# Lumina-Group/libzkp

Measured on NVIDIA B200. Metric: groth16_bn254_proofs_per_sec_batched, higher is better.
Workload: dtype u256 (8x32-bit Montgomery limbs, integer)

## Files before the change

### include/lzkp_b200.h

```cpp
#ifndef LZKP_B200_H
#define LZKP_B200_H
#include <stddef.h>
#include <stdint.h>

#ifdef __cplusplus
extern "C" {
#endif

#define LZKP_OK 0
#define LZKP_E_INVALID (-1)
#define LZKP_E_NO_DEVICE (-2)
#define LZKP_E_CUDA (-3)
#define LZKP_E_STATE (-4)
#define LZKP_E_NOMEM (-5)
#define LZKP_E_UNSUPPORTED (-6)

#define LZKP_CIRCUIT_EQUALITY 0
#define LZKP_CIRCUIT_MEMBERSHIP 1

typedef struct lzkp_pk lzkp_pk;

typedef struct lzkp_pk_options {
    int window_bits;
    uint64_t table_budget_bytes;
    uint32_t max_chunk;
    uint32_t shard_index, shard_count;
} lzkp_pk_options;
#define LZKP_PARTIAL_BYTES 768

int lzkp_init(const int *devices, int n_devices);
int lzkp_device_count(void);
int lzkp_shutdown(void);
const char *lzkp_last_error(void);
uint64_t lzkp_kernel_launches(void);

#define LZKP_REGION_WITGEN 0
#define LZKP_REGION_WITNESS_MAP 1
#define LZKP_REGION_DIGITS 2
#define LZKP_REGION_MSM_G1 3
#define LZKP_REGION_MSM_G2 4
#define LZKP_REGION_ASSEMBLE 5
#define LZKP_PROFILE_REGIONS 8
int lzkp_profile_enable(int on);
int lzkp_profile_read(lzkp_pk *pk, double ms[LZKP_PROFILE_REGIONS], uint64_t count[LZKP_PROFILE_REGIONS], int reset);

int lzkp_pk_load(const uint8_t *pk_bytes, size_t len, int validate, lzkp_pk **out);
int lzkp_pk_load_ex(const uint8_t *pk_bytes, size_t len, int validate, const lzkp_pk_options *opt, lzkp_pk **out);
void lzkp_pk_free(lzkp_pk *pk);
int lzkp_pk_info(const lzkp_pk *pk, uint64_t info[8]);
int lzkp_pk_work(const lzkp_pk *pk, uint64_t work[4]);

int lzkp_circuit_load(lzkp_pk *pk, uint32_t m, uint32_t n_inst, uint32_t n_wit,
                      const uint32_t *a_rowptr, const uint32_t *a_col, const uint8_t *a_val,
                      const uint32_t *b_rowptr, const uint32_t *b_col, const uint8_t *b_val,
                      const uint32_t *c_rowptr, const uint32_t *c_col, const uint8_t *c_val);
int lzkp_circuit_builtin(lzkp_pk *pk, int kind, uint32_t param);
int lzkp_builtin_circuit_csr(int kind, uint32_t param, uint64_t shape[6], uint32_t *rowptr[3], uint32_t *col[3],
                             uint8_t *val[3]);

int lzkp_key_sizes(uint32_t m, uint32_t n_inst, uint32_t n_wit, size_t *pk_len, size_t *vk_len);
int lzkp_setup(uint32_t m, uint32_t n_inst, uint32_t n_wit,
               const uint32_t *a_rowptr, const uint32_t *a_col, const uint8_t *a_val,
               const uint32_t *b_rowptr, const uint32_t *b_col, const uint8_t *b_val,
               const uint32_t *c_rowptr, const uint32_t *c_col, const uint8_t *c_val,
               const uint8_t toxic[160], uint8_t *pk_out, size_t pk_cap, uint8_t *vk_out, size_t vk_cap);
int lzkp_setup_builtin(int kind, uint32_t param, const uint8_t toxic[160], uint8_t *pk_out, size_t pk_cap,
                       uint8_t *vk_out, size_t vk_cap);

int lzkp_generator_mul(int group, const uint8_t *scalars, size_t n, uint8_t *out_affine);

int lzkp_builtin_witness(int kind, uint32_t param, uint64_t value, uint64_t other, const uint64_t *set,
                         uint32_t set_len, const uint8_t *commitment, uint8_t *z_out, size_t z_cap);

int lzkp_prove_batch(lzkp_pk *pk, size_t n_proofs, const uint8_t *z, const uint8_t *r, const uint8_t *s,
                     uint8_t *proofs_out, int32_t *status);
int lzkp_prove_batch_device(lzkp_pk *pk, size_t n_proofs, const void *d_z, const void *d_r, const void *d_s,
                            void *d_proofs, void *d_status, void *stream);
int lzkp_prove_equality_batch(lzkp_pk *pk, size_t n_proofs, const uint64_t *a, const uint64_t *b,
                              const uint8_t *commitments, const uint8_t *r, const uint8_t *s, uint8_t *proofs_out,
                              uint8_t *commitments_out, int32_t *status);
int lzkp_prove_membership_batch(lzkp_pk *pk, size_t n_proofs, const uint64_t *value, const uint64_t *sets,
                                const uint32_t *set_len, uint32_t set_stride, const uint8_t *commitments,
                                const uint8_t *r, const uint8_t *s, uint8_t *proofs_out, uint8_t *commitments_out,
                                int32_t *status);
int lzkp_prove_equality_enveloped(lzkp_pk *pk, size_t n_proofs, const uint64_t *a, const uint64_t *b, const uint8_t *r,
                                  const uint8_t *s, uint8_t *envelopes_out, uint32_t *envelope_len, int32_t *status);
int lzkp_prove_membership_enveloped(lzkp_pk *pk, size_t n_proofs, const uint64_t *value, const uint64_t *sets,
                                    const uint32_t *set_len, uint32_t set_stride, const uint8_t *r, const uint8_t *s,
                                    uint8_t *envelopes_out, uint32_t envelope_stride, uint32_t *envelope_len,
                                    int32_t *status);
int lzkp_prove_equality_batch_device(lzkp_pk *pk, size_t n_proofs, const void *d_a, const void *d_b, const void *d_r,
                                     const void *d_s, void *d_proofs, void *d_status, void *stream);

int lzkp_witness_map(lzkp_pk *pk, size_t n_proofs, const uint8_t *z, uint8_t *h_out);

int lzkp_witness_map_device(lzkp_pk *pk, const void *d_z, void *d_h, void *stream);
int lzkp_pk_shard_info(const lzkp_pk *pk, uint32_t first[5], uint32_t count[5], uint32_t *map_ranks);
int lzkp_prove_partial_device(lzkp_pk *pk, const void *d_z, const void *d_r, const void *d_s, const void *d_h,
                              void *d_partial, void *d_status, void *stream, int phase);
int lzkp_prove_combine_device(lzkp_pk *pk, const void *d_partials, int n_partials, const void *d_r, const void *d_s,
                              void *d_proof, void *stream);

int lzkp_msm_g1(const uint8_t *bases_affine, const uint8_t *scalars, size_t n, uint8_t *out_affine);
int lzkp_msm_g2(const uint8_t *bases_affine, const uint8_t *scalars, size_t n, uint8_t *out_affine);
typedef struct lzkp_bases lzkp_bases;
int lzkp_bases_load(int group, const uint8_t *bases_affine, size_t n, int window_bits, int resident_windows,
                    int validate, lzkp_bases **out);
void lzkp_bases_free(lzkp_bases *b);
int lzkp_msm(lzkp_bases *b, const uint8_t *scalars, size_t n, uint8_t *out_affine);
int lzkp_msm_device(lzkp_bases *b, const void *d_scalars, size_t n, void *d_out_affine, void *stream);

int lzkp_ntt(uint8_t *data, uint32_t log_n, int inverse, int coset);
int lzkp_ntt_device(void *d_in, void *d_out, uint32_t log_n, int inverse, int coset, void *stream);

typedef struct lzkp_vk lzkp_vk;
int lzkp_vk_load(const uint8_t *vk_bytes, size_t len, lzkp_vk **out);
void lzkp_vk_free(lzkp_vk *vk);
int lzkp_verify_batch(lzkp_vk *vk, size_t n, const uint8_t *proofs, const uint8_t *public_inputs, size_t n_pub,
                      uint8_t *ok_out);
int lzkp_vk_info(const lzkp_vk *vk, uint64_t info[4]);

int lzkp_commit_value_snark(uint64_t value, uint8_t out[32]);

#ifdef __cplusplus
}
#endif
#endif
```

### integration/rust/lzkp-sys/src/lib.rs

```rust
#![allow(non_camel_case_types)]
use std::ffi::CStr;
use std::os::raw::{c_char, c_int, c_void};

#[repr(C)]
pub struct lzkp_pk {
    _private: [u8; 0],
}
#[repr(C)]
pub struct lzkp_vk {
    _private: [u8; 0],
}
#[repr(C)]
#[derive(Default, Clone, Copy)]
pub struct lzkp_pk_options {
    pub window_bits: c_int,
    pub table_budget_bytes: u64,
    pub max_chunk: u32,
    pub shard_index: u32,
    pub shard_count: u32,
}
pub const LZKP_CIRCUIT_EQUALITY: c_int = 0;
pub const LZKP_CIRCUIT_MEMBERSHIP: c_int = 1;

extern "C" {
    pub fn lzkp_init(devices: *const c_int, n_devices: c_int) -> c_int;
    pub fn lzkp_device_count() -> c_int;
    pub fn lzkp_last_error() -> *const c_char;
    pub fn lzkp_pk_load_ex(pk: *const u8, len: usize, validate: c_int, opt: *const lzkp_pk_options,
                           out: *mut *mut lzkp_pk) -> c_int;
    pub fn lzkp_pk_free(pk: *mut lzkp_pk);
    pub fn lzkp_circuit_builtin(pk: *mut lzkp_pk, kind: c_int, param: u32) -> c_int;
    pub fn lzkp_key_sizes(m: u32, n_inst: u32, n_wit: u32, pk_len: *mut usize, vk_len: *mut usize) -> c_int;
    pub fn lzkp_setup_builtin(kind: c_int, param: u32, toxic: *const u8, pk_out: *mut u8, pk_cap: usize,
                              vk_out: *mut u8, vk_cap: usize) -> c_int;
    pub fn lzkp_prove_batch(pk: *mut lzkp_pk, n: usize, z: *const u8, r: *const u8, s: *const u8,
                            proofs_out: *mut u8, status: *mut i32) -> c_int;
    pub fn lzkp_prove_equality_batch(pk: *mut lzkp_pk, n: usize, a: *const u64, b: *const u64,
                                     commitments: *const u8, r: *const u8, s: *const u8, proofs_out: *mut u8,
                                     commitments_out: *mut u8, status: *mut i32) -> c_int;
    pub fn lzkp_prove_membership_batch(pk: *mut lzkp_pk, n: usize, value: *const u64, sets: *const u64,
                                       set_len: *const u32, set_stride: u32, commitments: *const u8,
                                       r: *const u8, s: *const u8, proofs_out: *mut u8,
                                       commitments_out: *mut u8, status: *mut i32) -> c_int;
    pub fn lzkp_prove_equality_enveloped(pk: *mut lzkp_pk, n: usize, a: *const u64, b: *const u64, r: *const u8,
                                         s: *const u8, envelopes_out: *mut u8, envelope_len: *mut u32,
                                         status: *mut i32) -> c_int;
    pub fn lzkp_prove_membership_enveloped(pk: *mut lzkp_pk, n: usize, value: *const u64, sets: *const u64,
                                           set_len: *const u32, set_stride: u32, r: *const u8, s: *const u8,
                                           envelopes_out: *mut u8, envelope_stride: u32, envelope_len: *mut u32,
                                           status: *mut i32) -> c_int;
    pub fn lzkp_vk_load(vk: *const u8, len: usize, out: *mut *mut lzkp_vk) -> c_int;
    pub fn lzkp_vk_free(vk: *mut lzkp_vk);
    pub fn lzkp_vk_info(vk: *const lzkp_vk, info: *mut u64) -> c_int;
    pub fn lzkp_verify_batch(vk: *mut lzkp_vk, n: usize, proofs: *const u8, public_inputs: *const u8, n_pub: usize,
                             ok_out: *mut u8) -> c_int;
    pub fn lzkp_commit_value_snark(value: u64, out: *mut u8) -> c_int;
    pub fn lzkp_msm_g1(bases: *const u8, scalars: *const u8, n: usize, out: *mut u8) -> c_int;
    pub fn lzkp_msm_g2(bases: *const u8, scalars: *const u8, n: usize, out: *mut u8) -> c_int;
    pub fn lzkp_ntt(data: *mut u8, log_n: u32, inverse: c_int, coset: c_int) -> c_int;
    pub fn lzkp_prove_batch_device(pk: *mut lzkp_pk, n: usize, d_z: *const c_void, d_r: *const c_void,
                                   d_s: *const c_void, d_proofs: *mut c_void, d_status: *mut c_void,
                                   stream: *mut c_void) -> c_int;
}

pub fn last_error() -> String {
    unsafe { CStr::from_ptr(lzkp_last_error()).to_string_lossy().into_owned() }
}

pub struct DevicePk(*mut lzkp_pk);
unsafe impl Send for DevicePk {}
unsafe impl Sync for DevicePk {}

impl DevicePk {
    pub fn load(pk_bytes: &[u8], kind: c_int, param: u32, validate: bool) -> Result<Self, String> {
        let mut h: *mut lzkp_pk = std::ptr::null_mut();
        let opt = lzkp_pk_options::default();
        let rc = unsafe { lzkp_pk_load_ex(pk_bytes.as_ptr(), pk_bytes.len(), validate as c_int, &opt, &mut h) };
        if rc != 0 {
            return Err(last_error());
        }
        let pk = DevicePk(h);
        if unsafe { lzkp_circuit_builtin(pk.0, kind, param) } != 0 {
            return Err(last_error());
        }
        Ok(pk)
    }

    pub fn prove_equality(&self, a: &[u64], b: &[u64], commitments: &[[u8; 32]], r: &[[u8; 32]],
                          s: &[[u8; 32]]) -> Result<Vec<Option<[u8; 256]>>, String> {
        let n = a.len();
        if b.len() != n || commitments.len() != n || r.len() != n || s.len() != n {
            return Err(format!("prove_equality: slice lengths differ (a {}, b {}, commitments {}, r {}, s {})",
                               n, b.len(), commitments.len(), r.len(), s.len()));
        }
        let mut proofs = vec![0u8; 256 * n];
        let mut status = vec![0i32; n];
        let rc = unsafe {
            lzkp_prove_equality_batch(self.0, n, a.as_ptr(), b.as_ptr(), commitments.as_ptr() as *const u8,
                                      r.as_ptr() as *const u8, s.as_ptr() as *const u8, proofs.as_mut_ptr(),
                                      std::ptr::null_mut(), status.as_mut_ptr())
        };
        if rc != 0 {
            return Err(last_error());
        }
        Ok((0..n).map(|i| if status[i] == 0 {
            let mut p = [0u8; 256];
            p.copy_from_slice(&proofs[256 * i..256 * (i + 1)]);
            Some(p)
        } else { None }).collect())
    }
}

impl Drop for DevicePk {
    fn drop(&mut self) {
        unsafe { lzkp_pk_free(self.0) }
    }
}
```

### libzkp_b200/_ffi.py

```python
from __future__ import annotations

import ctypes as C
import os

_HERE = os.path.dirname(os.path.abspath(__file__))
LIB_PATH = os.environ.get("LZKP_B200_LIB") or os.path.join(_HERE, "_lib", "liblzkp_b200.so")

LZKP_OK = 0
LZKP_E_INVALID = -1
LZKP_E_NO_DEVICE = -2
LZKP_E_CUDA = -3
LZKP_E_STATE = -4
LZKP_E_NOMEM = -5
LZKP_E_UNSUPPORTED = -6
LZKP_CIRCUIT_EQUALITY = 0
LZKP_CIRCUIT_MEMBERSHIP = 1
LZKP_PARTIAL_BYTES = 768


class PkOptions(C.Structure):
    _fields_ = [("window_bits", C.c_int), ("table_budget_bytes", C.c_uint64), ("max_chunk", C.c_uint32),
                ("shard_index", C.c_uint32), ("shard_count", C.c_uint32)]


_vp, _sz, _int = C.c_void_p, C.c_size_t, C.c_int
_u32, _u64 = C.c_uint32, C.c_uint64
SIGNATURES = {
    "lzkp_init": (_int, [_vp, _int]),
    "lzkp_device_count": (_int, []),
    "lzkp_shutdown": (_int, []),
    "lzkp_last_error": (C.c_char_p, []),
    "lzkp_kernel_launches": (_u64, []),
    "lzkp_profile_enable": (_int, [_int]),
    "lzkp_profile_read": (_int, [_vp, C.POINTER(C.c_double), C.POINTER(_u64), _int]),
    "lzkp_pk_load": (_int, [_vp, _sz, _int, C.POINTER(_vp)]),
    "lzkp_pk_load_ex": (_int, [_vp, _sz, _int, C.POINTER(PkOptions), C.POINTER(_vp)]),
    "lzkp_pk_free": (None, [_vp]),
    "lzkp_pk_info": (_int, [_vp, C.POINTER(_u64)]),
    "lzkp_pk_work": (_int, [_vp, C.POINTER(_u64)]),
    "lzkp_pk_shard_info": (_int, [_vp, C.POINTER(_u32), C.POINTER(_u32), C.POINTER(_u32)]),
    "lzkp_circuit_load": (_int, [_vp, _u32, _u32, _u32] + [_vp] * 9),
    "lzkp_circuit_builtin": (_int, [_vp, _int, _u32]),
    "lzkp_builtin_circuit_csr": (_int, [_int, _u32, C.POINTER(_u64), C.POINTER(_vp), C.POINTER(_vp), C.POINTER(_vp)]),
    "lzkp_key_sizes": (_int, [_u32, _u32, _u32, C.POINTER(_sz), C.POINTER(_sz)]),
    "lzkp_setup": (_int, [_u32, _u32, _u32] + [_vp] * 9 + [_vp, _vp, _sz, _vp, _sz]),
    "lzkp_setup_builtin": (_int, [_int, _u32, _vp, _vp, _sz, _vp, _sz]),
    "lzkp_generator_mul": (_int, [_int, _vp, _sz, _vp]),
    "lzkp_prove_batch": (_int, [_vp, _sz, _vp, _vp, _vp, _vp, _vp]),
    "lzkp_prove_batch_device": (_int, [_vp, _sz, _vp, _vp, _vp, _vp, _vp, _vp]),
    "lzkp_builtin_witness": (_int, [_int, _u32, _u64, _u64, _vp, _u32, _vp, _vp, _sz]),
    "lzkp_prove_equality_batch": (_int, [_vp, _sz, _vp, _vp, _vp, _vp, _vp, _vp, _vp, _vp]),
    "lzkp_prove_membership_batch": (_int, [_vp, _sz, _vp, _vp, _vp, _u32, _vp, _vp, _vp, _vp, _vp, _vp]),
    "lzkp_prove_equality_enveloped": (_int, [_vp, _sz, _vp, _vp, _vp, _vp, _vp, _vp, _vp]),
    "lzkp_prove_membership_enveloped": (_int, [_vp, _sz, _vp, _vp, _vp, _u32, _vp, _vp, _vp, _u32, _vp, _vp]),
    "lzkp_prove_equality_batch_device": (_int, [_vp, _sz, _vp, _vp, _vp, _vp, _vp, _vp, _vp]),
    "lzkp_witness_map": (_int, [_vp, _sz, _vp, _vp]),
    "lzkp_witness_map_device": (_int, [_vp, _vp, _vp, _vp]),
    "lzkp_prove_partial_device": (_int, [_vp, _vp, _vp, _vp, _vp, _vp, _vp, _vp, _int]),
    "lzkp_prove_combine_device": (_int, [_vp, _vp, _int, _vp, _vp, _vp, _vp]),
    "lzkp_msm_g1": (_int, [_vp, _vp, _sz, _vp]),
    "lzkp_msm_g2": (_int, [_vp, _vp, _sz, _vp]),
    "lzkp_bases_load": (_int, [_int, _vp, _sz, _int, _int, _int, C.POINTER(_vp)]),
    "lzkp_bases_free": (None, [_vp]),
    "lzkp_msm": (_int, [_vp, _vp, _sz, _vp]),
    "lzkp_msm_device": (_int, [_vp, _vp, _sz, _vp, _vp]),
    "lzkp_ntt": (_int, [_vp, _u32, _int, _int]),
    "lzkp_ntt_device": (_int, [_vp, _vp, _u32, _int, _int, _vp]),
    "lzkp_vk_load": (_int, [_vp, _sz, C.POINTER(_vp)]),
    "lzkp_vk_free": (None, [_vp]),
    "lzkp_vk_info": (_int, [_vp, C.POINTER(_u64)]),
    "lzkp_verify_batch": (_int, [_vp, _sz, _vp, _vp, _sz, _vp]),
    "lzkp_commit_value_snark": (_int, [_u64, _vp]),
}

_lib = None


def lib():
    global _lib
    if _lib is None:
        if not os.path.exists(LIB_PATH):
            raise ImportError(
                f"{LIB_PATH} is missing: build it with `python -c 'import __graft_entry__ as g; g.build()'` "
                "(the engine has no CPU fallback)")
        L = C.CDLL(LIB_PATH)
        for name, (res, args) in SIGNATURES.items():
            fn = getattr(L, name)
            fn.restype = res
            fn.argtypes = args
        _lib = L
    return _lib


def last_error() -> str:
    return (lib().lzkp_last_error() or b"").decode("utf-8", "replace")


def check(rc: int) -> None:
    if rc != LZKP_OK:
        from .errors import EngineError
        raise EngineError(rc, last_error())
```

### libzkp_b200/csrc/engine.cu

```cuda
#include <cuda_runtime.h>
#include <atomic>
#include <cmath>
#include <cstdio>
#include <cstdlib>
#include <mutex>
#include <string>
#include <thread>
#include <type_traits>
#include <vector>

#include "common.h"
#include "host_util.h"
#include "kernels_prove.cuh"
#include "tables.h"
#include "large.h"
#include "setup.h"
#include "verify.h"

using namespace lzkp;
using namespace lzkp::eng;

static thread_local std::string g_err;
static std::mutex g_mu;
static int g_device = -1;
static std::vector<int> g_devices;
static thread_local int t_device = -1;
static uint64_t g_mimc_uploaded = 0;
static std::atomic<int> g_profile{0};

namespace lzkp {
namespace eng {
std::atomic<uint64_t> g_launches{0};
int fail(int code, const std::string &msg) {
    g_err = msg;
    return code;
}
int DBuf::alloc(size_t n) {
    release();
    if (n == 0) n = 16;
    cudaError_t e = cudaMalloc(&p, n);
    if (e != cudaSuccess) {
        p = nullptr;
        cudaGetLastError();
        return fail(LZKP_E_NOMEM, "cudaMalloc(" + std::to_string(n) + "): " + cudaGetErrorString(e));
    }
    bytes = n;
    return LZKP_OK;
}
void DBuf::release() {
    if (p) cudaFree(p);
    p = nullptr;
    bytes = 0;
}
int ensure_device() {
    std::lock_guard<std::mutex> lk(g_mu);
    if (g_device < 0) {
        int n = 0;
        cudaError_t e = cudaGetDeviceCount(&n);
        if (e != cudaSuccess || n == 0) {
            cudaGetLastError();
            return fail(LZKP_E_NO_DEVICE, "no CUDA device: this engine has no CPU fallback");
        }
        int dev = 0;
        if (const char *lr = getenv("LOCAL_RANK")) dev = atoi(lr) % n;
        g_device = dev;
    }
    const int dev = t_device >= 0 ? t_device : g_device;
    CUDA_TRY(cudaSetDevice(dev));
    if (!(g_mimc_uploaded >> (dev & 63) & 1)) {
        std::vector<Fr> c(110);
        for (uint32_t i = 0; i < 110; i++) c[i] = host::mimc_constant(i);
        CUDA_TRY(cudaMemcpyToSymbol(c_mimc, c.data(), sizeof(Fr) * 110));
        g_mimc_uploaded |= 1ull << (dev & 63);
    }
    return LZKP_OK;
}
int current_device() { return t_device >= 0 ? t_device : g_device; }
DeviceScope::DeviceScope(int dev) : prev(t_device) {
    t_device = dev;
    cudaSetDevice(dev);
}
DeviceScope::~DeviceScope() {
    t_device = prev;
    const int back = prev >= 0 ? prev : g_device;
    if (back >= 0) cudaSetDevice(back);
}
}
}


struct MsmPlan {
    DBuf table;
    DBuf unit_dig, unit_tbl;
    DBuf items[4];
    DBuf msm_items[4];
    uint32_t n_items[4] = {0, 0, 0, 0};
    uint32_t item_len[4] = {8, 32, 128, 512};
    uint32_t n_units = 0, n_rows = 0, n_msm = 0;
    std::vector<uint32_t> msm_unit_begin;
    std::vector<uint2> msm_items_host[4];
};

struct HBuf {
    void *p = nullptr;
    size_t bytes = 0;
    int ensure(size_t n) {
        if (n <= bytes) return LZKP_OK;
        if (p) cudaFreeHost(p);
        p = nullptr;
        bytes = 0;
        cudaError_t err = cudaMallocHost(&p, n);
        if (err != cudaSuccess) { p = nullptr; cudaGetLastError(); return fail(LZKP_E_NOMEM, "cudaMallocHost failed"); }
        bytes = n;
        return LZKP_OK;
    }
    template <class T> T *as() const { return reinterpret_cast<T *>(p); }
    ~HBuf() { if (p) cudaFreeHost(p); }
};
struct Workspace {
    uint32_t chunk = 0;
    DBuf z, abc, tmp, h, dig, r, s, rs, part1, part2, res1, res2, proofs, status, a, b, commit, sets, setlen, env, envlen;
    HBuf h_proofs, h_status, h_commit, h_env, h_envlen;
    cudaEvent_t last_use = nullptr;
    ~Workspace() { if (last_use) cudaEventDestroy(last_use); }
};
static int ws_acquire(Workspace &ws, cudaStream_t st) {
    if (!ws.last_use) CUDA_TRY(cudaEventCreateWithFlags(&ws.last_use, cudaEventDisableTiming));
    else CUDA_TRY(cudaStreamWaitEvent(st, ws.last_use, 0));
    return LZKP_OK;
}
static int ws_release(Workspace &ws, cudaStream_t st) {
    CUDA_TRY(cudaEventRecord(ws.last_use, st));
    return LZKP_OK;
}

struct lzkp_pk {
    std::mutex mu;
    int device = 0;
    std::vector<lzkp_pk *> replicas;
    uint32_t n_vars = 0, n_inst = 0, n_wit = 0, n = 0, log_n = 0, m = 0;
    bool has_circuit = false;
    int kind = -1;
    uint32_t kind_param = 0;
    int c = 16;
    uint32_t W = 16, N = 32768;
    uint64_t table_bytes = 0;
    uint32_t max_chunk = 8192;
    uint32_t n_dig_rows = 0, nz = 0;
    MsmPlan g1, g2;
    MsmPlan g1_lat;
    uint32_t row_sz = 0, row_rz = 0;
    bool has_lat = false;
    ProofConsts consts;
    DBuf csr_rowptr[3], csr_col[3], csr_val[3];
    CsrDev csr[3];
    DBuf tw_fwd, tw_inv, coset_br, uncoset_br;
    NttTables ntt;
    Workspace ws[2];
    bool large = false;
    bool tiled_wm = false;
    MsmBases *L_a = nullptr, *L_b1 = nullptr, *L_b2 = nullptr, *L_l = nullptr, *L_h = nullptr;
    DBuf L_sa, L_sb, L_sl, L_sb1;
    cudaStream_t L_st[3] = {nullptr, nullptr, nullptr}, L_st_scale = nullptr;
    cudaEvent_t L_ev_in = nullptr, L_ev_done[3] = {nullptr, nullptr, nullptr}, L_ev_a = nullptr, L_ev_scale = nullptr;
    uint32_t shard_index = 0, shard_count = 1, map_ranks = 1;
    bool L_scaled = false;
    uint32_t L_lo[5] = {0, 0, 0, 0, 0}, L_cnt[5] = {0, 0, 0, 0, 0};
    cudaStream_t stream = nullptr, stream2 = nullptr;
    cudaEvent_t ev_fork = nullptr, ev_join[2] = {nullptr, nullptr};
    cudaStream_t chunk_stream(int i) const { return (i & 1) ? stream2 : stream; }
    struct Mark { int region; cudaEvent_t a, b; };
    std::vector<Mark> marks;
    double prof_ms[LZKP_PROFILE_REGIONS] = {0};
    uint64_t prof_count[LZKP_PROFILE_REGIONS] = {0};
    ~lzkp_pk() {
        for (lzkp_pk *r : replicas) { DeviceScope ds(r->device); delete r; }
        for (auto &m : marks) { cudaEventDestroy(m.a); cudaEventDestroy(m.b); }
        for (MsmBases *b : {L_a, L_b1, L_b2, L_l, L_h}) if (b) msm_bases_free(b);
        for (auto s_ : L_st) if (s_) cudaStreamDestroy(s_);
        if (L_ev_in) cudaEventDestroy(L_ev_in);
        if (L_ev_a) cudaEventDestroy(L_ev_a);
        if (L_ev_scale) cudaEventDestroy(L_ev_scale);
        if (L_st_scale) cudaStreamDestroy(L_st_scale);
        for (auto ev : L_ev_done) if (ev) cudaEventDestroy(ev);
        if (ev_fork) cudaEventDestroy(ev_fork);
        for (auto ev : ev_join) if (ev) cudaEventDestroy(ev);
        if (stream2) cudaStreamDestroy(stream2);
        if (stream) cudaStreamDestroy(stream);
    }
};

struct BaseRef { uint32_t dig_row, tbl_row; };
static int finish_plan(MsmPlan &pl, const std::vector<std::vector<BaseRef>> &msms, uint32_t W) {
    std::vector<uint32_t> ud, ut;
    pl.msm_unit_begin.clear();
    for (auto &ms : msms) {
        pl.msm_unit_begin.push_back((uint32_t)ud.size());
        for (auto &b : ms)
            for (uint32_t w = 0; w < W; w++) {
                ud.push_back(b.dig_row * W + w);
                ut.push_back(b.tbl_row * W + w);
            }
    }
    pl.msm_unit_begin.push_back((uint32_t)ud.size());
    pl.n_units = (uint32_t)ud.size();
    pl.n_msm = (uint32_t)msms.size();
    TRY(upload(pl.unit_dig, ud));
    TRY(upload(pl.unit_tbl, ut));
    for (int v = 0; v < 4; v++) {
        std::vector<uint2> items, mi;
        for (uint32_t q = 0; q < pl.n_msm; q++) {
            uint32_t first = (uint32_t)items.size();
            for (uint32_t u = pl.msm_unit_begin[q]; u < pl.msm_unit_begin[q + 1]; u += pl.item_len[v])
                items.push_back(make_uint2(u, std::min(u + pl.item_len[v], pl.msm_unit_begin[q + 1])));
            mi.push_back(make_uint2(first, (uint32_t)items.size()));
        }
        pl.n_items[v] = (uint32_t)items.size();
        pl.msm_items_host[v] = mi;
        TRY(upload(pl.items[v], items));
        TRY(upload(pl.msm_items[v], mi));
    }
    return LZKP_OK;
}

static uint32_t fit_item_len(const std::vector<std::vector<BaseRef>> &msms, uint32_t W, uint32_t resident) {
    uint32_t best = 128;
    uint64_t best_cost = UINT64_MAX;
    for (uint32_t len = 96; len <= 192; len++) {
        uint64_t items = 0, cost = 0;
        for (auto &ms : msms) items += ((uint64_t)ms.size() * W + len - 1) / len;
        for (uint64_t gx : {8u, 16u, 32u, 64u}) cost += (gx * items + resident - 1) / resident * len * (64 / gx);
        if (cost < best_cost) { best_cost = cost; best = len; }
    }
    return best;
}

static inline uint32_t window_count(int c) { return (uint32_t)((255 + c - 1) / c); }

namespace {
struct Reader {
    const uint8_t *p, *end;
    bool take(size_t n, const uint8_t **out) {
        if ((size_t)(end - p) < n) return false;
        *out = p;
        p += n;
        return true;
    }
    bool g1(host::G1Canon &o) { const uint8_t *b; return take(64, &b) && host::read_g1(b, o); }
    bool g2(host::G2Canon &o) { const uint8_t *b; return take(128, &b) && host::read_g2(b, o); }
    bool vec_g1(std::vector<host::G1Canon> &v) {
        const uint8_t *b;
        if (!take(8, &b)) return false;
        uint64_t len;
        memcpy(&len, b, 8);
        if (len > (uint64_t)(end - p) / 64) return false;
        v.resize(len);
        for (auto &x : v) if (!g1(x)) return false;
        return true;
    }
    bool vec_g2(std::vector<host::G2Canon> &v) {
        const uint8_t *b;
        if (!take(8, &b)) return false;
        uint64_t len;
        memcpy(&len, b, 8);
        if (len > (uint64_t)(end - p) / 128) return false;
        v.resize(len);
        for (auto &x : v) if (!g2(x)) return false;
        return true;
    }
};
host::G1Canon neg_canon(const host::G1Canon &p) {
    host::G1Canon r = p;
    if (!host::is_inf(p)) {
        Fq m = Fq::modulus();
        sub8(r.y.l, m.l, p.y.l);
    }
    return r;
}
}

static int pk_load_impl(const uint8_t *bytes, size_t len, int validate, const lzkp_pk_options *opt, lzkp_pk *pk) {
    static_assert(sizeof(host::G1Canon) == sizeof(G1Affine) && sizeof(host::G2Canon) == sizeof(G2Affine), "layout");
    Reader rd{bytes, bytes + len};
    host::G1Canon alpha_g1, beta_g1, delta_g1;
    host::G2Canon beta_g2, gamma_g2, delta_g2;
    std::vector<host::G1Canon> gamma_abc, a_q, b1_q, h_q, l_q;
    std::vector<host::G2Canon> b2_q;
    bool ok = rd.g1(alpha_g1) && rd.g2(beta_g2) && rd.g2(gamma_g2) && rd.g2(delta_g2) && rd.vec_g1(gamma_abc) &&
              rd.g1(beta_g1) && rd.g1(delta_g1) && rd.vec_g1(a_q) && rd.vec_g1(b1_q) && rd.vec_g2(b2_q) &&
              rd.vec_g1(h_q) && rd.vec_g1(l_q);
    if (!ok || rd.p != rd.end) return fail(LZKP_E_INVALID, "proving key: malformed ark-serialize bytes");
    const uint32_t nv = (uint32_t)a_q.size();
    if (nv < 2 || b1_q.size() != nv || b2_q.size() != nv || l_q.size() >= nv || gamma_abc.size() + l_q.size() != nv)
        return fail(LZKP_E_INVALID, "proving key: inconsistent query lengths");
    const uint32_t n = (uint32_t)h_q.size() + 1;
    if (n < 2 || (n & (n - 1))) return fail(LZKP_E_INVALID, "proving key: h_query length + 1 is not a power of two");
    pk->n_vars = nv;
    pk->n_wit = (uint32_t)l_q.size();
    pk->n_inst = nv - pk->n_wit;
    pk->n = n;
    pk->log_n = 0;
    while ((1u << pk->log_n) < n) pk->log_n++;
    pk->nz = nv - 1;
    pk->n_dig_rows = pk->nz + 3 + (n - 1);
    const uint32_t ROW_R = pk->nz, ROW_S = pk->nz + 1, ROW_RS = pk->nz + 2, ROW_H = pk->nz + 3;

    {
        size_t free_b0 = 0, total_b0 = 0;
        CUDA_TRY(cudaMemGetInfo(&free_b0, &total_b0));
        const uint64_t budget0 = opt && opt->table_budget_bytes ? opt->table_budget_bytes : (uint64_t)(free_b0 * 0.6);
        const uint64_t rows1_max = 2ull * nv + pk->n_wit + n + 2, rows2_max = (uint64_t)nv + 1;
        const uint64_t min_table = (rows1_max * 64 + rows2_max * 128) * 32 * 128;
        pk->large = pk->log_n > 16 || min_table > budget0 || getenv("LZKP_FORCE_LARGE") != nullptr;
    }
    if (pk->large) {
        CUDA_TRY(cudaStreamCreate(&pk->stream));
    CUDA_TRY(cudaStreamCreate(&pk->stream2));
    CUDA_TRY(cudaEventCreateWithFlags(&pk->ev_fork, cudaEventDisableTiming));
    for (auto &ev : pk->ev_join) CUDA_TRY(cudaEventCreateWithFlags(&ev, cudaEventDisableTiming));
        const int wb = opt && opt->window_bits ? opt->window_bits : 0;
        pk->shard_count = opt && opt->shard_count > 1 ? opt->shard_count : 1;
        pk->shard_index = pk->shard_count > 1 ? opt->shard_index : 0;
        if (pk->shard_index >= pk->shard_count) return fail(LZKP_E_INVALID, "shard_index >= shard_count");
        const uint32_t G_ = pk->shard_count;
        const uint64_t w_g2 = getenv("LZKP_SHARD_G2_WEIGHT") ? (uint64_t)atoi(getenv("LZKP_SHARD_G2_WEIGHT")) : (G_ > 2 ? 32 : 28);
        const uint64_t sizes[5] = {nv, nv, (uint64_t)pk->n_wit + 1, (uint64_t)n - 1, nv}, wts[5] = {10, 10, 10, 10, w_g2};
        const double Wh = (double)sizes[3] * wts[3];
        double Wz = 0;
        for (int q : {0, 1, 2, 4}) Wz += (double)sizes[q] * wts[q];
        const double map_frac = getenv("LZKP_SHARD_MAP_COST") ? atof(getenv("LZKP_SHARD_MAP_COST")) : (G_ > 4 ? 0.085 : 0.11);
        const double M = G_ > 1 ? map_frac * (Wz + Wh) : 0.0;
        uint32_t k = 1;
        while (k < G_ && k * ((Wz + Wh + k * M) / G_ - M) < Wh) k++;
        const double T = (Wz + Wh + k * M) / G_;
        std::vector<double> cutz(G_ + 1, 0.0), share(G_, 0.0);
        for (uint32_t i = 0; i < G_; i++) share[i] = i < k ? std::max(0.0, T - M - Wh / k) : T;
        const double piece_cost = G_ > 2 ? (getenv("LZKP_SHARD_PIECE_COST") ? atof(getenv("LZKP_SHARD_PIECE_COST")) : (G_ > 4 ? 0.25 : 0.45)) * 2.76e6 : 0.0;
        std::vector<double> adj(share);
        for (int round = 0; round < 4; round++) {
            double tot = 0;
            for (uint32_t i = 0; i < G_; i++) tot += adj[i];
            for (uint32_t i = 0; i < G_; i++) cutz[i + 1] = cutz[i] + adj[i] * Wz / tot;
            double bounds[5] = {0, 0, 0, 0, 0};
            { int j = 0; for (int q : {0, 1, 2, 4}) { bounds[j + 1] = bounds[j] + (double)sizes[q] * wts[q]; j++; } }
            if (piece_cost != 0.0)
                for (uint32_t i = 1; i < G_; i++)
                    for (int j = 1; j < 4; j++)
                        if (std::fabs(cutz[i] - bounds[j]) < 1.0e5) cutz[i] = bounds[j];
            if (round == 3 || piece_cost == 0.0) break;
            double extra_total = 0;
            std::vector<double> extra(G_, 0.0);
            for (uint32_t i = 0; i < G_; i++) {
                int pieces = 0;
                for (int j = 0; j < 4; j++)
                    if (std::min(cutz[i + 1], bounds[j + 1]) - std::max(cutz[i], bounds[j]) > 1e-6 * Wz) pieces++;
                extra[i] = piece_cost * std::max(0, pieces - 1);
                extra_total += extra[i];
            }
            for (uint32_t i = 0; i < G_; i++) adj[i] = std::max(0.0, share[i] - extra[i] + extra_total / G_);
        }
        pk->map_ranks = k;
        const uint32_t me = pk->shard_index;
        if (me < k) {
            pk->L_lo[3] = (uint32_t)(sizes[3] * me / k);
            pk->L_cnt[3] = (uint32_t)(sizes[3] * (me + 1) / k) - pk->L_lo[3];
        } else {
            pk->L_lo[3] = 0;
            pk->L_cnt[3] = 0;
        }
        double acc_w = 0;
        for (int q : {0, 1, 2, 4}) {
            auto first_at = [&](double w) -> uint64_t {
                if (w <= acc_w) return 0;
                return std::min<uint64_t>((uint64_t)std::ceil((w - acc_w) / wts[q]), sizes[q]);
            };
            uint64_t lo = first_at(cutz[me]), hi = me + 1 == G_ ? sizes[q] : first_at(cutz[me + 1]);
            pk->L_lo[q] = (uint32_t)lo;
            pk->L_cnt[q] = (uint32_t)(hi - lo);
            acc_w += (double)sizes[q] * wts[q];
        }
        auto load1 = [&](std::vector<host::G1Canon> v, size_t skip, const host::G1Canon *extra, int q, MsmBases **out) {
            v.erase(v.begin(), v.begin() + skip);
            if (extra) v.push_back(*extra);
            return msm_bases_load(1, reinterpret_cast<const uint8_t *>(v.data() + pk->L_lo[q]), pk->L_cnt[q], wb, 1, validate, out, 1);
        };
        host::G1Canon nd1 = neg_canon(delta_g1);
        TRY(load1(a_q, 1, &delta_g1, 0, &pk->L_a));
        TRY(load1(b1_q, 1, &delta_g1, 1, &pk->L_b1));
        TRY(load1(l_q, 0, &nd1, 2, &pk->L_l));
        TRY(load1(h_q, 0, nullptr, 3, &pk->L_h));
        {
            std::vector<host::G2Canon> v(b2_q.begin() + 1, b2_q.end());
            v.push_back(delta_g2);
            TRY(msm_bases_load(2, reinterpret_cast<const uint8_t *>(v.data() + pk->L_lo[4]), pk->L_cnt[4], wb, 1, validate, &pk->L_b2, 1));
        }
        {
            int prio_lo = 0, prio_hi = 0;
            CUDA_TRY(cudaDeviceGetStreamPriorityRange(&prio_lo, &prio_hi));
            const bool prio = !(getenv("LZKP_NO_STREAM_PRIORITY") && atoi(getenv("LZKP_NO_STREAM_PRIORITY")));
            for (int i = 0; i < 3; i++)
                CUDA_TRY(cudaStreamCreateWithPriority(&pk->L_st[i], cudaStreamNonBlocking, prio_lo));
            CUDA_TRY(cudaStreamCreateWithPriority(&pk->L_st_scale, cudaStreamNonBlocking, prio ? prio_hi : prio_lo));
        }
        CUDA_TRY(cudaEventCreateWithFlags(&pk->L_ev_in, cudaEventDisableTiming));
        CUDA_TRY(cudaEventCreateWithFlags(&pk->L_ev_a, cudaEventDisableTiming));
        CUDA_TRY(cudaEventCreateWithFlags(&pk->L_ev_scale, cudaEventDisableTiming));
        for (auto &ev : pk->L_ev_done) CUDA_TRY(cudaEventCreateWithFlags(&ev, cudaEventDisableTiming));
        pk->c = wb ? wb : 16;
        pk->W = (255 + pk->c - 1) / pk->c;
        pk->max_chunk = 1;
        pk->table_bytes = ((uint64_t)(a_q.size() + b1_q.size() + l_q.size() + 1 + h_q.size()) * 64 + (uint64_t)b2_q.size() * 128) * pk->W;
        std::vector<host::G1Canon> misc1 = {alpha_g1, beta_g1, a_q[0], b1_q[0]};
        std::vector<host::G2Canon> misc2 = {beta_g2, b2_q[0]};
        DBuf d_misc1, d_misc2, d_out1, d_out2;
        cudaStream_t st = pk->stream;
        TRY(upload(d_misc1, misc1)); TRY(upload(d_misc2, misc2));
        LAUNCH(k_fq_to_mont, 1, 128, 0, st, d_misc1.as<Fq>(), misc1.size() * 2);
        LAUNCH(k_fq_to_mont, 1, 128, 0, st, d_misc2.as<Fq>(), misc2.size() * 4);
        if (validate) {
            std::vector<host::G1Canon> v1 = gamma_abc;
            v1.push_back(alpha_g1); v1.push_back(beta_g1); v1.push_back(delta_g1); v1.push_back(a_q[0]); v1.push_back(b1_q[0]);
            std::vector<host::G2Canon> v2 = {beta_g2, gamma_g2, delta_g2, b2_q[0]};
            DBuf d_v1, d_v2, d_bad;
            TRY(upload(d_v1, v1)); TRY(upload(d_v2, v2)); TRY(d_bad.alloc(sizeof(int)));
            CUDA_TRY(cudaMemsetAsync(d_bad.p, 0, sizeof(int), st));
            LAUNCH(k_fq_to_mont, (unsigned)((v1.size() * 2 + 127) / 128), 128, 0, st, d_v1.as<Fq>(), v1.size() * 2);
            LAUNCH(k_fq_to_mont, 1, 128, 0, st, d_v2.as<Fq>(), v2.size() * 4);
            LAUNCH(k_check_g1, (unsigned)((v1.size() + 63) / 64), 64, 0, st, d_v1.as<G1Affine>(), (uint32_t)v1.size(), d_bad.as<int>());
            LAUNCH(k_check_g2, 1, 64, 0, st, d_v2.as<G2Affine>(), (uint32_t)v2.size(), d_bad.as<int>());
            int bad = 0;
            CUDA_TRY(cudaMemcpyAsync(&bad, d_bad.p, sizeof(int), cudaMemcpyDeviceToHost, st));
            CUDA_TRY(cudaStreamSynchronize(st));
            if (bad) return fail(LZKP_E_INVALID, "proving key: " + std::to_string(bad) + " point(s) off-curve or outside the subgroup");
        }
        TRY(d_out1.alloc(2 * sizeof(G1Affine))); TRY(d_out2.alloc(sizeof(G2Affine)));
        LAUNCH((k_affine_add<Fq>), 1, 1, 0, st, d_misc1.as<G1Affine>() + 0, d_misc1.as<G1Affine>() + 2, d_out1.as<G1Affine>() + 0, 0);
        LAUNCH((k_affine_add<Fq>), 1, 1, 0, st, d_misc1.as<G1Affine>() + 1, d_misc1.as<G1Affine>() + 3, d_out1.as<G1Affine>() + 1, 0);
        LAUNCH((k_affine_add<Fq2>), 1, 1, 0, st, d_misc2.as<G2Affine>() + 0, d_misc2.as<G2Affine>() + 1, d_out2.as<G2Affine>(), 0);
        G1Affine c1[2];
        G2Affine c2;
        CUDA_TRY(cudaMemcpyAsync(c1, d_out1.p, sizeof(c1), cudaMemcpyDeviceToHost, st));
        CUDA_TRY(cudaMemcpyAsync(&c2, d_out2.p, sizeof(c2), cudaMemcpyDeviceToHost, st));
        CUDA_TRY(cudaStreamSynchronize(st));
        pk->consts.a0 = c1[0]; pk->consts.b0 = c1[1]; pk->consts.b2 = c2;
        CUDA_TRY(cudaGetLastError());
        return LZKP_OK;
    }

    std::vector<host::G1Canon> rows1;
    std::vector<host::G2Canon> rows2;
    std::vector<std::vector<BaseRef>> msm1(5), msm2(1);
    std::vector<BaseRef> a_all, b1_all;
    auto add1 = [&](const host::G1Canon &p) { rows1.push_back(p); return (uint32_t)rows1.size() - 1; };
    auto same_point = [](const host::G1Canon &u, const host::G1Canon &v) {
        return memcmp(&u.x, &v.x, sizeof(Fq)) == 0 && memcmp(&u.y, &v.y, sizeof(Fq)) == 0;
    };
    for (uint32_t j = 1; j < nv; j++) {
        const bool has_a = !host::is_inf(a_q[j]), has_b = !host::is_inf(b1_q[j]);
        if (has_a && has_b && same_point(a_q[j], b1_q[j])) {
            const BaseRef ref{j - 1, add1(a_q[j])};
            msm1[4].push_back(ref); a_all.push_back(ref); b1_all.push_back(ref);
            continue;
        }
        if (has_a) { msm1[0].push_back({j - 1, add1(a_q[j])}); a_all.push_back(msm1[0].back()); }
        if (has_b) { msm1[1].push_back({j - 1, add1(b1_q[j])}); b1_all.push_back(msm1[1].back()); }
    }
    for (uint32_t j = 0; j < pk->n_wit; j++) if (!host::is_inf(l_q[j])) msm1[2].push_back({pk->n_inst + j - 1, add1(l_q[j])});
    for (uint32_t i = 0; i + 1 < n; i++) if (!host::is_inf(h_q[i])) msm1[3].push_back({ROW_H + i, add1(h_q[i])});
    if (!host::is_inf(delta_g1)) {
        uint32_t rd1 = add1(delta_g1), rnd1 = add1(neg_canon(delta_g1));
        msm1[0].push_back({ROW_R, rd1});
        msm1[1].push_back({ROW_S, rd1});
        msm1[2].push_back({ROW_RS, rnd1});
        a_all.push_back({ROW_R, rd1});
    }
    std::vector<std::vector<BaseRef>> msm1_lat(6);
    {
        pk->row_sz = pk->n_dig_rows;
        pk->row_rz = pk->n_dig_rows + pk->nz;
        msm1_lat[0] = a_all;
        msm1_lat[2] = msm1[2];
        msm1_lat[3] = msm1[3];
        for (auto &b : a_all) if (b.dig_row < pk->nz) msm1_lat[4].push_back({pk->row_sz + b.dig_row, b.tbl_row});
        for (auto &b : b1_all) msm1_lat[5].push_back({pk->row_rz + b.dig_row, b.tbl_row});
        auto mont = [](const host::G1Canon &c) { return G1Affine{Fq::from_canonical(c.x), Fq::from_canonical(c.y)}; };
        auto canon = [](const G1Affine &m) { host::G1Canon c; c.x = m.x.to_canonical(); c.y = m.y.to_canonical(); return c; };
        auto sum2 = [&](const host::G1Canon &u, const host::G1Canon &v) {
            G1XYZZ t = host::is_inf(u) ? G1XYZZ::inf() : G1XYZZ::from_affine(mont(u));
            if (!host::is_inf(v)) t.madd(mont(v));
            return t.is_inf() ? host::G1Canon{Fq::zero(), Fq::zero()} : canon(t.to_affine());
        };
        const host::G1Canon a0c = sum2(alpha_g1, a_q[0]), b0c = sum2(beta_g1, b1_q[0]), d2c = sum2(delta_g1, delta_g1);
        if (!host::is_inf(a0c)) msm1_lat[4].push_back({ROW_S, add1(a0c)});
        if (!host::is_inf(b0c)) msm1_lat[5].push_back({ROW_R, add1(b0c)});
        if (!host::is_inf(d2c)) msm1_lat[5].push_back({ROW_RS, add1(d2c)});
        pk->n_dig_rows += 2 * pk->nz;
        pk->has_lat = true;
    }
    for (uint32_t j = 1; j < nv; j++)
        if (!host::is_inf(b2_q[j])) { rows2.push_back(b2_q[j]); msm2[0].push_back({j - 1, (uint32_t)rows2.size() - 1}); }
    if (!host::is_inf(delta_g2)) { rows2.push_back(delta_g2); msm2[0].push_back({ROW_S, (uint32_t)rows2.size() - 1}); }
    pk->g1.n_rows = (uint32_t)rows1.size();
    pk->g2.n_rows = (uint32_t)rows2.size();

    size_t free_b = 0, total_b = 0;
    CUDA_TRY(cudaMemGetInfo(&free_b, &total_b));
    uint64_t budget = opt && opt->table_budget_bytes ? opt->table_budget_bytes : (uint64_t)(free_b * 0.6);
    int c = opt && opt->window_bits ? opt->window_bits : 0;
    if (const char *e = getenv("LZKP_WINDOW_BITS")) if (!c) c = atoi(e);
    auto bytes_for = [&](int cc) {
        uint64_t W = window_count(cc), N = 1ull << (cc - 1);
        return (rows1.size() * 64ull + rows2.size() * 128ull) * W * N;
    };
    if (c == 0) {
        c = 16;
        while (c > 8 && bytes_for(c) > budget) c--;
    }
    if (c < 8 || c > 17) return fail(LZKP_E_INVALID, "window_bits must be in [8,17]");
    if (bytes_for(c) > free_b) return fail(LZKP_E_NOMEM, "window tables do not fit in device memory");
    pk->c = c;
    pk->W = window_count(c);
    pk->N = 1u << (c - 1);
    pk->table_bytes = bytes_for(c);
    pk->max_chunk = opt && opt->max_chunk ? opt->max_chunk : 8192;
    if (pk->max_chunk > 32768) pk->max_chunk = 32768;

    CUDA_TRY(cudaStreamCreate(&pk->stream));
    CUDA_TRY(cudaStreamCreate(&pk->stream2));
    CUDA_TRY(cudaEventCreateWithFlags(&pk->ev_fork, cudaEventDisableTiming));
    for (auto &ev : pk->ev_join) CUDA_TRY(cudaEventCreateWithFlags(&ev, cudaEventDisableTiming));
    CUDA_TRY(cudaStreamCreateWithFlags(&pk->L_st[0], cudaStreamNonBlocking));
    CUDA_TRY(cudaEventCreateWithFlags(&pk->L_ev_in, cudaEventDisableTiming));
    CUDA_TRY(cudaEventCreateWithFlags(&pk->L_ev_done[0], cudaEventDisableTiming));
    cudaStream_t st = pk->stream;

    std::vector<host::G1Canon> misc1 = {alpha_g1, beta_g1, delta_g1, a_q[0], b1_q[0]};
    std::vector<host::G2Canon> misc2 = {beta_g2, gamma_g2, delta_g2, b2_q[0]};
    DBuf d_rows1, d_rows2, d_misc1, d_misc2, d_out1, d_out2;
    TRY(upload(d_rows1, rows1)); TRY(upload(d_rows2, rows2)); TRY(upload(d_misc1, misc1)); TRY(upload(d_misc2, misc2));
    auto to_mont = [&](DBuf &b, size_t n_fq) {
        if (n_fq) LAUNCH(k_fq_to_mont, (unsigned)((n_fq + 127) / 128), 128, 0, st, b.as<Fq>(), n_fq);
    };
    to_mont(d_rows1, rows1.size() * 2); to_mont(d_rows2, rows2.size() * 4);
    to_mont(d_misc1, misc1.size() * 2); to_mont(d_misc2, misc2.size() * 4);
    if (validate) {
        std::vector<host::G1Canon> all1 = gamma_abc;
        std::vector<host::G2Canon> all2;
        DBuf d_all1, d_bad;
        TRY(upload(d_all1, all1));
        to_mont(d_all1, all1.size() * 2);
        TRY(d_bad.alloc(sizeof(int)));
        CUDA_TRY(cudaMemsetAsync(d_bad.p, 0, sizeof(int), st));
        auto chk1 = [&](DBuf &b, size_t cnt) {
            if (cnt) LAUNCH(k_check_g1, (unsigned)((cnt + 63) / 64), 64, 0, st, b.as<G1Affine>(), (uint32_t)cnt, d_bad.as<int>());
        };
        auto chk2 = [&](DBuf &b, size_t cnt) {
            if (cnt) LAUNCH(k_check_g2, (unsigned)((cnt + 63) / 64), 64, 0, st, b.as<G2Affine>(), (uint32_t)cnt, d_bad.as<int>());
        };
        chk1(d_rows1, rows1.size()); chk1(d_misc1, misc1.size()); chk1(d_all1, all1.size());
        chk2(d_rows2, rows2.size()); chk2(d_misc2, misc2.size());
        int bad = 0;
        CUDA_TRY(cudaMemcpyAsync(&bad, d_bad.p, sizeof(int), cudaMemcpyDeviceToHost, st));
        CUDA_TRY(cudaStreamSynchronize(st));
        if (bad) return fail(LZKP_E_INVALID, "proving key: " + std::to_string(bad) + " point(s) off-curve or outside the subgroup");
    }
    TRY(d_out1.alloc(2 * sizeof(G1Affine))); TRY(d_out2.alloc(sizeof(G2Affine)));
    LAUNCH((k_affine_add<Fq>), 1, 1, 0, st, d_misc1.as<G1Affine>() + 0, d_misc1.as<G1Affine>() + 3, d_out1.as<G1Affine>() + 0, 0);
    LAUNCH((k_affine_add<Fq>), 1, 1, 0, st, d_misc1.as<G1Affine>() + 1, d_misc1.as<G1Affine>() + 4, d_out1.as<G1Affine>() + 1, 0);
    LAUNCH((k_affine_add<Fq2>), 1, 1, 0, st, d_misc2.as<G2Affine>() + 0, d_misc2.as<G2Affine>() + 3, d_out2.as<G2Affine>(), 0);
    G1Affine c1[2];
    G2Affine c2;
    CUDA_TRY(cudaMemcpyAsync(c1, d_out1.p, sizeof(c1), cudaMemcpyDeviceToHost, st));
    CUDA_TRY(cudaMemcpyAsync(&c2, d_out2.p, sizeof(c2), cudaMemcpyDeviceToHost, st));
    CUDA_TRY(cudaStreamSynchronize(st));
    pk->consts.a0 = c1[0]; pk->consts.b0 = c1[1]; pk->consts.b2 = c2;

    TRY(pk->g1.table.alloc((size_t)rows1.size() * pk->W * pk->N * sizeof(G1Affine)));
    TRY(pk->g2.table.alloc((size_t)rows2.size() * pk->W * pk->N * sizeof(G2Affine)));
    if (!rows1.empty())
        TRY(build_table_g1(d_rows1.p, (uint32_t)rows1.size(), c, pk->W, pk->N, pk->g1.table.p, st));
    if (!rows2.empty())
        TRY(build_table_g2(d_rows2.p, (uint32_t)rows2.size(), c, pk->W, pk->N, pk->g2.table.p, st));
    {
        uint32_t resident = 0;
        TRY(batch_msm_g1_resident(c > 16 ? 4 : 2, &resident));
        pk->g1.item_len[2] = fit_item_len(msm1, pk->W, resident);
    }
    TRY(finish_plan(pk->g1, msm1, pk->W));
    TRY(finish_plan(pk->g1_lat, msm1_lat, pk->W));
    TRY(finish_plan(pk->g2, msm2, pk->W));
    {
        const uint64_t per_proof = (uint64_t)nv * 32 + 7ull * n * 32 + (uint64_t)pk->n_dig_rows * pk->W * (c > 16 ? 4 : 2) +
                                   (uint64_t)pk->g1.n_items[2] * sizeof(G1XYZZ) + (uint64_t)pk->g2.n_items[1] * sizeof(G2XYZZ) +
                                   4 * sizeof(G1XYZZ) + sizeof(G2XYZZ) + 1024;
        size_t free_now = 0, total_now = 0;
        CUDA_TRY(cudaMemGetInfo(&free_now, &total_now));
        uint64_t fit = (uint64_t)(free_now * 0.4) / (2 * per_proof);
        fit = std::max<uint64_t>(32, fit / 32 * 32);
        if (pk->max_chunk > fit) pk->max_chunk = (uint32_t)fit;
    }
    CUDA_TRY(cudaGetLastError());
    return LZKP_OK;
}

static int circuit_install(lzkp_pk *pk, uint32_t m, uint32_t n_inst, uint32_t n_wit, const uint32_t *const rowptr[3],
                           const uint32_t *const col[3], const uint8_t *const val[3]) {
    if (n_inst != pk->n_inst || n_wit != pk->n_wit) return fail(LZKP_E_INVALID, "circuit shape does not match the proving key");
    uint64_t need = (uint64_t)m + n_inst;
    uint32_t n = 1;
    while (n < need) n <<= 1;
    if (n != pk->n) return fail(LZKP_E_INVALID, "circuit domain size does not match the proving key's h_query");
    pk->tiled_wm = pk->large || pk->log_n > 12;
    cudaStream_t st = pk->stream;
    for (int k = 0; k < 3; k++) {
        uint32_t nnz = rowptr[k][m];
        for (uint32_t i = 0; i < nnz; i++) if (col[k][i] >= pk->n_vars) return fail(LZKP_E_INVALID, "matrix column out of range");
        TRY(pk->csr_rowptr[k].alloc(sizeof(uint32_t) * (m + 1)));
        TRY(pk->csr_col[k].alloc(sizeof(uint32_t) * nnz));
        TRY(pk->csr_val[k].alloc(sizeof(Fr) * (size_t)nnz));
        CUDA_TRY(cudaMemcpy(pk->csr_rowptr[k].p, rowptr[k], sizeof(uint32_t) * (m + 1), cudaMemcpyHostToDevice));
        if (nnz) {
            CUDA_TRY(cudaMemcpy(pk->csr_col[k].p, col[k], sizeof(uint32_t) * nnz, cudaMemcpyHostToDevice));
            CUDA_TRY(cudaMemcpy(pk->csr_val[k].p, val[k], 32 * (size_t)nnz, cudaMemcpyHostToDevice));
            LAUNCH(k_to_r2_form, (nnz + 127) / 128, 128, 0, st, pk->csr_val[k].as<Fr>(), nnz);
        }
        pk->csr[k] = CsrDev{pk->csr_rowptr[k].as<uint32_t>(), pk->csr_col[k].as<uint32_t>(), pk->csr_val[k].as<Fr>()};
    }
    pk->m = m;
    Fr w, wi, g, gi;
    for (int i = 0; i < 8; i++) { w.l[i] = FrParams::ROOT28(i); wi.l[i] = FrParams::ROOT28_INV(i); g.l[i] = FrParams::GEN(i); gi.l[i] = FrParams::GEN_INV(i); }
    for (uint32_t i = pk->log_n; i < 28; i++) { w = w.sqr(); wi = wi.sqr(); }
    Fr ninv = host::fr_from_u64(n).inverse();
    Fr gn = g;
    for (uint32_t i = 0; i < pk->log_n; i++) gn = gn.sqr();
    Fr zinv = (gn - Fr::one()).inverse();
    if (pk->tiled_wm) {
        pk->ntt = NttTables{nullptr, nullptr, nullptr, nullptr, nullptr, ninv, zinv};
        CUDA_TRY(cudaStreamSynchronize(st));
        CUDA_TRY(cudaGetLastError());
        pk->has_circuit = true;
        return LZKP_OK;
    }
    TRY(pk->tw_fwd.alloc(sizeof(Fr) * (n / 2))); TRY(pk->tw_inv.alloc(sizeof(Fr) * (n / 2)));
    TRY(pk->coset_br.alloc(sizeof(Fr) * n)); TRY(pk->uncoset_br.alloc(sizeof(Fr) * n));
    LAUNCH(k_pow_table, (n / 2 + 127) / 128, 128, 0, st, pk->tw_fwd.as<Fr>(), w, Fr::one(), n / 2, 0u);
    LAUNCH(k_pow_table, (n / 2 + 127) / 128, 128, 0, st, pk->tw_inv.as<Fr>(), wi, Fr::one(), n / 2, 0u);
    LAUNCH(k_pow_table, (n + 127) / 128, 128, 0, st, pk->coset_br.as<Fr>(), g, ninv, n, pk->log_n);
    LAUNCH(k_pow_table, (n + 127) / 128, 128, 0, st, pk->uncoset_br.as<Fr>(), gi, ninv.to_canonical(), n, pk->log_n);
    pk->ntt = NttTables{pk->tw_fwd.as<Fr>(), pk->tw_inv.as<Fr>(), pk->coset_br.as<Fr>(), pk->uncoset_br.as<Fr>(), nullptr, ninv, zinv};
    size_t smem = (size_t)32 * n;
    if (smem > 48 * 1024) {
        CUDA_TRY(cudaFuncSetAttribute(k_ntt_icoset, cudaFuncAttributeMaxDynamicSharedMemorySize, (int)smem));
        CUDA_TRY(cudaFuncSetAttribute(k_ntt_final, cudaFuncAttributeMaxDynamicSharedMemorySize, (int)smem));
    }
    CUDA_TRY(cudaStreamSynchronize(st));
    CUDA_TRY(cudaGetLastError());
    pk->has_circuit = true;
    return LZKP_OK;
}

static inline int item_variant(uint32_t P) {
    return P > small_batch_limit() ? (P >= 256 ? 2 : 1) : 0;
}
static inline int fit_variant(const MsmPlan &pl, int v) {
    while (v < 3 && pl.n_items[v] > 65535u) v++;
    return v;
}
static inline uint32_t latency_limit() {
    static const uint32_t v = getenv("LZKP_LATENCY_BATCH") ? (uint32_t)atoi(getenv("LZKP_LATENCY_BATCH")) : 384u;
    return v;
}
static inline bool use_lat(const lzkp_pk *pk, uint32_t P) { return pk->has_lat && P <= latency_limit() && P <= small_batch_limit(); }
static inline int item_variant_g2(uint32_t P) {
    return P > small_batch_limit() ? 1 : 0;
}
static int ensure_workspace(lzkp_pk *pk, Workspace &ws, uint32_t P) {
    if (P <= ws.chunk) return LZKP_OK;
    size_t part1 = 0, part2 = 0;
    for (uint32_t pp : {std::min(P, small_batch_limit()), std::min(P, std::max(latency_limit(), 1u)), std::min(P, 255u), std::min(P, 2047u), P}) {
        part1 = std::max(part1, (size_t)pk->g1.n_items[fit_variant(pk->g1, item_variant(pp))] * pp);
        if (use_lat(pk, pp)) part1 = std::max(part1, (size_t)pk->g1_lat.n_items[fit_variant(pk->g1_lat, item_variant(pp))] * pp);
        part2 = std::max(part2, (size_t)pk->g2.n_items[fit_variant(pk->g2, item_variant_g2(pp))] * pp);
    }
    const size_t nv = pk->n_vars, n = pk->n;
    TRY(ws.z.ensure(P * nv * 32));
    TRY(ws.abc.ensure(3 * P * n * 32));
    TRY(ws.h.ensure(P * n * 32));
    if (pk->tiled_wm) TRY(ws.tmp.ensure(3 * P * n * 32));
    if (pk->large) {
        TRY(pk->L_sa.ensure(nv * 32)); TRY(pk->L_sb.ensure(nv * 32)); TRY(pk->L_sb1.ensure(nv * 32)); TRY(pk->L_sl.ensure(((size_t)pk->n_wit + 1) * 32));
    } else {
        TRY(ws.dig.ensure((size_t)pk->n_dig_rows * pk->W * P * (pk->c > 16 ? 4 : 2)));
    }
    TRY(ws.r.ensure(P * 32)); TRY(ws.s.ensure(P * 32)); TRY(ws.rs.ensure(P * 32));
    TRY(ws.part1.ensure(part1 * sizeof(G1XYZZ)));
    TRY(ws.part2.ensure(part2 * sizeof(G2XYZZ)));
    TRY(ws.res1.ensure((size_t)6 * P * sizeof(G1XYZZ)));
    TRY(ws.res2.ensure((size_t)P * sizeof(G2XYZZ)));
    TRY(ws.proofs.ensure((size_t)P * 256));
    TRY(ws.status.ensure((size_t)P * sizeof(int32_t)));
    TRY(ws.a.ensure(P * 8)); TRY(ws.b.ensure(P * 8)); TRY(ws.commit.ensure(P * 32));
    ws.chunk = P;
    return LZKP_OK;
}

static inline void wires_to_canonical(Fr *z, uint32_t P, uint32_t nv, uint32_t first, uint32_t count, cudaStream_t st) {
    const size_t total = (size_t)P * count;
    LAUNCH(k_wires_to_canonical, (unsigned)((total + 127) / 128), 128, 0, st, z, P, nv, first, count);
}

struct Region {
    lzkp_pk *pk;
    cudaStream_t st;
    cudaEvent_t b = nullptr;
    Region(lzkp_pk *pk_, int region, cudaStream_t st_) : pk(pk_), st(st_) {
        if (!g_profile.load(std::memory_order_relaxed) || pk->marks.size() > 65536) return;
        cudaEvent_t a;
        if (cudaEventCreate(&a) != cudaSuccess || cudaEventCreate(&b) != cudaSuccess) { b = nullptr; return; }
        cudaEventRecord(a, st);
        pk->marks.push_back({region, a, b});
    }
    ~Region() { if (b) cudaEventRecord(b, st); }
};

static int run_witness_map(lzkp_pk *pk, Workspace &ws, uint32_t P, cudaStream_t st) {
    const uint32_t n = pk->n, threads = std::max(32u, std::min(n / 2, 512u));
    const size_t smem = (size_t)32 * n;
    Region reg(pk, LZKP_REGION_WITNESS_MAP, st);
    if (pk->tiled_wm) {
        Fr *abc = ws.abc.as<Fr>(), *tmp = ws.tmp.as<Fr>(), *h = ws.h.as<Fr>();
        const size_t plane = (size_t)P * n;
        LAUNCH(k_spmv_abc, dim3((n + 127) / 128, P), 128, 0, st, pk->csr[0], pk->csr[1], pk->csr[2], ws.z.as<Fr>(), abc, P,
               pk->n_vars, pk->m, pk->n_inst, n);
        TRY(large_ntt_device(abc, tmp, pk->log_n, 1, 0, st, 3 * P, n));
        TRY(large_ntt_device(tmp, abc, pk->log_n, 0, 1, st, 3 * P, n));
        LAUNCH(k_pointwise_h, (unsigned)((plane + 127) / 128), 128, 0, st, abc, abc + plane, abc + 2 * plane, tmp, pk->ntt.zinv,
               plane);
        TRY(large_ntt_device(tmp, h, pk->log_n, 1, 1, st, P, n));
        LAUNCH(k_fr_to_canonical, (unsigned)((plane + 127) / 128), 128, 0, st, h, plane);
        return LZKP_OK;
    }
    LAUNCH(k_spmv_abc, dim3((n + 127) / 128, P), 128, 0, st, pk->csr[0], pk->csr[1], pk->csr[2], ws.z.as<Fr>(),
           ws.abc.as<Fr>(), P, pk->n_vars, pk->m, pk->n_inst, n);
    LAUNCH(k_ntt_icoset, dim3(P, 3), threads, smem, st, ws.abc.as<Fr>(), pk->ntt, P, pk->log_n);
    LAUNCH(k_ntt_final, P, threads, smem, st, ws.abc.as<Fr>(), ws.h.as<Fr>(), pk->ntt, P, pk->log_n);
    return LZKP_OK;
}

static int run_prove(lzkp_pk *pk, Workspace &ws, uint32_t P, const Fr *d_r, const Fr *d_s, uint8_t *d_proofs,
                     int32_t *d_status, cudaStream_t st, bool have_h = false, int phase = 3) {
    if (pk->large) {
        if (P != 1) return fail(LZKP_E_STATE, "large-domain proving runs one proof per pass");
        const uint32_t nv = pk->n_vars, ni = pk->n_inst, nw = pk->n_wit;
        const uint8_t *z = ws.z.as<uint8_t>();
        uint8_t *sa = pk->L_sa.as<uint8_t>(), *sb = pk->L_sb.as<uint8_t>(), *sl = pk->L_sl.as<uint8_t>();
        G1XYZZ *res1 = ws.res1.as<G1XYZZ>();
        const uint32_t *lo = pk->L_lo, *cnt = pk->L_cnt;
        if (phase & 1) {
        LAUNCH(k_fr_mul_canonical, 1, 128, 0, st, d_r, d_s, ws.rs.as<Fr>(), 1u);
        LAUNCH(k_check_canonical, (nv + 127) / 128, 128, 0, st, ws.z.as<Fr>(), nv, d_status);
        LAUNCH(k_check_canonical, 1, 32, 0, st, d_r, 1u, d_status);
        LAUNCH(k_check_canonical, 1, 32, 0, st, d_s, 1u, d_status);
        const cudaMemcpyKind dd = cudaMemcpyDeviceToDevice;
        CUDA_TRY(cudaMemcpyAsync(sa, z + 32, (size_t)(nv - 1) * 32, dd, st));
        CUDA_TRY(cudaMemcpyAsync(sa + (size_t)(nv - 1) * 32, d_r, 32, dd, st));
        CUDA_TRY(cudaMemcpyAsync(sb, z + 32, (size_t)(nv - 1) * 32, dd, st));
        CUDA_TRY(cudaMemcpyAsync(sb + (size_t)(nv - 1) * 32, d_s, 32, dd, st));
        CUDA_TRY(cudaMemcpyAsync(sl, z + (size_t)ni * 32, (size_t)nw * 32, dd, st));
        CUDA_TRY(cudaMemcpyAsync(sl + (size_t)nw * 32, ws.rs.p, 32, dd, st));
        CUDA_TRY(cudaEventRecord(pk->L_ev_in, st));
        for (auto s_ : pk->L_st) CUDA_TRY(cudaStreamWaitEvent(s_, pk->L_ev_in, 0));
        CUDA_TRY(cudaStreamWaitEvent(pk->L_st_scale, pk->L_ev_in, 0));
        TRY(msm_device_raw(pk->L_a, sa + (size_t)lo[0] * 32, cnt[0], res1 + 0, pk->L_st_scale));
        pk->L_scaled = cnt[0] || pk->shard_index == 0;
        if (pk->L_scaled) LAUNCH(k_scale_a, 1, 128, 0, pk->L_st_scale, res1, pk->consts, d_r, d_s, pk->shard_index == 0 ? 1 : 0);
        CUDA_TRY(cudaEventRecord(pk->L_ev_scale, pk->L_st_scale));
        {
            Region reg(pk, LZKP_REGION_MSM_G1, pk->L_st[0]);
            TRY(msm_device_raw(pk->L_l, sl + (size_t)lo[2] * 32, cnt[2], res1 + 2, pk->L_st[0]));
        }
        if (cnt[1]) {
            uint8_t *sb1 = pk->L_sb1.as<uint8_t>();
            const uint32_t last = nv - 1, hi = lo[1] + cnt[1], zc = std::min(hi, last) - lo[1];
            if (zc) LAUNCH(k_scalars_times, (zc + 127) / 128, 128, 0, pk->L_st[1], (const Fr *)(sb + (size_t)lo[1] * 32), d_r,
                           (Fr *)(sb1 + (size_t)lo[1] * 32), zc);
            if (hi > last) CUDA_TRY(cudaMemcpyAsync(sb1 + (size_t)last * 32, ws.rs.p, 32, dd, pk->L_st[1]));
            TRY(msm_device_raw(pk->L_b1, sb1 + (size_t)lo[1] * 32, cnt[1], res1 + 1, pk->L_st[1]));
        } else {
            TRY(msm_device_raw(pk->L_b1, sb, 0, res1 + 1, pk->L_st[1]));
        }
        {
            Region reg(pk, LZKP_REGION_MSM_G2, pk->L_st[2]);
            TRY(msm_device_raw(pk->L_b2, sb + (size_t)lo[4] * 32, cnt[4], ws.res2.p, pk->L_st[2]));
        }
        }
        if (!(phase & 2)) return LZKP_OK;
        if (!have_h && cnt[3]) TRY(run_witness_map(pk, ws, P, st));
        TRY(msm_device_raw(pk->L_h, ws.h.as<uint8_t>() + (size_t)lo[3] * 32, cnt[3], res1 + 3, st));
        for (int i = 0; i < 3; i++) {
            CUDA_TRY(cudaEventRecord(pk->L_ev_done[i], pk->L_st[i]));
            CUDA_TRY(cudaStreamWaitEvent(st, pk->L_ev_done[i], 0));
        }
        CUDA_TRY(cudaStreamWaitEvent(st, pk->L_ev_scale, 0));
        if (pk->L_scaled) LAUNCH(k_add_slot, 1, 1, 0, st, res1, 1, 4);
        if (!d_proofs) return LZKP_OK;
        Region reg(pk, LZKP_REGION_ASSEMBLE, st);
        LAUNCH(k_assemble_sums, 1, 96, 0, st, res1, ws.res2.as<G2XYZZ>(), pk->consts, 1u, d_proofs, 1, -1);
        return LZKP_OK;
    }
    const uint32_t c = pk->c, W = pk->W, gx = (P + 127) / 128;
    void *dig = ws.dig.p;
    const uint32_t dig_bytes = pk->c > 16 ? 4u : 2u;
    const bool lat = use_lat(pk, P);
    const uint32_t ymax = 32768u;
    auto digits_z = [&](auto *dg) -> int {
        using DigT = std::remove_pointer_t<decltype(dg)>;
        LAUNCH(k_digits<DigT>, dim3(gx, std::min(pk->nz, ymax)), 128, 0, st, ws.z.as<Fr>(), pk->n_vars, 1u, dg, 0u, P, c, W, d_status, pk->nz);
        LAUNCH(k_digits<DigT>, dim3(gx, 1), 128, 0, st, d_r, 1u, 0u, dg, pk->nz, P, c, W, d_status, 1u);
        LAUNCH(k_digits<DigT>, dim3(gx, 1), 128, 0, st, d_s, 1u, 0u, dg, pk->nz + 1, P, c, W, d_status, 1u);
        LAUNCH(k_digits<DigT>, dim3(gx, 1), 128, 0, st, ws.rs.as<Fr>(), 1u, 0u, dg, pk->nz + 2, P, c, W, d_status, 1u);
        if (lat) {
            LAUNCH(k_digits_scaled<DigT>, dim3(gx, std::min(pk->nz, ymax)), 128, 0, st, ws.z.as<Fr>(), pk->n_vars, 1u, d_s, dg, pk->row_sz, P, c, W, pk->nz);
            LAUNCH(k_digits_scaled<DigT>, dim3(gx, std::min(pk->nz, ymax)), 128, 0, st, ws.z.as<Fr>(), pk->n_vars, 1u, d_r, dg, pk->row_rz, P, c, W, pk->nz);
        }
        return LZKP_OK;
    };
    auto digits_h = [&](auto *dg) -> int {
        using DigT = std::remove_pointer_t<decltype(dg)>;
        LAUNCH(k_digits<DigT>, dim3(gx, std::min(pk->n - 1, ymax)), 128, 0, st, ws.h.as<Fr>(), pk->n, 0u, dg, pk->nz + 3, P, c, W, d_status,
               pk->n - 1);
        return LZKP_OK;
    };
    auto args = [&](MsmPlan &pl, int iv, void *partial, void *out) {
        return BatchMsmArgs{pl.table.p, pk->N, pl.unit_dig.as<uint32_t>(), pl.unit_tbl.as<uint32_t>(), pl.items[iv].p,
                            pl.n_items[iv], pl.msm_items[iv].p, pl.n_msm, dig, dig_bytes, P, partial, out};
    };
    cudaStream_t st_g2 = st;
    if (lat) {
        {
            Region reg(pk, LZKP_REGION_DIGITS, st);
            LAUNCH(k_fr_mul_canonical, gx, 128, 0, st, d_r, d_s, ws.rs.as<Fr>(), P);
            if (dig_bytes == 2) TRY(digits_z((int16_t *)dig)); else TRY(digits_z((int32_t *)dig));
        }
        st_g2 = pk->L_st[0];
        CUDA_TRY(cudaEventRecord(pk->L_ev_in, st));
        CUDA_TRY(cudaStreamWaitEvent(st_g2, pk->L_ev_in, 0));
        { Region reg(pk, LZKP_REGION_MSM_G2, st_g2); batch_msm_g2(args(pk->g2, fit_variant(pk->g2, item_variant_g2(P)), ws.part2.p, ws.res2.p), st_g2); }
        CUDA_TRY(cudaEventRecord(pk->L_ev_done[0], st_g2));
        if (!have_h) TRY(run_witness_map(pk, ws, P, st));
        { Region reg(pk, LZKP_REGION_DIGITS, st); if (dig_bytes == 2) TRY(digits_h((int16_t *)dig)); else TRY(digits_h((int32_t *)dig)); }
    } else {
        if (!have_h) TRY(run_witness_map(pk, ws, P, st));
        Region reg(pk, LZKP_REGION_DIGITS, st);
        LAUNCH(k_fr_mul_canonical, gx, 128, 0, st, d_r, d_s, ws.rs.as<Fr>(), P);
        if (dig_bytes == 2) { TRY(digits_z((int16_t *)dig)); TRY(digits_h((int16_t *)dig)); }
        else { TRY(digits_z((int32_t *)dig)); TRY(digits_h((int32_t *)dig)); }
    }
    MsmPlan &pl1 = lat ? pk->g1_lat : pk->g1;
    static const bool g2_conc = getenv("LZKP_G2_CONCURRENT") && atoi(getenv("LZKP_G2_CONCURRENT")) != 0;
    if (!lat && g2_conc) {
        CUDA_TRY(cudaEventRecord(pk->L_ev_in, st));
        CUDA_TRY(cudaStreamWaitEvent(pk->L_st[0], pk->L_ev_in, 0));
        { Region reg(pk, LZKP_REGION_MSM_G2, pk->L_st[0]); batch_msm_g2(args(pk->g2, fit_variant(pk->g2, item_variant_g2(P)), ws.part2.p, ws.res2.p), pk->L_st[0]); }
        CUDA_TRY(cudaEventRecord(pk->L_ev_done[0], pk->L_st[0]));
    }
    {
        Region reg(pk, LZKP_REGION_MSM_G1, st);
        BatchMsmArgs a1 = args(pl1, fit_variant(pl1, item_variant(P)), ws.part1.p, ws.res1.p);
        a1.table = pk->g1.table.p;
        batch_msm_g1(a1, st);
    }
    if (lat || g2_conc) CUDA_TRY(cudaStreamWaitEvent(st, pk->L_ev_done[0], 0));
    else { Region reg(pk, LZKP_REGION_MSM_G2, st); batch_msm_g2(args(pk->g2, fit_variant(pk->g2, item_variant_g2(P)), ws.part2.p, ws.res2.p), st); }
    Region reg(pk, LZKP_REGION_ASSEMBLE, st);
    if (lat) {
        LAUNCH(k_assemble_sums, (P + 31) / 32, 96, 0, st, ws.res1.as<G1XYZZ>(), ws.res2.as<G2XYZZ>(), pk->consts, P, d_proofs, 4, 5);
        return LZKP_OK;
    }
    LAUNCH(k_assemble, (P + 31) / 32, 128, 0, st, ws.res1.as<G1XYZZ>(), ws.res2.as<G2XYZZ>(), pk->consts, d_r, d_s, P, d_proofs);
    return LZKP_OK;
}

static void blank_failed(size_t n, const int32_t *status, uint8_t *proofs) {
    for (size_t i = 0; i < n; i++)
        if (status[i]) memset(proofs + 256 * i, 0, 256);
}

static int small_ntt_host(uint8_t *data, uint32_t log_n, int inverse, int coset) {
    const uint32_t n = 1u << log_n;
    DBuf d, tw_f, tw_i, cbr, ubr;
    TRY(d.alloc((size_t)n * 32));
    TRY(tw_f.alloc(sizeof(Fr) * std::max(1u, n / 2))); TRY(tw_i.alloc(sizeof(Fr) * std::max(1u, n / 2)));
    TRY(cbr.alloc(sizeof(Fr) * n)); TRY(ubr.alloc(sizeof(Fr) * n));
    Fr w, wi, g, gi;
    for (int i = 0; i < 8; i++) { w.l[i] = FrParams::ROOT28(i); wi.l[i] = FrParams::ROOT28_INV(i); g.l[i] = FrParams::GEN(i); gi.l[i] = FrParams::GEN_INV(i); }
    for (uint32_t i = log_n; i < 28; i++) { w = w.sqr(); wi = wi.sqr(); }
    Fr ninv = host::fr_from_u64(n).inverse();
    cudaStream_t st = nullptr;
    if (n >= 2) {
        LAUNCH(k_pow_table, (n / 2 + 127) / 128, 128, 0, st, tw_f.as<Fr>(), w, Fr::one(), n / 2, 0u);
        LAUNCH(k_pow_table, (n / 2 + 127) / 128, 128, 0, st, tw_i.as<Fr>(), wi, Fr::one(), n / 2, 0u);
    }
    LAUNCH(k_pow_table, (n + 127) / 128, 128, 0, st, cbr.as<Fr>(), g, ninv, n, log_n);
    LAUNCH(k_pow_table, (n + 127) / 128, 128, 0, st, ubr.as<Fr>(), gi, ninv.to_canonical(), n, log_n);
    NttTables T{tw_f.as<Fr>(), tw_i.as<Fr>(), cbr.as<Fr>(), ubr.as<Fr>(), nullptr, ninv, Fr::zero()};
    CUDA_TRY(cudaMemcpy(d.p, data, (size_t)n * 32, cudaMemcpyHostToDevice));
    size_t smem = (size_t)32 * n;
    if (smem > 48 * 1024) CUDA_TRY(cudaFuncSetAttribute(k_ntt_small, cudaFuncAttributeMaxDynamicSharedMemorySize, (int)smem));
    LAUNCH(k_ntt_small, 1, std::max(32u, std::min(n / 2, 512u)), smem, st, d.as<Fr>(), T, log_n, inverse, coset);
    CUDA_TRY(cudaMemcpy(data, d.p, (size_t)n * 32, cudaMemcpyDeviceToHost));
    CUDA_TRY(cudaGetLastError());
    return LZKP_OK;
}

static uint32_t chunk_size(const lzkp_pk *pk, size_t n) {
    if (pk->large) return 1;
    uint32_t c = pk->max_chunk;
    static const int split = getenv("LZKP_BATCH_SPLIT") ? atoi(getenv("LZKP_BATCH_SPLIT")) : 1;
    if (split > 1 && n >= 1024) {
        uint32_t q = (uint32_t)((n + split - 1) / split);
        q = (q + 127) / 128 * 128;
        c = std::min(c, std::max(256u, q));
    }
    return c;
}
struct HostOut {
    uint8_t *proofs; int32_t *status; uint8_t *commit;
    uint8_t *env = nullptr; uint32_t *env_len = nullptr; uint32_t env_stride = 0, scheme = 0; bool with_sets = false;
    uint32_t set_stride = 0;
};
template <class Prep>
static int run_batch_host(lzkp_pk *pk, size_t n, const uint8_t *r, const uint8_t *s, HostOut out, Prep prep) {
    const uint32_t C = chunk_size(pk, n);
    struct Pending { size_t off; uint32_t P; int w; };
    std::vector<Pending> pend;
    auto drain = [&](int w) -> int {
        CUDA_TRY(cudaStreamSynchronize(pk->chunk_stream(w)));
        for (auto it = pend.begin(); it != pend.end();) {
            if (it->w != w) { ++it; continue; }
            Workspace &ws = pk->ws[w];
            if (out.proofs) memcpy(out.proofs + it->off * 256, ws.h_proofs.p, (size_t)it->P * 256);
            if (out.env) {
                memcpy(out.env + it->off * out.env_stride, ws.h_env.p, (size_t)it->P * out.env_stride);
                memcpy(out.env_len + it->off, ws.h_envlen.p, (size_t)it->P * 4);
            }
            memcpy(out.status + it->off, ws.h_status.p, (size_t)it->P * 4);
            if (out.commit) memcpy(out.commit + it->off * 32, ws.h_commit.p, (size_t)it->P * 32);
            it = pend.erase(it);
        }
        return LZKP_OK;
    };
    int i = 0;
    for (size_t off = 0; off < n; off += C, i++) {
        const int w = pk->large ? 0 : (i & 1);
        const uint32_t P = (uint32_t)std::min<size_t>(C, n - off);
        Workspace &ws = pk->ws[w];
        cudaStream_t st = pk->chunk_stream(w);
        TRY(drain(w));
        TRY(ws_acquire(ws, st));
        TRY(ensure_workspace(pk, ws, P));
        TRY(ws.h_proofs.ensure((size_t)ws.chunk * 256)); TRY(ws.h_status.ensure((size_t)ws.chunk * 4));
        TRY(ws.h_commit.ensure((size_t)ws.chunk * 32));
        CUDA_TRY(cudaMemcpyAsync(ws.r.p, r + off * 32, (size_t)P * 32, cudaMemcpyHostToDevice, st));
        CUDA_TRY(cudaMemcpyAsync(ws.s.p, s + off * 32, (size_t)P * 32, cudaMemcpyHostToDevice, st));
        CUDA_TRY(cudaMemsetAsync(ws.status.p, 0, (size_t)P * 4, st));
        TRY(prep(ws, off, P, st));
        TRY(run_prove(pk, ws, P, ws.r.as<Fr>(), ws.s.as<Fr>(), ws.proofs.as<uint8_t>(), ws.status.as<int32_t>(), st));
        if (out.proofs) CUDA_TRY(cudaMemcpyAsync(ws.h_proofs.p, ws.proofs.p, (size_t)P * 256, cudaMemcpyDeviceToHost, st));
        if (out.env) {
            TRY(ws.env.ensure((size_t)ws.chunk * out.env_stride)); TRY(ws.envlen.ensure((size_t)ws.chunk * 4));
            TRY(ws.h_env.ensure((size_t)ws.chunk * out.env_stride)); TRY(ws.h_envlen.ensure((size_t)ws.chunk * 4));
            LAUNCH(k_envelope, (P * 32 + 127) / 128, 128, 0, st, ws.proofs.as<uint8_t>(), ws.commit.as<uint8_t>(),
                   ws.status.as<int32_t>(), out.with_sets ? ws.sets.as<uint64_t>() : nullptr, ws.setlen.as<uint32_t>(),
                   out.set_stride, out.scheme, P, ws.env.as<uint8_t>(), out.env_stride, ws.envlen.as<uint32_t>());
            CUDA_TRY(cudaMemcpyAsync(ws.h_env.p, ws.env.p, (size_t)P * out.env_stride, cudaMemcpyDeviceToHost, st));
            CUDA_TRY(cudaMemcpyAsync(ws.h_envlen.p, ws.envlen.p, (size_t)P * 4, cudaMemcpyDeviceToHost, st));
        }
        CUDA_TRY(cudaMemcpyAsync(ws.h_status.p, ws.status.p, (size_t)P * 4, cudaMemcpyDeviceToHost, st));
        if (out.commit) CUDA_TRY(cudaMemcpyAsync(ws.h_commit.p, ws.commit.p, (size_t)P * 32, cudaMemcpyDeviceToHost, st));
        TRY(ws_release(ws, st));
        pend.push_back({off, P, w});
    }
    TRY(drain(0));
    TRY(drain(1));
    CUDA_TRY(cudaGetLastError());
    if (out.proofs) blank_failed(n, out.status, out.proofs);
    return LZKP_OK;
}
template <class Prep>
static int run_batch_device(lzkp_pk *pk, size_t n, const void *d_r, const void *d_s, void *d_proofs, void *d_status,
                            cudaStream_t caller, Prep prep) {
    const uint32_t C = chunk_size(pk, n);
    const bool fork = !pk->large && n > C;
    if (fork) {
        CUDA_TRY(cudaEventRecord(pk->ev_fork, caller));
        CUDA_TRY(cudaStreamWaitEvent(pk->stream, pk->ev_fork, 0));
        CUDA_TRY(cudaStreamWaitEvent(pk->stream2, pk->ev_fork, 0));
    }
    int i = 0;
    for (size_t off = 0; off < n; off += C, i++) {
        const int w = fork ? (i & 1) : 0;
        const uint32_t P = (uint32_t)std::min<size_t>(C, n - off);
        Workspace &ws = pk->ws[w];
        cudaStream_t st = fork ? pk->chunk_stream(w) : caller;
        TRY(ws_acquire(ws, st));
        TRY(ensure_workspace(pk, ws, P));
        int32_t *stat = (int32_t *)d_status + off;
        CUDA_TRY(cudaMemsetAsync(stat, 0, (size_t)P * 4, st));
        TRY(prep(ws, off, P, stat, st));
        TRY(run_prove(pk, ws, P, (const Fr *)d_r + off, (const Fr *)d_s + off, (uint8_t *)d_proofs + off * 256, stat, st));
        TRY(ws_release(ws, st));
    }
    if (fork) {
        for (int w = 0; w < 2; w++) {
            CUDA_TRY(cudaEventRecord(pk->ev_join[w], pk->chunk_stream(w)));
            CUDA_TRY(cudaStreamWaitEvent(caller, pk->ev_join[w], 0));
        }
    }
    CUDA_TRY(cudaGetLastError());
    return LZKP_OK;
}

static constexpr size_t kFanMinBlock = 256;
static thread_local bool t_in_fan = false;
static inline bool should_fan(const lzkp_pk *pk, size_t n) {
    return !t_in_fan && !pk->replicas.empty() && n >= 2 * kFanMinBlock;
}
static HostOut slice(HostOut o, size_t off) {
    if (o.proofs) o.proofs += off * 256;
    o.status += off;
    if (o.commit) o.commit += off * 32;
    if (o.env) { o.env += off * o.env_stride; o.env_len += off; }
    return o;
}
template <class Fn>
static int fan_out(lzkp_pk *pk, size_t n, Fn fn) {
    const size_t G = std::min<size_t>(1 + pk->replicas.size(), std::max<size_t>(1, n / kFanMinBlock));
    const size_t base = n / G, rem = n % G;
    auto begin = [&](size_t g) { return g * base + std::min(g, rem); };
    std::vector<int> rcs(G, LZKP_OK);
    std::vector<std::string> errs(G);
    std::vector<std::thread> th;
    for (size_t g = 1; g < G; g++)
        th.emplace_back([&, g] {
            lzkp_pk *q = pk->replicas[g - 1];
            DeviceScope ds(q->device);
            t_in_fan = true;
            rcs[g] = fn(q, begin(g), begin(g + 1) - begin(g));
            if (rcs[g] != LZKP_OK) errs[g] = g_err;
        });
    t_in_fan = true;
    rcs[0] = fn(pk, 0, begin(1));
    t_in_fan = false;
    if (rcs[0] != LZKP_OK) errs[0] = g_err;
    for (auto &t : th) t.join();
    for (size_t g = 0; g < G; g++)
        if (rcs[g] != LZKP_OK) return fail(rcs[g], errs[g]);
    return LZKP_OK;
}

#pragma GCC visibility push(default)
extern "C" {

int lzkp_init(const int *devices, int n_devices) {
    if (devices && n_devices > 0) {
        int visible = 0;
        if (cudaGetDeviceCount(&visible) != cudaSuccess || visible == 0) {
            cudaGetLastError();
            return fail(LZKP_E_NO_DEVICE, "no CUDA device: this engine has no CPU fallback");
        }
        if (n_devices > 64) return fail(LZKP_E_INVALID, "at most 64 devices");
        for (int i = 0; i < n_devices; i++) {
            if (devices[i] < 0 || devices[i] >= visible) return fail(LZKP_E_INVALID, "device index out of range");
            for (int j = 0; j < i; j++) if (devices[j] == devices[i]) return fail(LZKP_E_INVALID, "device listed twice");
        }
        std::lock_guard<std::mutex> lk(g_mu);
        if (g_device >= 0 && g_device != devices[0]) return fail(LZKP_E_STATE, "device already selected");
        g_device = devices[0];
        if ((size_t)n_devices > g_devices.size()) g_devices.assign(devices, devices + n_devices);
    }
    TRY(ensure_device());
    std::vector<int> devs;
    { std::lock_guard<std::mutex> lk(g_mu); devs = g_devices; }
    for (size_t i = 1; i < devs.size(); i++) {
        DeviceScope ds(devs[i]);
        TRY(ensure_device());
    }
    return LZKP_OK;
}
int lzkp_device_count(void) {
    std::lock_guard<std::mutex> lk(g_mu);
    return g_devices.empty() ? (g_device >= 0 ? 1 : 0) : (int)g_devices.size();
}
int lzkp_shutdown(void) {
    if (g_device >= 0) cudaSetDevice(g_device);
    ntt_plans_free();
    generator_tables_free();
    return LZKP_OK;
}
const char *lzkp_last_error(void) { return g_err.c_str(); }
uint64_t lzkp_kernel_launches(void) { return g_launches.load(); }

int lzkp_profile_enable(int on) {
    g_profile.store(on ? 1 : 0);
    return LZKP_OK;
}
int lzkp_profile_read(lzkp_pk *pk, double ms[LZKP_PROFILE_REGIONS], uint64_t count[LZKP_PROFILE_REGIONS], int reset) {
    if (!pk || !ms || !count) return fail(LZKP_E_INVALID, "null argument");
    TRY(ensure_device());
    std::lock_guard<std::mutex> lk(pk->mu);
    for (auto &m : pk->marks) {
        float t = 0;
        CUDA_TRY(cudaEventSynchronize(m.b));
        CUDA_TRY(cudaEventElapsedTime(&t, m.a, m.b));
        pk->prof_ms[m.region] += t;
        pk->prof_count[m.region]++;
        cudaEventDestroy(m.a);
        cudaEventDestroy(m.b);
    }
    pk->marks.clear();
    for (int i = 0; i < LZKP_PROFILE_REGIONS; i++) {
        ms[i] = pk->prof_ms[i];
        count[i] = pk->prof_count[i];
        if (reset) { pk->prof_ms[i] = 0; pk->prof_count[i] = 0; }
    }
    return LZKP_OK;
}

int lzkp_pk_load_ex(const uint8_t *pk_bytes, size_t len, int validate, const lzkp_pk_options *opt, lzkp_pk **out) {
    if (!pk_bytes || !out) return fail(LZKP_E_INVALID, "null argument");
    *out = nullptr;
    TRY(ensure_device());
    lzkp_pk *pk = new (std::nothrow) lzkp_pk();
    if (!pk) return fail(LZKP_E_NOMEM, "host allocation failed");
    pk->device = current_device();
    int rc = pk_load_impl(pk_bytes, len, validate, opt, pk);
    if (rc != LZKP_OK) {
        delete pk;
        return rc;
    }
    std::vector<int> devs;
    { std::lock_guard<std::mutex> lk(g_mu); devs = g_devices; }
    const bool sharded = opt && opt->shard_count > 1;
    if (devs.size() > 1 && !sharded && !pk->large && pk->device == devs[0]) {
        lzkp_pk_options ro{};
        if (opt) ro = *opt;
        ro.window_bits = pk->c;
        ro.max_chunk = pk->max_chunk;
        const size_t R = devs.size() - 1;
        std::vector<lzkp_pk *> reps(R, nullptr);
        std::vector<int> rcs(R, LZKP_OK);
        std::vector<std::string> errs(R);
        std::vector<std::thread> th;
        for (size_t i = 0; i < R; i++)
            th.emplace_back([&, i] {
                DeviceScope ds(devs[i + 1]);
                int rc_ = ensure_device();
                lzkp_pk *r = rc_ == LZKP_OK ? new (std::nothrow) lzkp_pk() : nullptr;
                if (rc_ == LZKP_OK && !r) rc_ = fail(LZKP_E_NOMEM, "host allocation failed");
                if (rc_ == LZKP_OK) {
                    r->device = devs[i + 1];
                    rc_ = pk_load_impl(pk_bytes, len, 0 , &ro, r);
                }
                if (rc_ != LZKP_OK) { errs[i] = g_err; delete r; r = nullptr; }
                reps[i] = r;
                rcs[i] = rc_;
            });
        for (auto &t : th) t.join();
        for (size_t i = 0; i < R; i++)
            if (rcs[i] != LZKP_OK) {
                for (lzkp_pk *r : reps) if (r) { DeviceScope ds(r->device); delete r; }
                delete pk;
                return fail(rcs[i], "replica on device " + std::to_string(devs[i + 1]) + ": " + errs[i]);
            }
        pk->replicas = reps;
    }
    *out = pk;
    return LZKP_OK;
}
int lzkp_pk_load(const uint8_t *pk_bytes, size_t len, int validate, lzkp_pk **out) {
    return lzkp_pk_load_ex(pk_bytes, len, validate, nullptr, out);
}
void lzkp_pk_free(lzkp_pk *pk) {
    if (!pk) return;
    DeviceScope ds(pk->device);
    delete pk;
}
int lzkp_pk_info(const lzkp_pk *pk, uint64_t info[8]) {
    if (!pk || !info) return fail(LZKP_E_INVALID, "null argument");
    info[0] = pk->n_vars; info[1] = pk->n_inst; info[2] = pk->n_wit; info[3] = pk->n;
    info[4] = (uint64_t)pk->c; info[5] = pk->W; info[6] = pk->table_bytes; info[7] = pk->max_chunk;
    if (pk->large) info[7] = 1;
    return LZKP_OK;
}

int lzkp_pk_shard_info(const lzkp_pk *pk, uint32_t first[5], uint32_t count[5], uint32_t *map_ranks) {
    if (!pk || !first || !count) return fail(LZKP_E_INVALID, "null argument");
    if (!pk->large) return fail(LZKP_E_STATE, "not a large-domain proving key");
    for (int q = 0; q < 5; q++) { first[q] = pk->L_lo[q]; count[q] = pk->L_cnt[q]; }
    if (map_ranks) *map_ranks = pk->map_ranks;
    return LZKP_OK;
}

int lzkp_pk_work(const lzkp_pk *pk, uint64_t work[4]) {
    if (!pk || !work) return fail(LZKP_E_INVALID, "null argument");
    work[0] = pk->g1.n_units; work[1] = pk->g2.n_units; work[2] = pk->g1.n_rows; work[3] = pk->g2.n_rows;
    return LZKP_OK;
}

int lzkp_circuit_load(lzkp_pk *pk, uint32_t m, uint32_t n_inst, uint32_t n_wit, const uint32_t *a_rowptr,
                      const uint32_t *a_col, const uint8_t *a_val, const uint32_t *b_rowptr, const uint32_t *b_col,
                      const uint8_t *b_val, const uint32_t *c_rowptr, const uint32_t *c_col, const uint8_t *c_val) {
    if (!pk || !a_rowptr || !b_rowptr || !c_rowptr) return fail(LZKP_E_INVALID, "null argument");
    TRY(ensure_device());
    std::lock_guard<std::mutex> lk(pk->mu);
    const uint32_t *rp[3] = {a_rowptr, b_rowptr, c_rowptr}, *cl[3] = {a_col, b_col, c_col};
    const uint8_t *vl[3] = {a_val, b_val, c_val};
    pk->kind = -1;
    TRY(circuit_install(pk, m, n_inst, n_wit, rp, cl, vl));
    for (lzkp_pk *q : pk->replicas) {
        DeviceScope ds(q->device);
        TRY(ensure_device());
        std::lock_guard<std::mutex> lq(q->mu);
        q->kind = -1;
        TRY(circuit_install(q, m, n_inst, n_wit, rp, cl, vl));
    }
    return LZKP_OK;
}
static host::R1cs synth(int kind, uint32_t param) {
    return kind == LZKP_CIRCUIT_EQUALITY ? host::synth_equality(param) : host::synth_membership(param);
}
int lzkp_circuit_builtin(lzkp_pk *pk, int kind, uint32_t param) {
    if (!pk || (kind != LZKP_CIRCUIT_EQUALITY && kind != LZKP_CIRCUIT_MEMBERSHIP) || param == 0)
        return fail(LZKP_E_INVALID, "bad circuit kind / parameter");
    TRY(ensure_device());
    std::lock_guard<std::mutex> lk(pk->mu);
    host::R1cs cs = synth(kind, param);
    const host::Csr *M[3] = {&cs.A, &cs.B, &cs.C};
    const uint32_t *rp[3], *cl[3];
    const uint8_t *vl[3];
    for (int k = 0; k < 3; k++) {
        rp[k] = M[k]->rowptr.data(); cl[k] = M[k]->col.data();
        vl[k] = reinterpret_cast<const uint8_t *>(M[k]->val.data());
    }
    TRY(circuit_install(pk, cs.m, cs.n_inst, cs.n_wit, rp, cl, vl));
    pk->kind = kind;
    pk->kind_param = param;
    for (lzkp_pk *q : pk->replicas) {
        DeviceScope ds(q->device);
        TRY(ensure_device());
        std::lock_guard<std::mutex> lq(q->mu);
        TRY(circuit_install(q, cs.m, cs.n_inst, cs.n_wit, rp, cl, vl));
        q->kind = kind;
        q->kind_param = param;
    }
    return LZKP_OK;
}
int lzkp_builtin_circuit_csr(int kind, uint32_t param, uint64_t shape[6], uint32_t *rowptr[3], uint32_t *col[3],
                             uint8_t *val[3]) {
    if ((kind != LZKP_CIRCUIT_EQUALITY && kind != LZKP_CIRCUIT_MEMBERSHIP) || param == 0 || !shape)
        return fail(LZKP_E_INVALID, "bad circuit kind / parameter");
    host::R1cs cs = synth(kind, param);
    const host::Csr *M[3] = {&cs.A, &cs.B, &cs.C};
    shape[0] = cs.m; shape[1] = cs.n_inst; shape[2] = cs.n_wit;
    for (int k = 0; k < 3; k++) shape[3 + k] = M[k]->col.size();
    if (rowptr && col && val)
        for (int k = 0; k < 3; k++) {
            memcpy(rowptr[k], M[k]->rowptr.data(), sizeof(uint32_t) * (cs.m + 1));
            memcpy(col[k], M[k]->col.data(), sizeof(uint32_t) * M[k]->col.size());
            memcpy(val[k], M[k]->val.data(), 32 * M[k]->col.size());
        }
    return LZKP_OK;
}

int lzkp_key_sizes(uint32_t m, uint32_t n_inst, uint32_t n_wit, size_t *pk_len, size_t *vk_len) {
    if (!pk_len || !vk_len || n_inst < 1) return fail(LZKP_E_INVALID, "bad argument");
    uint64_t need = (uint64_t)m + n_inst, n = 2;
    while (n < need) n <<= 1;
    const size_t nv = (size_t)n_inst + n_wit;
    *vk_len = 64 + 3 * 128 + 8 + 64 * (size_t)n_inst;
    *pk_len = *vk_len + 128 + 5 * 8 + 64 * (2 * nv + (n - 1) + n_wit) + 128 * nv;
    return LZKP_OK;
}
static int setup_common(uint32_t m, uint32_t n_inst, uint32_t n_wit, const uint32_t *const rp[3],
                        const uint32_t *const cl[3], const uint8_t *const vl[3], const uint8_t *toxic, uint8_t *pk_out,
                        size_t pk_cap, uint8_t *vk_out, size_t vk_cap) {
    if (!toxic || !pk_out || !vk_out) return fail(LZKP_E_INVALID, "null argument");
    size_t pl, vl_;
    TRY(lzkp_key_sizes(m, n_inst, n_wit, &pl, &vl_));
    if (pk_cap < pl || vk_cap < vl_) return fail(LZKP_E_INVALID, "setup: output buffer too small (see lzkp_key_sizes)");
    TRY(ensure_device());
    std::vector<uint8_t> pk, vk;
    TRY(setup_run(m, n_inst, n_wit, rp, cl, vl, toxic, pk, vk));
    if (pk.size() != pl || vk.size() != vl_) return fail(LZKP_E_STATE, "setup: size mismatch");
    memcpy(pk_out, pk.data(), pl);
    memcpy(vk_out, vk.data(), vl_);
    return LZKP_OK;
}
int lzkp_setup(uint32_t m, uint32_t n_inst, uint32_t n_wit, const uint32_t *a_rowptr, const uint32_t *a_col,
               const uint8_t *a_val, const uint32_t *b_rowptr, const uint32_t *b_col, const uint8_t *b_val,
               const uint32_t *c_rowptr, const uint32_t *c_col, const uint8_t *c_val, const uint8_t toxic[160],
               uint8_t *pk_out, size_t pk_cap, uint8_t *vk_out, size_t vk_cap) {
    if (!a_rowptr || !b_rowptr || !c_rowptr) return fail(LZKP_E_INVALID, "null argument");
    const uint32_t *rp[3] = {a_rowptr, b_rowptr, c_rowptr}, *cl[3] = {a_col, b_col, c_col};
    const uint8_t *vl[3] = {a_val, b_val, c_val};
    return setup_common(m, n_inst, n_wit, rp, cl, vl, toxic, pk_out, pk_cap, vk_out, vk_cap);
}
int lzkp_setup_builtin(int kind, uint32_t param, const uint8_t toxic[160], uint8_t *pk_out, size_t pk_cap,
                       uint8_t *vk_out, size_t vk_cap) {
    if ((kind != LZKP_CIRCUIT_EQUALITY && kind != LZKP_CIRCUIT_MEMBERSHIP) || param == 0)
        return fail(LZKP_E_INVALID, "bad circuit kind / parameter");
    host::R1cs cs = synth(kind, param);
    const host::Csr *M[3] = {&cs.A, &cs.B, &cs.C};
    const uint32_t *rp[3], *cl[3];
    const uint8_t *vl[3];
    for (int k = 0; k < 3; k++) {
        rp[k] = M[k]->rowptr.data(); cl[k] = M[k]->col.data();
        vl[k] = reinterpret_cast<const uint8_t *>(M[k]->val.data());
    }
    return setup_common(cs.m, cs.n_inst, cs.n_wit, rp, cl, vl, toxic, pk_out, pk_cap, vk_out, vk_cap);
}

int lzkp_generator_mul(int group, const uint8_t *scalars, size_t n, uint8_t *out_affine) {
    if ((group != 1 && group != 2) || (n && (!scalars || !out_affine))) return fail(LZKP_E_INVALID, "bad argument");
    return generator_mul(group, scalars, n, out_affine);
}

int lzkp_prove_batch(lzkp_pk *pk, size_t n_proofs, const uint8_t *z, const uint8_t *r, const uint8_t *s,
                     uint8_t *proofs_out, int32_t *status) {
    if (!pk || (n_proofs && (!z || !r || !s || !proofs_out || !status))) return fail(LZKP_E_INVALID, "null argument");
    if (should_fan(pk, n_proofs)) {
        const size_t zrow = (size_t)pk->n_vars * 32;
        return fan_out(pk, n_proofs, [&](lzkp_pk *q, size_t off, size_t cnt) {
            return lzkp_prove_batch(q, cnt, z + off * zrow, r + off * 32, s + off * 32, proofs_out + off * 256, status + off);
        });
    }
    TRY(ensure_device());
    std::lock_guard<std::mutex> lk(pk->mu);
    if (!pk->has_circuit) return fail(LZKP_E_STATE, "lzkp_circuit_load has not been called");
    const size_t nv = pk->n_vars;
    return run_batch_host(pk, n_proofs, r, s, HostOut{proofs_out, status, nullptr},
                          [&](Workspace &ws, size_t off, uint32_t P, cudaStream_t st) -> int {
        CUDA_TRY(cudaMemcpyAsync(ws.z.p, z + off * nv * 32, (size_t)P * nv * 32, cudaMemcpyHostToDevice, st));
        return LZKP_OK;
    });
}

int lzkp_prove_batch_device(lzkp_pk *pk, size_t n_proofs, const void *d_z, const void *d_r, const void *d_s,
                            void *d_proofs, void *d_status, void *stream) {
    if (!pk || (n_proofs && (!d_z || !d_r || !d_s || !d_proofs || !d_status))) return fail(LZKP_E_INVALID, "null argument");
    TRY(ensure_device());
    std::lock_guard<std::mutex> lk(pk->mu);
    if (!pk->has_circuit) return fail(LZKP_E_STATE, "lzkp_circuit_load has not been called");
    const size_t nv = pk->n_vars;
    return run_batch_device(pk, n_proofs, d_r, d_s, d_proofs, d_status, (cudaStream_t)stream,
                            [&](Workspace &ws, size_t off, uint32_t P, int32_t *, cudaStream_t st) -> int {
        CUDA_TRY(cudaMemcpyAsync(ws.z.p, (const uint8_t *)d_z + off * nv * 32, (size_t)P * nv * 32, cudaMemcpyDeviceToDevice, st));
        return LZKP_OK;
    });
}

int lzkp_builtin_witness(int kind, uint32_t param, uint64_t value, uint64_t other, const uint64_t *set,
                         uint32_t set_len, const uint8_t *commitment, uint8_t *z_out, size_t z_cap) {
    if (!z_out || param == 0) return fail(LZKP_E_INVALID, "bad argument");
    std::vector<Fr> z;
    if (kind == LZKP_CIRCUIT_EQUALITY) z = host::assign_equality(param, value, other, commitment);
    else if (kind == LZKP_CIRCUIT_MEMBERSHIP) {
        if (!set) return fail(LZKP_E_INVALID, "null set");
        z = host::assign_membership(param, value, set, set_len, commitment);
        if (z.empty()) return fail(LZKP_E_INVALID, "membership inputs rejected (empty / oversized set or value not in set)");
    } else return fail(LZKP_E_INVALID, "bad circuit kind");
    if (z_cap < z.size() * 32) return fail(LZKP_E_INVALID, "z_out too small");
    memcpy(z_out, z.data(), z.size() * 32);
    return LZKP_OK;
}

static int equality_batch_impl(lzkp_pk *pk, size_t n_proofs, const uint64_t *a, const uint64_t *b,
                               const uint8_t *commitments, const uint8_t *r, const uint8_t *s, HostOut out) {
    if (!pk || (n_proofs && (!a || !b || !r || !s || !out.status || (!out.proofs && !out.env)))) return fail(LZKP_E_INVALID, "null argument");
    if (should_fan(pk, n_proofs))
        return fan_out(pk, n_proofs, [&](lzkp_pk *q, size_t off, size_t cnt) {
            return equality_batch_impl(q, cnt, a + off, b + off, commitments ? commitments + off * 32 : nullptr, r + off * 32,
                                       s + off * 32, slice(out, off));
        });
    TRY(ensure_device());
    std::lock_guard<std::mutex> lk(pk->mu);
    if (!pk->has_circuit || pk->kind != LZKP_CIRCUIT_EQUALITY) return fail(LZKP_E_STATE, "pk is not bound to the builtin equality circuit");
    return run_batch_host(pk, n_proofs, r, s, out,
                          [&](Workspace &ws, size_t off, uint32_t P, cudaStream_t st) -> int {
        CUDA_TRY(cudaMemcpyAsync(ws.a.p, a + off, (size_t)P * 8, cudaMemcpyHostToDevice, st));
        CUDA_TRY(cudaMemcpyAsync(ws.b.p, b + off, (size_t)P * 8, cudaMemcpyHostToDevice, st));
        if (commitments) CUDA_TRY(cudaMemcpyAsync(ws.commit.p, commitments + off * 32, (size_t)P * 32, cudaMemcpyHostToDevice, st));
        Region reg(pk, LZKP_REGION_WITGEN, st);
        LAUNCH(k_witgen_equality, (P + 127) / 128, 128, 0, st, ws.a.as<uint64_t>(), ws.b.as<uint64_t>(),
               commitments ? ws.commit.as<Fr>() : nullptr, ws.z.as<Fr>(), ws.commit.as<Fr>(), ws.status.as<int32_t>(), P,
               pk->kind_param, pk->n_vars);
        wires_to_canonical(ws.z.as<Fr>(), P, pk->n_vars, 4u, 3u * pk->kind_param, st);
        return LZKP_OK;
    });
}

int lzkp_prove_equality_batch(lzkp_pk *pk, size_t n_proofs, const uint64_t *a, const uint64_t *b,
                              const uint8_t *commitments, const uint8_t *r, const uint8_t *s, uint8_t *proofs_out,
                              uint8_t *commitments_out, int32_t *status) {
    if (n_proofs && !proofs_out) return fail(LZKP_E_INVALID, "null argument");
    HostOut out{proofs_out, status, commitments_out};
    return equality_batch_impl(pk, n_proofs, a, b, commitments, r, s, out);
}
int lzkp_prove_equality_enveloped(lzkp_pk *pk, size_t n_proofs, const uint64_t *a, const uint64_t *b, const uint8_t *r,
                                  const uint8_t *s, uint8_t *envelopes_out, uint32_t *envelope_len, int32_t *status) {
    if (n_proofs && (!envelopes_out || !envelope_len)) return fail(LZKP_E_INVALID, "null argument");
    HostOut out{nullptr, status, nullptr};
    out.env = envelopes_out; out.env_len = envelope_len; out.env_stride = 298; out.scheme = 2;
    return equality_batch_impl(pk, n_proofs, a, b, nullptr, r, s, out);
}

static int membership_batch_impl(lzkp_pk *pk, size_t n_proofs, const uint64_t *value, const uint64_t *sets,
                                 const uint32_t *set_len, uint32_t set_stride, const uint8_t *commitments,
                                 const uint8_t *r, const uint8_t *s, HostOut out) {
    if (!pk || (n_proofs && (!value || !sets || !set_len || !r || !s || !out.status || (!out.proofs && !out.env))))
        return fail(LZKP_E_INVALID, "null argument");
    if (n_proofs && set_stride == 0) return fail(LZKP_E_INVALID, "set_stride must be at least 1");
    if (should_fan(pk, n_proofs))
        return fan_out(pk, n_proofs, [&](lzkp_pk *q, size_t off, size_t cnt) {
            return membership_batch_impl(q, cnt, value + off, sets + off * set_stride, set_len + off, set_stride,
                                         commitments ? commitments + off * 32 : nullptr, r + off * 32, s + off * 32, slice(out, off));
        });
    TRY(ensure_device());
    std::lock_guard<std::mutex> lk(pk->mu);
    if (!pk->has_circuit || pk->kind != LZKP_CIRCUIT_MEMBERSHIP) return fail(LZKP_E_STATE, "pk is not bound to the builtin membership circuit");
    return run_batch_host(pk, n_proofs, r, s, out,
                          [&](Workspace &ws, size_t off, uint32_t P, cudaStream_t st) -> int {
        TRY(ws.sets.ensure((size_t)ws.chunk * set_stride * 8));
        TRY(ws.setlen.ensure((size_t)ws.chunk * 4));
        CUDA_TRY(cudaMemcpyAsync(ws.a.p, value + off, (size_t)P * 8, cudaMemcpyHostToDevice, st));
        CUDA_TRY(cudaMemcpyAsync(ws.sets.p, sets + off * set_stride, (size_t)P * set_stride * 8, cudaMemcpyHostToDevice, st));
        CUDA_TRY(cudaMemcpyAsync(ws.setlen.p, set_len + off, (size_t)P * 4, cudaMemcpyHostToDevice, st));
        if (commitments) CUDA_TRY(cudaMemcpyAsync(ws.commit.p, commitments + off * 32, (size_t)P * 32, cudaMemcpyHostToDevice, st));
        Region reg(pk, LZKP_REGION_WITGEN, st);
        LAUNCH(k_witgen_membership, (P + 127) / 128, 128, 0, st, ws.a.as<uint64_t>(), ws.sets.as<uint64_t>(),
               ws.setlen.as<uint32_t>(), set_stride, commitments ? ws.commit.as<Fr>() : nullptr, ws.z.as<Fr>(),
               ws.commit.as<Fr>(), ws.status.as<int32_t>(), P, pk->kind_param, pk->n_vars);
        wires_to_canonical(ws.z.as<Fr>(), P, pk->n_vars, 2u + 2u * pk->kind_param + 1u, 330u, st);
        return LZKP_OK;
    });
}

int lzkp_prove_membership_batch(lzkp_pk *pk, size_t n_proofs, const uint64_t *value, const uint64_t *sets,
                                const uint32_t *set_len, uint32_t set_stride, const uint8_t *commitments,
                                const uint8_t *r, const uint8_t *s, uint8_t *proofs_out, uint8_t *commitments_out,
                                int32_t *status) {
    if (n_proofs && !proofs_out) return fail(LZKP_E_INVALID, "null argument");
    HostOut out{proofs_out, status, commitments_out};
    return membership_batch_impl(pk, n_proofs, value, sets, set_len, set_stride, commitments, r, s, out);
}
int lzkp_prove_membership_enveloped(lzkp_pk *pk, size_t n_proofs, const uint64_t *value, const uint64_t *sets,
                                    const uint32_t *set_len, uint32_t set_stride, const uint8_t *r, const uint8_t *s,
                                    uint8_t *envelopes_out, uint32_t envelope_stride, uint32_t *envelope_len,
                                    int32_t *status) {
    if (n_proofs && (!envelopes_out || !envelope_len)) return fail(LZKP_E_INVALID, "null argument");
    if (!pk) return fail(LZKP_E_INVALID, "null argument");
    if (pk->kind != LZKP_CIRCUIT_MEMBERSHIP) return fail(LZKP_E_STATE, "pk is not bound to the builtin membership circuit");
    if (envelope_stride < 10 + 4 + 8 * std::max(pk->kind_param, set_stride) + 256 + 32)
        return fail(LZKP_E_INVALID, "envelope_stride below 302 + 8 * set slots");
    HostOut out{nullptr, status, nullptr};
    out.env = envelopes_out; out.env_len = envelope_len; out.env_stride = envelope_stride; out.scheme = 4;
    out.with_sets = true; out.set_stride = set_stride;
    return membership_batch_impl(pk, n_proofs, value, sets, set_len, set_stride, nullptr, r, s, out);
}

int lzkp_prove_equality_batch_device(lzkp_pk *pk, size_t n_proofs, const void *d_a, const void *d_b, const void *d_r,
                                     const void *d_s, void *d_proofs, void *d_status, void *stream) {
    if (!pk || !d_a || !d_b || !d_r || !d_s || !d_proofs || !d_status) return fail(LZKP_E_INVALID, "null argument");
    TRY(ensure_device());
    std::lock_guard<std::mutex> lk(pk->mu);
    if (!pk->has_circuit || pk->kind != LZKP_CIRCUIT_EQUALITY) return fail(LZKP_E_STATE, "pk is not bound to the builtin equality circuit");
    return run_batch_device(pk, n_proofs, d_r, d_s, d_proofs, d_status, (cudaStream_t)stream,
                            [&](Workspace &ws, size_t off, uint32_t P, int32_t *stat, cudaStream_t st) -> int {
        Region reg(pk, LZKP_REGION_WITGEN, st);
        LAUNCH(k_witgen_equality, (P + 127) / 128, 128, 0, st, (const uint64_t *)d_a + off, (const uint64_t *)d_b + off,
               (const Fr *)nullptr, ws.z.as<Fr>(), ws.commit.as<Fr>(), stat, P, pk->kind_param, pk->n_vars);
        wires_to_canonical(ws.z.as<Fr>(), P, pk->n_vars, 4u, 3u * pk->kind_param, st);
        return LZKP_OK;
    });
}

int lzkp_witness_map(lzkp_pk *pk, size_t n_proofs, const uint8_t *z, uint8_t *h_out) {
    if (!pk || (n_proofs && (!z || !h_out))) return fail(LZKP_E_INVALID, "null argument");
    TRY(ensure_device());
    std::lock_guard<std::mutex> lk(pk->mu);
    if (!pk->has_circuit) return fail(LZKP_E_STATE, "lzkp_circuit_load has not been called");
    cudaStream_t st = pk->stream;
    Workspace &ws = pk->ws[0];
    const size_t nv = pk->n_vars, n = pk->n;
    for (size_t off = 0; off < n_proofs; off += pk->max_chunk) {
        uint32_t P = (uint32_t)std::min<size_t>(pk->max_chunk, n_proofs - off);
        TRY(ws_acquire(ws, st));
        TRY(ensure_workspace(pk, ws, P));
        CUDA_TRY(cudaMemcpyAsync(ws.z.p, z + off * nv * 32, (size_t)P * nv * 32, cudaMemcpyHostToDevice, st));
        TRY(run_witness_map(pk, ws, P, st));
        CUDA_TRY(cudaMemcpyAsync(h_out + off * n * 32, ws.h.p, (size_t)P * n * 32, cudaMemcpyDeviceToHost, st));
        TRY(ws_release(ws, st));
        CUDA_TRY(cudaStreamSynchronize(st));
        CUDA_TRY(cudaGetLastError());
    }
    return LZKP_OK;
}

int lzkp_witness_map_device(lzkp_pk *pk, const void *d_z, void *d_h, void *stream) {
    if (!pk || !d_z || !d_h) return fail(LZKP_E_INVALID, "null argument");
    TRY(ensure_device());
    std::lock_guard<std::mutex> lk(pk->mu);
    if (!pk->has_circuit) return fail(LZKP_E_STATE, "lzkp_circuit_load has not been called");
    cudaStream_t st = (cudaStream_t)stream;
    Workspace &ws = pk->ws[0];
    TRY(ws_acquire(ws, st));
    TRY(ensure_workspace(pk, ws, 1));
    CUDA_TRY(cudaMemcpyAsync(ws.z.p, d_z, (size_t)pk->n_vars * 32, cudaMemcpyDeviceToDevice, st));
    TRY(run_witness_map(pk, ws, 1, st));
    CUDA_TRY(cudaMemcpyAsync(d_h, ws.h.p, (size_t)pk->n * 32, cudaMemcpyDeviceToDevice, st));
    TRY(ws_release(ws, st));
    return LZKP_OK;
}

int lzkp_prove_partial_device(lzkp_pk *pk, const void *d_z, const void *d_r, const void *d_s, const void *d_h,
                              void *d_partial, void *d_status, void *stream, int phase) {
    if (phase == 0) phase = 3;
    if (!pk || !d_r || !d_s || !d_status || ((phase & 1) && !d_z) || ((phase & 2) && !d_partial))
        return fail(LZKP_E_INVALID, "null argument");
    TRY(ensure_device());
    std::lock_guard<std::mutex> lk(pk->mu);
    if (!pk->large) return fail(LZKP_E_STATE, "sharded proving needs a large-domain proving key");
    if ((phase & 2) && !d_h && pk->L_cnt[3] && !pk->has_circuit)
        return fail(LZKP_E_STATE, "this shard holds h_query points: pass h, or bind the circuit so that it runs the witness map itself");
    cudaStream_t st = (cudaStream_t)stream;
    Workspace &ws = pk->ws[0];
    TRY(ws_acquire(ws, st));
    TRY(ensure_workspace(pk, ws, 1));
    if (phase & 1) {
        for (auto ev : pk->L_ev_done) CUDA_TRY(cudaStreamWaitEvent(st, ev, 0));
        if (pk->L_ev_scale) CUDA_TRY(cudaStreamWaitEvent(st, pk->L_ev_scale, 0));
        CUDA_TRY(cudaMemsetAsync(d_status, 0, 4, st));
        CUDA_TRY(cudaMemcpyAsync(ws.z.p, d_z, (size_t)pk->n_vars * 32, cudaMemcpyDeviceToDevice, st));
    }
    if ((phase & 2) && d_h) CUDA_TRY(cudaMemcpyAsync(ws.h.p, d_h, (size_t)pk->n * 32, cudaMemcpyDeviceToDevice, st));
    TRY(run_prove(pk, ws, 1, (const Fr *)d_r, (const Fr *)d_s, nullptr, (int32_t *)d_status, st, d_h != nullptr, phase));
    if (!(phase & 2)) { TRY(ws_release(ws, st)); return LZKP_OK; }
    uint8_t *out = (uint8_t *)d_partial;
    CUDA_TRY(cudaMemcpyAsync(out, ws.res1.p, 4 * sizeof(G1XYZZ), cudaMemcpyDeviceToDevice, st));
    CUDA_TRY(cudaMemcpyAsync(out + 4 * sizeof(G1XYZZ), ws.res2.p, sizeof(G2XYZZ), cudaMemcpyDeviceToDevice, st));
    TRY(ws_release(ws, st));
    return LZKP_OK;
}

int lzkp_prove_combine_device(lzkp_pk *pk, const void *d_partials, int n_partials, const void *d_r, const void *d_s,
                              void *d_proof, void *stream) {
    if (!pk || !d_partials || n_partials < 1 || !d_r || !d_s || !d_proof) return fail(LZKP_E_INVALID, "bad argument");
    TRY(ensure_device());
    std::lock_guard<std::mutex> lk(pk->mu);
    if (!pk->large) return fail(LZKP_E_STATE, "sharded proving needs a large-domain proving key");
    cudaStream_t st = (cudaStream_t)stream;
    Workspace &ws = pk->ws[0];
    TRY(ws_acquire(ws, st));
    TRY(ensure_workspace(pk, ws, 1));
    LAUNCH(k_sum_partials, 1, 160, 0, st, (const uint8_t *)d_partials, (uint32_t)n_partials, ws.res1.as<G1XYZZ>(),
           ws.res2.as<G2XYZZ>());
    LAUNCH(k_assemble_sums, 1, 96, 0, st, ws.res1.as<G1XYZZ>(), ws.res2.as<G2XYZZ>(), pk->consts, 1u, (uint8_t *)d_proof, 1, -1);
    TRY(ws_release(ws, st));
    CUDA_TRY(cudaGetLastError());
    return LZKP_OK;
}

int lzkp_msm_g1(const uint8_t *bases_affine, const uint8_t *scalars, size_t n, uint8_t *out_affine) {
    if (!out_affine || (n && (!bases_affine || !scalars))) return fail(LZKP_E_INVALID, "null argument");
    TRY(ensure_device());
    return large_msm_g1_host(bases_affine, scalars, n, out_affine);
}
int lzkp_msm_g2(const uint8_t *bases_affine, const uint8_t *scalars, size_t n, uint8_t *out_affine) {
    if (!out_affine || (n && (!bases_affine || !scalars))) return fail(LZKP_E_INVALID, "null argument");
    TRY(ensure_device());
    return large_msm_g2_host(bases_affine, scalars, n, out_affine);
}
struct lzkp_bases { MsmBases *b; };
int lzkp_bases_load(int group, const uint8_t *bases_affine, size_t n, int window_bits, int resident_windows,
                    int validate, lzkp_bases **out) {
    if (!out || (group != 1 && group != 2) || (n && !bases_affine)) return fail(LZKP_E_INVALID, "bad argument");
    *out = nullptr;
    TRY(ensure_device());
    MsmBases *b = nullptr;
    TRY(msm_bases_load(group, bases_affine, n, window_bits, resident_windows, validate, &b));
    *out = new lzkp_bases{b};
    return LZKP_OK;
}
void lzkp_bases_free(lzkp_bases *b) {
    if (!b) return;
    if (g_device >= 0) cudaSetDevice(g_device);
    msm_bases_free(b->b);
    delete b;
}
int lzkp_msm(lzkp_bases *b, const uint8_t *scalars, size_t n, uint8_t *out_affine) {
    if (!b || !out_affine || (n && !scalars)) return fail(LZKP_E_INVALID, "null argument");
    TRY(ensure_device());
    return msm_host(b->b, scalars, n, out_affine);
}
int lzkp_msm_device(lzkp_bases *b, const void *d_scalars, size_t n, void *d_out_affine, void *stream) {
    if (!b || !d_out_affine || (n && !d_scalars)) return fail(LZKP_E_INVALID, "null argument");
    TRY(ensure_device());
    return msm_device(b->b, d_scalars, n, d_out_affine, (cudaStream_t)stream);
}

int lzkp_ntt(uint8_t *data, uint32_t log_n, int inverse, int coset) {
    if (!data || log_n > 28) return fail(LZKP_E_INVALID, "bad argument");
    TRY(ensure_device());
    if (log_n <= 12 && !getenv("LZKP_NTT_FORCE_TILED")) return small_ntt_host(data, log_n, inverse, coset);
    return large_ntt_host(data, log_n, inverse, coset);
}

int lzkp_ntt_device(void *d_in, void *d_out, uint32_t log_n, int inverse, int coset, void *stream) {
    if (!d_in || !d_out || log_n > 28) return fail(LZKP_E_INVALID, "bad argument");
    if (log_n > 11 && d_in == d_out) return fail(LZKP_E_INVALID, "lzkp_ntt_device: d_out must differ from d_in above 2^11");
    TRY(ensure_device());
    return large_ntt_device(d_in, d_out, log_n, inverse, coset, (cudaStream_t)stream);
}

struct lzkp_vk { VerifyingKeyDev *v; };
int lzkp_vk_load(const uint8_t *vk_bytes, size_t len, lzkp_vk **out) {
    if (!vk_bytes || !out) return fail(LZKP_E_INVALID, "null argument");
    *out = nullptr;
    TRY(ensure_device());
    VerifyingKeyDev *v = nullptr;
    TRY(vk_load(vk_bytes, len, &v));
    *out = new lzkp_vk{v};
    return LZKP_OK;
}
int lzkp_vk_info(const lzkp_vk *vk, uint64_t info[4]) {
    if (!vk || !info) return fail(LZKP_E_INVALID, "null argument");
    vk_info(vk->v, info);
    return LZKP_OK;
}
void lzkp_vk_free(lzkp_vk *vk) {
    if (!vk) return;
    if (g_device >= 0) cudaSetDevice(g_device);
    vk_free(vk->v);
    delete vk;
}
int lzkp_verify_batch(lzkp_vk *vk, size_t n, const uint8_t *proofs, const uint8_t *public_inputs, size_t n_pub,
                      uint8_t *ok_out) {
    if (!vk || (n && (!proofs || !ok_out || (n_pub && !public_inputs)))) return fail(LZKP_E_INVALID, "null argument");
    TRY(ensure_device());
    return verify_batch(vk->v, n, proofs, public_inputs, n_pub, ok_out);
}

int lzkp_commit_value_snark(uint64_t value, uint8_t out[32]) {
    if (!out) return fail(LZKP_E_INVALID, "null argument");
    static std::mutex mu;
    std::lock_guard<std::mutex> lk(mu);
    host::commit_value_snark(value, out);
    return LZKP_OK;
}

}
#pragma GCC visibility pop
```

### libzkp_b200/csrc/kernels_prove.cuh

```cuda
#pragma once
#include "dev_util.cuh"

namespace lzkp {

__global__ void k_pow_table(Fr *out, Fr base, Fr scale, uint32_t count, uint32_t log_rev) {
    uint32_t k = blockIdx.x * blockDim.x + threadIdx.x;
    if (k >= count) return;
    uint32_t e = log_rev ? bitrev(k, log_rev) : k;
    Fr acc = Fr::one(), b = base;
    while (e) {
        if (e & 1u) acc = acc * b;
        b = b.sqr();
        e >>= 1;
    }
    st_vec(out + k, acc * scale);
}
__global__ void k_to_r2_form(Fr *v, uint32_t count) {
    uint32_t k = blockIdx.x * blockDim.x + threadIdx.x;
    if (k >= count) return;
    Fr r3;
#pragma unroll
    for (int i = 0; i < 8; i++) r3.l[i] = FrParams::R3(i);
    st_vec(v + k, ld_vec(v + k) * r3);
}
__global__ void k_fq_to_mont(Fq *v, size_t count) {
    size_t k = (size_t)blockIdx.x * blockDim.x + threadIdx.x;
    if (k >= count) return;
    st_vec(v + k, Fq::from_canonical(ld_vec(v + k)));
}

__constant__ Fr c_mimc[110];

__global__ void k_witgen_equality(const uint64_t *a, const uint64_t *b, const Fr *commit_in, Fr *z, Fr *commit_out,
                                  int32_t *status, uint32_t P, uint32_t rounds, uint32_t nv) {
    uint32_t p = blockIdx.x * blockDim.x + threadIdx.x;
    if (p >= P) return;
    if (a[p] != b[p]) status[p] = 1;
    Fr *zp = z + (size_t)p * nv;
    Fr one = Fr::zero();
    one.l[0] = 1;
    st_vec(zp + 0, one);
    st_vec(zp + 2, fr_from_u64(a[p]));
    st_vec(zp + 3, fr_from_u64(b[p]));
    Fr x = Fr::from_canonical(fr_from_u64(a[p]));
    for (uint32_t i = 0; i < rounds; i++) {
        Fr t = x + c_mimc[i % 110];
        Fr t2 = t.sqr(), t4 = t2.sqr();
        x = t4 * t;
        st_vec(zp + 4 + 3 * i, t2);
        st_vec(zp + 5 + 3 * i, t4);
        st_vec(zp + 6 + 3 * i, x);
    }
    Fr cm = commit_in ? ld_vec(commit_in + p) : x.to_canonical();
    st_vec(zp + 1, cm);
    if (commit_out) st_vec(commit_out + p, cm);
}

__global__ void __launch_bounds__(128) k_wires_to_canonical(Fr *z, uint32_t P, uint32_t nv, uint32_t first, uint32_t count) {
    const size_t i = (size_t)blockIdx.x * blockDim.x + threadIdx.x;
    if (i >= (size_t)P * count) return;
    Fr *e = z + (i / count) * nv + first + (uint32_t)(i % count);
    st_vec(e, ld_vec(e).to_canonical());
}

__global__ void k_witgen_membership(const uint64_t *value, const uint64_t *sets, const uint32_t *set_len,
                                    uint32_t set_stride, const Fr *commit_in, Fr *z, Fr *commit_out, int32_t *status,
                                    uint32_t P, uint32_t S, uint32_t nv) {
    uint32_t p = blockIdx.x * blockDim.x + threadIdx.x;
    if (p >= P) return;
    Fr *zp = z + (size_t)p * nv;
    const uint64_t *set = sets + (size_t)p * set_stride;
    uint32_t len = set_len[p];
    uint64_t v = value[p];
    uint32_t pos = 0xffffffffu;
    if (len >= 1 && len <= S && len <= set_stride)
        for (uint32_t i = 0; i < len; i++)
            if (set[i] == v) { pos = i; break; }
    if (pos == 0xffffffffu) { status[p] = 2; len = 0; }
    Fr one = Fr::zero(), zero = Fr::zero();
    one.l[0] = 1;
    st_vec(zp + 0, one);
    for (uint32_t i = 0; i < S; i++) {
        st_vec(zp + 2 + i, i < len ? fr_from_u64(set[i]) : zero);
        st_vec(zp + 2 + S + i, i < len ? one : zero);
    }
    const uint32_t w0 = 2 + 2 * S;
    st_vec(zp + w0, fr_from_u64(v));
    Fr x = Fr::from_canonical(fr_from_u64(v));
    for (uint32_t i = 0; i < 110; i++) {
        Fr t = x + c_mimc[i];
        Fr t2 = t.sqr(), t4 = t2.sqr();
        x = t4 * t;
        st_vec(zp + w0 + 1 + 3 * i, t2);
        st_vec(zp + w0 + 2 + 3 * i, t4);
        st_vec(zp + w0 + 3 + 3 * i, x);
    }
    Fr cm = commit_in ? ld_vec(commit_in + p) : x.to_canonical();
    st_vec(zp + 1, cm);
    if (commit_out) st_vec(commit_out + p, cm);
    const uint32_t s0 = w0 + 331;
    Fr r = Fr::modulus();
    for (uint32_t i = 0; i < S; i++) {
        bool sel = (i == pos);
        st_vec(zp + s0 + i, sel ? one : zero);
        st_vec(zp + s0 + S + i, zero);
        Fr d = zero;
        if (sel) {
            Fr sv = fr_from_u64(i < len ? set[i] : 0), vv = fr_from_u64(v), t;
            uint32_t bw = sub8(t.l, vv.l, sv.l);
            if (bw) add8(d.l, t.l, r.l); else d = t;
        }
        st_vec(zp + s0 + 2 * S + i, d);
    }
}

struct CsrDev {
    const uint32_t *rowptr;
    const uint32_t *col;
    const Fr *val;
};

__device__ __forceinline__ Fr spmv_row(const CsrDev &M, uint32_t row, const Fr *z) {
    Fr acc = Fr::zero();
    uint32_t lo = __ldg(M.rowptr + row), hi = __ldg(M.rowptr + row + 1);
    for (uint32_t t = lo; t < hi; t++) acc = acc + ldg_vec(M.val + t) * ld_vec(z + __ldg(M.col + t));
    return acc;
}
__global__ void __launch_bounds__(128) k_spmv_abc(CsrDev A, CsrDev B, CsrDev C, const Fr *z, Fr *abc, uint32_t P,
                                                  uint32_t nv, uint32_t m, uint32_t n_inst, uint32_t n) {
    uint32_t i = blockIdx.x * blockDim.x + threadIdx.x, p = blockIdx.y;
    if (i >= n) return;
    const Fr *zp = z + (size_t)p * nv;
    Fr a = Fr::zero(), b = Fr::zero(), c = Fr::zero();
    if (i < m) {
        a = spmv_row(A, i, zp);
        b = spmv_row(B, i, zp);
        c = spmv_row(C, i, zp);
    } else if (i < m + n_inst) {
        a = Fr::from_canonical(ld_vec(zp + (i - m)));
    }
    size_t plane = (size_t)P * n, off = (size_t)p * n + i;
    st_vec(abc + off, a);
    st_vec(abc + plane + off, b);
    st_vec(abc + 2 * plane + off, c);
}

struct SmemPoly {
    uint4 *lo, *hi;
    __device__ __forceinline__ Fr get(uint32_t i) const {
        Fr r;
        uint4 a = lo[i], b = hi[i];
        r.l[0] = a.x; r.l[1] = a.y; r.l[2] = a.z; r.l[3] = a.w;
        r.l[4] = b.x; r.l[5] = b.y; r.l[6] = b.z; r.l[7] = b.w;
        return r;
    }
    __device__ __forceinline__ void put(uint32_t i, const Fr &v) const {
        lo[i] = make_uint4(v.l[0], v.l[1], v.l[2], v.l[3]);
        hi[i] = make_uint4(v.l[4], v.l[5], v.l[6], v.l[7]);
    }
};
__device__ __forceinline__ void ntt_dif(const SmemPoly &s, uint32_t log_n, const Fr *tw) {
    const uint32_t n = 1u << log_n;
    for (uint32_t lh = log_n; lh-- > 0;) {
        const uint32_t h = 1u << lh;
        for (uint32_t bf = threadIdx.x; bf < n / 2; bf += blockDim.x) {
            uint32_t k = bf & (h - 1), i = ((bf >> lh) << (lh + 1)) | k;
            Fr x = s.get(i), y = s.get(i + h);
            s.put(i, x + y);
            Fr d = x - y;
            s.put(i + h, lh == 0 ? d : d * ldg_vec(tw + (k << (log_n - 1 - lh))));
        }
        __syncthreads();
    }
}
__device__ __forceinline__ void ntt_dit(const SmemPoly &s, uint32_t log_n, const Fr *tw) {
    const uint32_t n = 1u << log_n;
    for (uint32_t lh = 0; lh < log_n; lh++) {
        const uint32_t h = 1u << lh;
        for (uint32_t bf = threadIdx.x; bf < n / 2; bf += blockDim.x) {
            uint32_t k = bf & (h - 1), i = ((bf >> lh) << (lh + 1)) | k;
            Fr x = s.get(i), y = s.get(i + h);
            if (lh != 0) y = y * ldg_vec(tw + (k << (log_n - 1 - lh)));
            s.put(i, x + y);
            s.put(i + h, x - y);
        }
        __syncthreads();
    }
}
struct NttTables {
    const Fr *tw_fwd;
    const Fr *tw_inv;
    const Fr *coset_br;
    const Fr *uncoset_br;
    const Fr *ninv_br;
    Fr ninv;
    Fr zinv;
};
__global__ void k_ntt_icoset(Fr *abc, NttTables T, uint32_t P, uint32_t log_n) {
    extern __shared__ uint4 smem[];
    const uint32_t n = 1u << log_n;
    SmemPoly s{smem, smem + n};
    Fr *poly = abc + ((size_t)blockIdx.y * P + blockIdx.x) * n;
    for (uint32_t i = threadIdx.x; i < n; i += blockDim.x) s.put(i, ld_vec(poly + i));
    __syncthreads();
    ntt_dif(s, log_n, T.tw_inv);
    for (uint32_t i = threadIdx.x; i < n; i += blockDim.x) s.put(i, s.get(i) * ldg_vec(T.coset_br + i));
    __syncthreads();
    ntt_dit(s, log_n, T.tw_fwd);
    for (uint32_t i = threadIdx.x; i < n; i += blockDim.x) st_vec(poly + i, s.get(i));
}
__global__ void k_ntt_final(const Fr *abc, Fr *h, NttTables T, uint32_t P, uint32_t log_n) {
    extern __shared__ uint4 smem[];
    const uint32_t n = 1u << log_n;
    SmemPoly s{smem, smem + n};
    const size_t plane = (size_t)P * n, off = (size_t)blockIdx.x * n;
    for (uint32_t i = threadIdx.x; i < n; i += blockDim.x) {
        Fr a = ld_vec(abc + off + i), b = ld_vec(abc + plane + off + i), c = ld_vec(abc + 2 * plane + off + i);
        s.put(i, (a * b - c) * T.zinv);
    }
    __syncthreads();
    ntt_dif(s, log_n, T.tw_inv);
    for (uint32_t i = threadIdx.x; i < n; i += blockDim.x)
        st_vec(h + off + bitrev(i, log_n), s.get(i) * ldg_vec(T.uncoset_br + i));
}
__global__ void k_ntt_small(Fr *data, NttTables T, uint32_t log_n, int inverse, int coset) {
    extern __shared__ uint4 smem[];
    const uint32_t n = 1u << log_n;
    SmemPoly s{smem, smem + n};
    Fr *poly = data + (size_t)blockIdx.x * n;
    Fr one_c = Fr::zero();
    one_c.l[0] = 1;
    if (!inverse) {
        Fr nn = T.ninv.inverse();
        for (uint32_t i = threadIdx.x; i < n; i += blockDim.x) {
            Fr v = Fr::from_canonical(ld_vec(poly + i));
            if (coset) v = v * ldg_vec(T.coset_br + bitrev(i, log_n)) * nn;
            s.put(i, v);
        }
        __syncthreads();
        ntt_dif(s, log_n, T.tw_fwd);
        for (uint32_t i = threadIdx.x; i < n; i += blockDim.x) st_vec(poly + bitrev(i, log_n), s.get(i).to_canonical());
    } else {
        for (uint32_t i = threadIdx.x; i < n; i += blockDim.x) s.put(i, Fr::from_canonical(ld_vec(poly + i)));
        __syncthreads();
        ntt_dif(s, log_n, T.tw_inv);
        for (uint32_t i = threadIdx.x; i < n; i += blockDim.x) {
            Fr v = s.get(i);
            v = coset ? v * ldg_vec(T.uncoset_br + i) : (v * T.ninv).to_canonical();
            st_vec(poly + bitrev(i, log_n), v);
        }
    }
}

__global__ void k_pointwise_h(const Fr *a, const Fr *b, const Fr *c, Fr *hq, Fr zinv, size_t n) {
    size_t i = (size_t)blockIdx.x * blockDim.x + threadIdx.x;
    if (i >= n) return;
    st_vec(hq + i, (ld_vec(a + i) * ld_vec(b + i) - ld_vec(c + i)) * zinv);
}
__global__ void k_fr_to_canonical(Fr *v, size_t n) {
    size_t i = (size_t)blockIdx.x * blockDim.x + threadIdx.x;
    if (i >= n) return;
    st_vec(v + i, ld_vec(v + i).to_canonical());
}
__global__ void k_check_canonical(const Fr *v, uint32_t count, int32_t *status) {
    uint32_t i = blockIdx.x * blockDim.x + threadIdx.x;
    if (i >= count) return;
    if (!fr_is_canonical(ld_vec(v + i))) status[0] = 1;
}

template <class DigT>
__global__ void __launch_bounds__(128) k_digits(const Fr *scalars, uint32_t stride, uint32_t first, DigT *dig,
                                                uint32_t row0, uint32_t P, uint32_t c, uint32_t W, int32_t *status,
                                                uint32_t count) {
    uint32_t p = blockIdx.x * blockDim.x + threadIdx.x;
    if (p >= P) return;
    for (uint32_t j = blockIdx.y; j < count; j += gridDim.y) {
        Fr s = ld_vec(scalars + (size_t)p * stride + first + j);
        if (!fr_is_canonical(s)) {
            status[p] = 1;
            s = Fr::zero();
        }
        uint32_t v[10];
        recode_offset(s, c, W, v);
        const size_t base = ((size_t)(row0 + j) * W) * P + p;
        for (uint32_t w = 0; w < W; w++) dig[base + (size_t)w * P] = (DigT)recoded_digit(v, c, w);
    }
}
template <class DigT>
__global__ void __launch_bounds__(128) k_digits_scaled(const Fr *scalars, uint32_t stride, uint32_t first, const Fr *mult,
                                                       DigT *dig, uint32_t row0, uint32_t P, uint32_t c, uint32_t W,
                                                       uint32_t count) {
    uint32_t p = blockIdx.x * blockDim.x + threadIdx.x;
    if (p >= P) return;
    Fr m = ld_vec(mult + p);
    if (!fr_is_canonical(m)) m = Fr::zero();
    const Fr mr2 = m * Fr::r2();
    for (uint32_t j = blockIdx.y; j < count; j += gridDim.y) {
        Fr z = ld_vec(scalars + (size_t)p * stride + first + j);
        if (!fr_is_canonical(z)) z = Fr::zero();
        const Fr s = z * mr2;
        uint32_t v[10];
        recode_offset(s, c, W, v);
        const size_t base = ((size_t)(row0 + j) * W) * P + p;
        for (uint32_t w = 0; w < W; w++) dig[base + (size_t)w * P] = (DigT)recoded_digit(v, c, w);
    }
}
__global__ void k_fr_mul_canonical(const Fr *r, const Fr *s, Fr *rs, uint32_t P) {
    uint32_t p = blockIdx.x * blockDim.x + threadIdx.x;
    if (p >= P) return;
    st_vec(rs + p, (ld_vec(r + p) * ld_vec(s + p)) * Fr::r2());
}

struct ProofConsts {
    G1Affine a0;
    G1Affine b0;
    G2Affine b2;
};
__device__ __forceinline__ G1XYZZ glv_half(const G1XYZZ &P, const Fr &k, int half) {
    GlvSplit sp = glv_split(k);
    if (!sp.ok) return half == 0 ? scalar_mul(P, k) : G1XYZZ::inf();
    G1XYZZ Q = P;
    if (half == 1) {
        Fq beta;
#pragma unroll
        for (int i = 0; i < 8; i++) beta.l[i] = FqParams::BETA(i);
        Q.x = Q.x * beta;
    }
    if (half == 0 ? sp.neg1 : sp.neg2) Q.y = Q.y.neg();
    return half == 0 ? scalar_mul_u128(Q, sp.k1) : scalar_mul_u128(Q, sp.k2);
}
__global__ void __launch_bounds__(128) k_assemble(const G1XYZZ *g1, const G2XYZZ *g2, ProofConsts K, const Fr *r,
                                                  const Fr *s, uint32_t P, uint8_t *proofs) {
    __shared__ uint4 sm_raw[3 * 32 * sizeof(G1XYZZ) / 16];
    G1XYZZ *sm = reinterpret_cast<G1XYZZ *>(sm_raw);
    const uint32_t role = threadIdx.x >> 5, lane = threadIdx.x & 31, p = blockIdx.x * 32 + lane;
    const bool live = p < P;
    uint8_t *out = proofs + (size_t)p * 256;
    G1XYZZ acc = G1XYZZ::inf(), A = G1XYZZ::inf();
    if (live) {
        if (role <= 1) {
            A = ld_vec(g1 + p);
            A.add_cold(ld_vec(g1 + 4 * (size_t)P + p));
            A.madd_cold(K.a0);
            if (role == 0) acc = glv_half(A, ld_vec(s + p), 0);
            else st_vec(sm + lane, glv_half(A, ld_vec(s + p), 1));
        } else {
            G1XYZZ B1 = ld_vec(g1 + (size_t)P + p);
            B1.add_cold(ld_vec(g1 + 4 * (size_t)P + p));
            B1.madd_cold(K.b0);
            st_vec(sm + (role - 1) * 32 + lane, glv_half(B1, ld_vec(r + p), role - 2));
        }
    }
    __syncthreads();
    if (!live) return;
    if (role == 0) {
        acc.add_cold(ld_vec(sm + lane));
        acc.add_cold(ld_vec(sm + 32 + lane));
        acc.add_cold(ld_vec(sm + 64 + lane));
        acc.add_cold(ld_vec(g1 + 2 * (size_t)P + p));
        acc.add_cold(ld_vec(g1 + 3 * (size_t)P + p));
        write_g1(out + 192, acc.to_affine());
    } else if (role == 1) {
        write_g1(out, A.to_affine());
    } else if (role == 2) {
        G2XYZZ B2 = ld_vec(g2 + p);
        B2.madd_cold(K.b2);
        write_g2(out + 64, B2.to_affine());
    }
}

__global__ void __launch_bounds__(128) k_scale_a(G1XYZZ *g1, ProofConsts K, const Fr *r, const Fr *s, int with_consts) {
    __shared__ uint4 sm_raw[3 * sizeof(G1XYZZ) / 16];
    G1XYZZ *sm = reinterpret_cast<G1XYZZ *>(sm_raw);
    const uint32_t role = threadIdx.x >> 5, lane = threadIdx.x & 31;
    G1XYZZ acc = G1XYZZ::inf();
    if (lane == 0 && (role <= 1 || with_consts)) {
        G1XYZZ X = role <= 1 ? ld_vec(g1) : G1XYZZ::from_affine(K.b0);
        if (role <= 1 && with_consts) X.madd_cold(K.a0);
        acc = glv_half(X, ld_vec(role <= 1 ? s : r), role & 1);
    }
    if (lane == 0 && role) st_vec(sm + (role - 1), acc);
    __syncthreads();
    if (threadIdx.x == 0) {
        acc.add_cold(ld_vec(sm));
        acc.add_cold(ld_vec(sm + 1));
        acc.add_cold(ld_vec(sm + 2));
        st_vec(g1 + 4, acc);
    }
}
__global__ void k_scalars_times(const Fr *z, const Fr *k, Fr *out, uint32_t count) {
    const uint32_t i = blockIdx.x * blockDim.x + threadIdx.x;
    if (i >= count) return;
    st_vec(out + i, (ld_vec(z + i) * ld_vec(k)) * Fr::r2());
}
__global__ void k_add_slot(G1XYZZ *g1, int dst, int src) {
    G1XYZZ a = ld_vec(g1 + dst);
    a.add_cold(ld_vec(g1 + src));
    st_vec(g1 + dst, a);
}

__global__ void __launch_bounds__(96) k_assemble_sums(const G1XYZZ *g1, const G2XYZZ *g2, ProofConsts K, uint32_t P,
                                                      uint8_t *proofs, int q0, int q1) {
    const uint32_t role = threadIdx.x >> 5, lane = threadIdx.x & 31, p = blockIdx.x * 32 + lane;
    if (p >= P) return;
    uint8_t *out = proofs + (size_t)p * 256;
    if (role == 0) {
        G1XYZZ acc = ld_vec(g1 + (size_t)q0 * P + p);
        if (q1 >= 0) acc.add_cold(ld_vec(g1 + (size_t)q1 * P + p));
        acc.add_cold(ld_vec(g1 + 2 * (size_t)P + p));
        acc.add_cold(ld_vec(g1 + 3 * (size_t)P + p));
        write_g1(out + 192, acc.to_affine());
    } else if (role == 1) {
        G1XYZZ A = ld_vec(g1 + p);
        A.madd_cold(K.a0);
        write_g1(out, A.to_affine());
    } else {
        G2XYZZ B2 = ld_vec(g2 + p);
        B2.madd_cold(K.b2);
        write_g2(out + 64, B2.to_affine());
    }
}

__global__ void __launch_bounds__(128) k_envelope(const uint8_t *proofs, const uint8_t *commit, const int32_t *status,
                                                  const uint64_t *sets, const uint32_t *set_len, uint32_t set_stride,
                                                  uint32_t scheme, uint32_t P, uint8_t *out, uint32_t out_stride,
                                                  uint32_t *out_len) {
    const uint32_t p = (blockIdx.x * blockDim.x + threadIdx.x) >> 5, lane = threadIdx.x & 31;
    if (p >= P) return;
    uint8_t *o = out + (size_t)p * out_stride;
    if (status[p] != 0) {
        if (lane == 0) out_len[p] = 0;
        return;
    }
    const uint32_t len = sets ? set_len[p] : 0, prefix = sets ? 4 + 8 * len : 0, payload = prefix + 256;
    if (lane == 0) {
        o[0] = 2; o[1] = (uint8_t)scheme;
        for (int i = 0; i < 4; i++) { o[2 + i] = (uint8_t)(payload >> (8 * i)); o[6 + i] = (uint8_t)(32u >> (8 * i)); }
        if (sets) for (int i = 0; i < 4; i++) o[10 + i] = (uint8_t)(len >> (8 * i));
        out_len[p] = 10 + payload + 32;
    }
    if (sets) {
        const uint8_t *sv = reinterpret_cast<const uint8_t *>(sets + (size_t)p * set_stride);
        for (uint32_t i = lane; i < 8 * len; i += 32) o[14 + i] = sv[i];
    }
    for (uint32_t i = lane; i < 256; i += 32) o[10 + prefix + i] = proofs[(size_t)p * 256 + i];
    o[10 + payload + lane] = commit[(size_t)p * 32 + lane];
}

constexpr uint32_t kPartialBytes = 4 * sizeof(G1XYZZ) + sizeof(G2XYZZ);
__global__ void k_sum_partials(const uint8_t *partials, uint32_t n, G1XYZZ *g1, G2XYZZ *g2) {
    const uint32_t q = threadIdx.x >> 5;
    if (threadIdx.x & 31) return;
    if (q < 4) {
        G1XYZZ acc = G1XYZZ::inf();
        for (uint32_t i = 0; i < n; i++)
            acc.add_cold(ld_vec(reinterpret_cast<const G1XYZZ *>(partials + (size_t)i * kPartialBytes) + q));
        st_vec(g1 + q, acc);
    } else if (q == 4) {
        G2XYZZ acc = G2XYZZ::inf();
        for (uint32_t i = 0; i < n; i++)
            acc.add_cold(ld_vec(reinterpret_cast<const G2XYZZ *>(partials + (size_t)i * kPartialBytes + 4 * sizeof(G1XYZZ))));
        st_vec(g2, acc);
    }
}

template <class F>
__global__ void k_affine_add(const Affine<F> *a, const Affine<F> *b, Affine<F> *out, int negate_b) {
    XYZZ<F> s = XYZZ<F>::from_affine(ld_vec(a));
    Affine<F> q = ld_vec(b);
    if (negate_b) q = q.neg();
    s.madd_cold(q);
    st_vec(out, s.to_affine());
}
__global__ void k_check_g1(const G1Affine *pts, uint32_t n, int *bad) {
    uint32_t i = blockIdx.x * blockDim.x + threadIdx.x;
    if (i >= n) return;
    if (!g1_on_curve(ld_vec(pts + i))) atomicAdd(bad, 1);
}
__global__ void k_check_g2(const G2Affine *pts, uint32_t n, int *bad) {
    uint32_t i = blockIdx.x * blockDim.x + threadIdx.x;
    if (i >= n) return;
    G2Affine p = ld_vec(pts + i);
    if (!g2_on_curve(p)) { atomicAdd(bad, 1); return; }
    if (p.is_inf()) return;
    Fr rm1 = Fr::modulus();
    rm1.l[0] -= 1;
    G2XYZZ t = scalar_mul(G2XYZZ::from_affine(p), rm1);
    t.madd_cold(p);
    if (!t.is_inf()) atomicAdd(bad, 1);
}

}
```

### libzkp_b200/engine.py

```python
from __future__ import annotations

import ctypes as C
from typing import Optional, Sequence, Tuple

import numpy as np

from . import _ffi
from ._ffi import check, lib

EQUALITY = _ffi.LZKP_CIRCUIT_EQUALITY
MEMBERSHIP = _ffi.LZKP_CIRCUIT_MEMBERSHIP


def _p(a: Optional[np.ndarray]):
    return None if a is None else a.ctypes.data_as(C.c_void_p)


def _u8(a, shape_tail: int) -> np.ndarray:
    a = np.ascontiguousarray(a, dtype=np.uint8)
    if a.size % shape_tail:
        raise ValueError(f"byte array size {a.size} is not a multiple of {shape_tail}")
    return a.reshape(-1, shape_tail)


def init(device=None) -> None:
    if device is None:
        check(lib().lzkp_init(None, 0))
    else:
        devs = [int(device)] if isinstance(device, (int, np.integer)) else [int(d) for d in device]
        arr = (C.c_int * len(devs))(*devs)
        check(lib().lzkp_init(arr, len(devs)))


def device_count() -> int:
    return int(lib().lzkp_device_count())


def profile_enable(on: bool) -> None:
    check(lib().lzkp_profile_enable(int(on)))


def kernel_launches() -> int:
    return int(lib().lzkp_kernel_launches())


def commit_value_snark(value: int) -> bytes:
    out = (C.c_uint8 * 32)()
    check(lib().lzkp_commit_value_snark(C.c_uint64(int(value) & (2**64 - 1)), out))
    return bytes(out)


def builtin_circuit_csr(kind: int, param: int):
    shape = (C.c_uint64 * 6)()
    check(lib().lzkp_builtin_circuit_csr(kind, param, shape, None, None, None))
    m, n_inst, n_wit = int(shape[0]), int(shape[1]), int(shape[2])
    mats = [(np.zeros(m + 1, np.uint32), np.zeros(int(shape[3 + k]), np.uint32),
             np.zeros((int(shape[3 + k]), 32), np.uint8)) for k in range(3)]
    rp = (C.c_void_p * 3)(*[m_[0].ctypes.data for m_ in mats])
    cl = (C.c_void_p * 3)(*[m_[1].ctypes.data for m_ in mats])
    vl = (C.c_void_p * 3)(*[m_[2].ctypes.data for m_ in mats])
    check(lib().lzkp_builtin_circuit_csr(kind, param, shape, rp, cl, vl))
    return (m, n_inst, n_wit), mats


def key_sizes(m: int, n_inst: int, n_wit: int) -> Tuple[int, int]:
    pl, vl = C.c_size_t(), C.c_size_t()
    check(lib().lzkp_key_sizes(m, n_inst, n_wit, C.byref(pl), C.byref(vl)))
    return int(pl.value), int(vl.value)


def _toxic(toxic: Sequence[int]) -> np.ndarray:
    if len(toxic) != 5:
        raise ValueError("toxic waste = (alpha, beta, gamma, delta, tau)")
    return np.frombuffer(b"".join(int(t).to_bytes(32, "little") for t in toxic), np.uint8).copy()


def setup_builtin(kind: int, param: int, toxic: Sequence[int]) -> Tuple[bytes, bytes]:
    (m, n_inst, n_wit), _ = builtin_circuit_csr(kind, param)
    pl, vl = key_sizes(m, n_inst, n_wit)
    pk, vk, tx = np.zeros(pl, np.uint8), np.zeros(vl, np.uint8), _toxic(toxic)
    check(lib().lzkp_setup_builtin(kind, param, _p(tx), _p(pk), pl, _p(vk), vl))
    return pk.tobytes(), vk.tobytes()


def setup(m: int, n_inst: int, n_wit: int, mats, toxic: Sequence[int]) -> Tuple[bytes, bytes]:
    pl, vl = key_sizes(m, n_inst, n_wit)
    pk, vk, tx = np.zeros(pl, np.uint8), np.zeros(vl, np.uint8), _toxic(toxic)
    flat, keep = [], []
    for rowptr, col, val in mats:
        arrs = [np.ascontiguousarray(rowptr, np.uint32), np.ascontiguousarray(col, np.uint32),
                np.ascontiguousarray(val, np.uint8)]
        keep += arrs
        flat += [_p(a) for a in arrs]
    check(lib().lzkp_setup(m, n_inst, n_wit, *flat, _p(tx), _p(pk), pl, _p(vk), vl))
    return pk.tobytes(), vk.tobytes()


def builtin_witness(kind: int, param: int, value: int, other: int = 0, set_: Optional[Sequence[int]] = None,
                    commitment: Optional[bytes] = None) -> np.ndarray:
    (_, n_inst, n_wit), _ = (builtin_circuit_shape(kind, param), None)
    z = np.zeros((n_inst + n_wit, 32), np.uint8)
    sa = None if set_ is None else np.asarray(list(set_), np.uint64)
    cm = None if commitment is None else np.frombuffer(commitment, np.uint8).copy()
    check(lib().lzkp_builtin_witness(kind, param, int(value), int(other), _p(sa), 0 if sa is None else len(sa), _p(cm),
                                     _p(z), z.size))
    return z


def builtin_circuit_shape(kind: int, param: int) -> Tuple[int, int, int]:
    shape = (C.c_uint64 * 6)()
    check(lib().lzkp_builtin_circuit_csr(kind, param, shape, None, None, None))
    return int(shape[0]), int(shape[1]), int(shape[2])


class ProvingKey:

    def __init__(self, pk_bytes: bytes, validate: bool = False, window_bits: int = 0,
                 table_budget_bytes: int = 0, max_chunk: int = 0, shard_index: int = 0, shard_count: int = 0):
        self._h = C.c_void_p()
        buf = np.frombuffer(pk_bytes, dtype=np.uint8)
        opt = _ffi.PkOptions(window_bits, table_budget_bytes, max_chunk, shard_index, shard_count)
        check(lib().lzkp_pk_load_ex(_p(buf), len(pk_bytes), int(validate), C.byref(opt), C.byref(self._h)))
        info = (C.c_uint64 * 8)()
        check(lib().lzkp_pk_info(self._h, info))
        (self.n_vars, self.n_inst, self.n_wit, self.n, self.window_bits, self.windows, self.table_bytes,
         self.max_chunk) = [int(x) for x in info]

    def work(self):
        w = (C.c_uint64 * 4)()
        check(lib().lzkp_pk_work(self._h, w))
        return tuple(int(x) for x in w)

    def shard_info(self):
        first, count, k = (C.c_uint32 * 5)(), (C.c_uint32 * 5)(), C.c_uint32()
        check(lib().lzkp_pk_shard_info(self._h, first, count, C.byref(k)))
        return list(first), list(count), int(k.value)

    def close(self):
        if self._h:
            lib().lzkp_pk_free(self._h)
            self._h = C.c_void_p()

    def __del__(self):
        try:
            self.close()
        except Exception:
            pass

    REGIONS = ("witgen", "witness_map", "digits", "msm_g1", "msm_g2", "assemble")

    def profile_read(self, reset: bool = True):
        ms, cnt = (C.c_double * 8)(), (C.c_uint64 * 8)()
        check(lib().lzkp_profile_read(self._h, ms, cnt, int(reset)))
        return {name: (float(ms[i]), int(cnt[i])) for i, name in enumerate(self.REGIONS)}

    def circuit_builtin(self, kind: int, param: int) -> "ProvingKey":
        check(lib().lzkp_circuit_builtin(self._h, kind, param))
        return self

    def circuit_load(self, m: int, n_inst: int, n_wit: int, mats) -> "ProvingKey":
        flat = []
        keep = []
        for rowptr, col, val in mats:
            rowptr = np.ascontiguousarray(rowptr, np.uint32)
            col = np.ascontiguousarray(col, np.uint32)
            val = np.ascontiguousarray(val, np.uint8)
            keep += [rowptr, col, val]
            flat += [_p(rowptr), _p(col), _p(val)]
        check(lib().lzkp_circuit_load(self._h, m, n_inst, n_wit, *flat))
        return self

    def prove_batch(self, z, r, s) -> Tuple[np.ndarray, np.ndarray]:
        z = _u8(z, 32 * self.n_vars)
        n = z.shape[0]
        r, s = _u8(r, 32), _u8(s, 32)
        if r.shape[0] != n or s.shape[0] != n:
            raise ValueError("r, s must hold one scalar per proof")
        proofs = np.zeros((n, 256), np.uint8)
        status = np.zeros(n, np.int32)
        check(lib().lzkp_prove_batch(self._h, n, _p(z), _p(r), _p(s), _p(proofs), _p(status)))
        return proofs, status

    def prove_batch_device(self, n: int, d_z: int, d_r: int, d_s: int, d_proofs: int, d_status: int,
                           stream: int = 0) -> None:
        check(lib().lzkp_prove_batch_device(self._h, n, d_z, d_r, d_s, d_proofs, d_status, stream))

    def witness_map_device(self, d_z: int, d_h: int, stream: int = 0) -> None:
        check(lib().lzkp_witness_map_device(self._h, d_z, d_h, stream))

    def prove_partial_device(self, d_z: int, d_r: int, d_s: int, d_h: int, d_partial: int, d_status: int,
                             stream: int = 0, phase: int = 3) -> None:
        check(lib().lzkp_prove_partial_device(self._h, d_z, d_r, d_s, d_h, d_partial, d_status, stream, phase))

    def prove_combine_device(self, d_partials: int, n_partials: int, d_r: int, d_s: int, d_proof: int,
                             stream: int = 0) -> None:
        check(lib().lzkp_prove_combine_device(self._h, d_partials, n_partials, d_r, d_s, d_proof, stream))

    def prove_equality_batch(self, a, b, r, s, commitments=None, out=None):
        a = np.ascontiguousarray(a, np.uint64)
        b = np.ascontiguousarray(b, np.uint64)
        n = a.shape[0]
        r, s = _u8(r, 32), _u8(s, 32)
        cm = None if commitments is None else _u8(commitments, 32)
        if out is not None:
            proofs, cm_out, status = out
            if (proofs.shape, cm_out.shape, status.shape) != ((n, 256), (n, 32), (n,)) or proofs.dtype != np.uint8 \
                    or cm_out.dtype != np.uint8 or status.dtype != np.int32 or not (proofs.flags.c_contiguous and cm_out.flags.c_contiguous):
                raise ValueError("out buffers must be C-contiguous (n, 256) uint8, (n, 32) uint8, (n,) int32")
        else:
            proofs = np.zeros((n, 256), np.uint8)
            cm_out = np.zeros((n, 32), np.uint8)
            status = np.zeros(n, np.int32)
        check(lib().lzkp_prove_equality_batch(self._h, n, _p(a), _p(b), _p(cm), _p(r), _p(s), _p(proofs), _p(cm_out),
                                              _p(status)))
        return proofs, cm_out, status

    def prove_equality_enveloped(self, a, b, r, s):
        a = np.ascontiguousarray(a, np.uint64)
        b = np.ascontiguousarray(b, np.uint64)
        n = a.shape[0]
        r, s = _u8(r, 32), _u8(s, 32)
        env = np.zeros((n, 298), np.uint8)
        lens = np.zeros(n, np.uint32)
        status = np.zeros(n, np.int32)
        check(lib().lzkp_prove_equality_enveloped(self._h, n, _p(a), _p(b), _p(r), _p(s), _p(env), _p(lens), _p(status)))
        return env, lens, status

    def prove_membership_enveloped(self, value, sets, set_len, r, s):
        value = np.ascontiguousarray(value, np.uint64)
        sets = np.ascontiguousarray(sets, np.uint64)
        set_len = np.ascontiguousarray(set_len, np.uint32)
        n, stride = value.shape[0], sets.shape[1]
        r, s = _u8(r, 32), _u8(s, 32)
        row = 302 + 8 * stride
        env = np.zeros((n, row), np.uint8)
        lens = np.zeros(n, np.uint32)
        status = np.zeros(n, np.int32)
        check(lib().lzkp_prove_membership_enveloped(self._h, n, _p(value), _p(sets), _p(set_len), stride, _p(r), _p(s),
                                                    _p(env), row, _p(lens), _p(status)))
        return env, lens, status

    def prove_membership_batch(self, value, sets, set_len, r, s, commitments=None):
        value = np.ascontiguousarray(value, np.uint64)
        sets = np.ascontiguousarray(sets, np.uint64)
        set_len = np.ascontiguousarray(set_len, np.uint32)
        n = value.shape[0]
        stride = sets.shape[1] if sets.ndim == 2 else 0
        r, s = _u8(r, 32), _u8(s, 32)
        cm = None if commitments is None else _u8(commitments, 32)
        proofs = np.zeros((n, 256), np.uint8)
        cm_out = np.zeros((n, 32), np.uint8)
        status = np.zeros(n, np.int32)
        check(lib().lzkp_prove_membership_batch(self._h, n, _p(value), _p(sets), _p(set_len), stride, _p(cm), _p(r),
                                                _p(s), _p(proofs), _p(cm_out), _p(status)))
        return proofs, cm_out, status

    def prove_equality_batch_device(self, n: int, d_a: int, d_b: int, d_r: int, d_s: int, d_proofs: int,
                                    d_status: int, stream: int = 0) -> None:
        check(lib().lzkp_prove_equality_batch_device(self._h, n, d_a, d_b, d_r, d_s, d_proofs, d_status, stream))

    def witness_map(self, z) -> np.ndarray:
        z = _u8(z, 32 * self.n_vars)
        n = z.shape[0]
        h = np.zeros((n, self.n, 32), np.uint8)
        check(lib().lzkp_witness_map(self._h, n, _p(z), _p(h)))
        return h


def msm_g1(bases, scalars) -> bytes:
    bases, scalars = _u8(bases, 64), _u8(scalars, 32)
    n = min(bases.shape[0], scalars.shape[0])
    out = np.zeros(64, np.uint8)
    check(lib().lzkp_msm_g1(_p(bases), _p(scalars), n, _p(out)))
    return out.tobytes()


def msm_g2(bases, scalars) -> bytes:
    bases, scalars = _u8(bases, 128), _u8(scalars, 32)
    n = min(bases.shape[0], scalars.shape[0])
    out = np.zeros(128, np.uint8)
    check(lib().lzkp_msm_g2(_p(bases), _p(scalars), n, _p(out)))
    return out.tobytes()


def ntt(data, inverse: bool = False, coset: bool = False) -> np.ndarray:
    a = _u8(data, 32).copy()
    n = a.shape[0]
    log_n = n.bit_length() - 1
    if n == 0 or (1 << log_n) != n:
        raise ValueError("NTT size must be a power of two")
    check(lib().lzkp_ntt(_p(a), log_n, int(inverse), int(coset)))
    return a


def ntt_device(d_in: int, d_out: int, log_n: int, inverse: bool = False, coset: bool = False, stream: int = 0) -> None:
    check(lib().lzkp_ntt_device(d_in, d_out, log_n, int(inverse), int(coset), stream))


class MsmBases:

    def __init__(self, group: int, bases, window_bits: int = 0, resident_windows: bool = True, validate: bool = False):
        self.group = group
        self.point_bytes = 64 if group == 1 else 128
        bases = _u8(bases, self.point_bytes)
        self.n = bases.shape[0]
        self._h = C.c_void_p()
        check(lib().lzkp_bases_load(group, _p(bases), self.n, window_bits, int(resident_windows), int(validate),
                                    C.byref(self._h)))

    def msm(self, scalars) -> bytes:
        scalars = _u8(scalars, 32)
        out = np.zeros(self.point_bytes, np.uint8)
        check(lib().lzkp_msm(self._h, _p(scalars), scalars.shape[0], _p(out)))
        return out.tobytes()

    def msm_device(self, d_scalars: int, n: int, d_out: int, stream: int = 0) -> None:
        check(lib().lzkp_msm_device(self._h, d_scalars, n, d_out, stream))

    def close(self):
        if self._h:
            lib().lzkp_bases_free(self._h)
            self._h = C.c_void_p()

    def __del__(self):
        try:
            self.close()
        except Exception:
            pass


def generator_mul(group: int, scalars) -> np.ndarray:
    scalars = _u8(scalars, 32)
    out = np.zeros((scalars.shape[0], 64 if group == 1 else 128), np.uint8)
    check(lib().lzkp_generator_mul(group, _p(scalars), scalars.shape[0], _p(out)))
    return out


class VerifyingKey:

    def __init__(self, vk_bytes: bytes):
        self._h = C.c_void_p()
        buf = np.frombuffer(vk_bytes, dtype=np.uint8)
        check(lib().lzkp_vk_load(_p(buf), len(vk_bytes), C.byref(self._h)))
        self.n_pub = (len(vk_bytes) - 456) // 64 - 1

    def verify_batch(self, proofs, public_inputs) -> np.ndarray:
        proofs = _u8(proofs, 256)
        n = proofs.shape[0]
        x = np.ascontiguousarray(public_inputs, np.uint8).reshape(n, -1) if n else np.zeros((0, 0), np.uint8)
        n_pub = x.shape[1] // 32 if n else self.n_pub
        ok = np.zeros(n, np.uint8)
        check(lib().lzkp_verify_batch(self._h, n, _p(proofs), _p(x) if x.size else None, n_pub, _p(ok)))
        return ok.astype(bool)

    def info(self):
        v = (C.c_uint64 * 4)()
        check(lib().lzkp_vk_info(self._h, v))
        return int(v[0]), int(v[1]), bool(v[2]), bool(v[3])

    def close(self):
        if self._h:
            lib().lzkp_vk_free(self._h)
            self._h = C.c_void_p()

    def __del__(self):
        try:
            self.close()
        except Exception:
            pass
```

Before: 178,500.

## Fold C-matrix contribution into proving-key H and L bases at circuit install

At circuit install, precomputes modified h_query and l_query bases so the C polynomial's contribution to the quotient is absorbed into the MSM bases. The per-proof witness map then skips the C SpMV and its NTT, doing only two inverse-coset NTTs and a cheap pointwise fold with a precomputed w^-k table (NTT count per proof drops from 7 to 4). This costs a large one-time batch MSM at install, extra device memory for the original rows, and applies only when every L/H base is non-infinity and C touches no instance columns. It also makes concurrent G2 MSM on a side stream the default.

```diff
diff --git a/include/lzkp_b200.h b/include/lzkp_b200.h
--- a/include/lzkp_b200.h
+++ b/include/lzkp_b200.h
@@ -49,6 +49,7 @@
 void lzkp_pk_free(lzkp_pk *pk);
 int lzkp_pk_info(const lzkp_pk *pk, uint64_t info[8]);
 int lzkp_pk_work(const lzkp_pk *pk, uint64_t work[4]);
+int lzkp_pk_map_info(const lzkp_pk *pk, uint32_t info[2]);
 
 int lzkp_circuit_load(lzkp_pk *pk, uint32_t m, uint32_t n_inst, uint32_t n_wit,
                       const uint32_t *a_rowptr, const uint32_t *a_col, const uint8_t *a_val,
diff --git a/integration/rust/lzkp-sys/src/lib.rs b/integration/rust/lzkp-sys/src/lib.rs
--- a/integration/rust/lzkp-sys/src/lib.rs
+++ b/integration/rust/lzkp-sys/src/lib.rs
@@ -29,6 +29,7 @@
     pub fn lzkp_pk_load_ex(pk: *const u8, len: usize, validate: c_int, opt: *const lzkp_pk_options,
                            out: *mut *mut lzkp_pk) -> c_int;
     pub fn lzkp_pk_free(pk: *mut lzkp_pk);
+    pub fn lzkp_pk_map_info(pk: *const lzkp_pk, info: *mut u32) -> c_int;
     pub fn lzkp_circuit_builtin(pk: *mut lzkp_pk, kind: c_int, param: u32) -> c_int;
     pub fn lzkp_key_sizes(m: u32, n_inst: u32, n_wit: u32, pk_len: *mut usize, vk_len: *mut usize) -> c_int;
     pub fn lzkp_setup_builtin(kind: c_int, param: u32, toxic: *const u8, pk_out: *mut u8, pk_cap: usize,
diff --git a/libzkp_b200/_ffi.py b/libzkp_b200/_ffi.py
--- a/libzkp_b200/_ffi.py
+++ b/libzkp_b200/_ffi.py
@@ -38,6 +38,7 @@
     "lzkp_pk_free": (None, [_vp]),
     "lzkp_pk_info": (_int, [_vp, C.POINTER(_u64)]),
     "lzkp_pk_work": (_int, [_vp, C.POINTER(_u64)]),
+    "lzkp_pk_map_info": (_int, [_vp, C.POINTER(_u32)]),
     "lzkp_pk_shard_info": (_int, [_vp, C.POINTER(_u32), C.POINTER(_u32), C.POINTER(_u32)]),
     "lzkp_circuit_load": (_int, [_vp, _u32, _u32, _u32] + [_vp] * 9),
     "lzkp_circuit_builtin": (_int, [_vp, _int, _u32]),
diff --git a/libzkp_b200/csrc/engine.cu b/libzkp_b200/csrc/engine.cu
--- a/libzkp_b200/csrc/engine.cu
+++ b/libzkp_b200/csrc/engine.cu
@@ -156,6 +156,9 @@
     CsrDev csr[3];
     DBuf tw_fwd, tw_inv, coset_br, uncoset_br;
     NttTables ntt;
+    DBuf orig_l, orig_h, map_winv;
+    uint32_t row_l0 = 0, row_h0 = 0;
+    bool can_fold = false, folded = false;
     Workspace ws[2];
     bool large = false;
     bool tiled_wm = false;
@@ -465,8 +468,11 @@
         if (has_a) { msm1[0].push_back({j - 1, add1(a_q[j])}); a_all.push_back(msm1[0].back()); }
         if (has_b) { msm1[1].push_back({j - 1, add1(b1_q[j])}); b1_all.push_back(msm1[1].back()); }
     }
+    pk->row_l0 = (uint32_t)rows1.size();
     for (uint32_t j = 0; j < pk->n_wit; j++) if (!host::is_inf(l_q[j])) msm1[2].push_back({pk->n_inst + j - 1, add1(l_q[j])});
+    pk->row_h0 = (uint32_t)rows1.size();
     for (uint32_t i = 0; i + 1 < n; i++) if (!host::is_inf(h_q[i])) msm1[3].push_back({ROW_H + i, add1(h_q[i])});
+    pk->can_fold = msm1[2].size() == pk->n_wit && msm1[3].size() == n - 1;
     if (!host::is_inf(delta_g1)) {
         uint32_t rd1 = add1(delta_g1), rnd1 = add1(neg_canon(delta_g1));
         msm1[0].push_back({ROW_R, rd1});
@@ -543,6 +549,15 @@
     };
     to_mont(d_rows1, rows1.size() * 2); to_mont(d_rows2, rows2.size() * 4);
     to_mont(d_misc1, misc1.size() * 2); to_mont(d_misc2, misc2.size() * 4);
+    if (pk->can_fold) {
+        TRY(pk->orig_l.alloc((size_t)pk->n_wit * sizeof(G1Affine)));
+        TRY(pk->orig_h.alloc((size_t)(n - 1) * sizeof(G1Affine)));
+        if (pk->n_wit)
+            CUDA_TRY(cudaMemcpyAsync(pk->orig_l.p, d_rows1.as<G1Affine>() + pk->row_l0, (size_t)pk->n_wit * sizeof(G1Affine),
+                                     cudaMemcpyDeviceToDevice, st));
+        CUDA_TRY(cudaMemcpyAsync(pk->orig_h.p, d_rows1.as<G1Affine>() + pk->row_h0, (size_t)(n - 1) * sizeof(G1Affine),
+                                 cudaMemcpyDeviceToDevice, st));
+    }
     if (validate) {
         std::vector<host::G1Canon> all1 = gamma_abc;
         std::vector<host::G2Canon> all2;
@@ -603,6 +618,10 @@
     return LZKP_OK;
 }
 
+static int unfold_rows(lzkp_pk *pk, cudaStream_t st);
+static int fold_circuit(lzkp_pk *pk, uint32_t m, const uint32_t *c_rowptr, const uint32_t *c_col, const uint8_t *c_val,
+                        Fr wi, Fr gi, Fr s, cudaStream_t st);
+
 static int circuit_install(lzkp_pk *pk, uint32_t m, uint32_t n_inst, uint32_t n_wit, const uint32_t *const rowptr[3],
                            const uint32_t *const col[3], const uint8_t *const val[3]) {
     if (n_inst != pk->n_inst || n_wit != pk->n_wit) return fail(LZKP_E_INVALID, "circuit shape does not match the proving key");
@@ -610,11 +629,17 @@
     uint32_t n = 1;
     while (n < need) n <<= 1;
     if (n != pk->n) return fail(LZKP_E_INVALID, "circuit domain size does not match the proving key's h_query");
+    for (int k = 0; k < 3; k++)
+        for (uint32_t i = 0; i < rowptr[k][m]; i++)
+            if (col[k][i] >= pk->n_vars) return fail(LZKP_E_INVALID, "matrix column out of range");
+    pk->has_circuit = false;
     pk->tiled_wm = pk->large || pk->log_n > 12;
     cudaStream_t st = pk->stream;
+    TRY(ws_acquire(pk->ws[0], st));
+    TRY(ws_acquire(pk->ws[1], st));
+    CUDA_TRY(cudaStreamSynchronize(st));
     for (int k = 0; k < 3; k++) {
         uint32_t nnz = rowptr[k][m];
-        for (uint32_t i = 0; i < nnz; i++) if (col[k][i] >= pk->n_vars) return fail(LZKP_E_INVALID, "matrix column out of range");
         TRY(pk->csr_rowptr[k].alloc(sizeof(uint32_t) * (m + 1)));
         TRY(pk->csr_col[k].alloc(sizeof(uint32_t) * nnz));
         TRY(pk->csr_val[k].alloc(sizeof(Fr) * (size_t)nnz));
@@ -634,6 +659,10 @@
     Fr gn = g;
     for (uint32_t i = 0; i < pk->log_n; i++) gn = gn.sqr();
     Fr zinv = (gn - Fr::one()).inverse();
+    if (!pk->large) {
+        TRY(unfold_rows(pk, st));
+        if (pk->can_fold) TRY(fold_circuit(pk, m, rowptr[2], col[2], val[2], wi, gi, ninv * zinv, st));
+    }
     if (pk->tiled_wm) {
         pk->ntt = NttTables{nullptr, nullptr, nullptr, nullptr, nullptr, ninv, zinv};
         CUDA_TRY(cudaStreamSynchronize(st));
@@ -704,6 +733,94 @@
     return LZKP_OK;
 }
 
+
+static int rebuild_rows(lzkp_pk *pk, const DBuf &pts, uint32_t row0, uint32_t count, cudaStream_t st) {
+    if (!count) return LZKP_OK;
+    uint8_t *dst = pk->g1.table.as<uint8_t>() + (size_t)row0 * pk->W * pk->N * sizeof(G1Affine);
+    return build_table_g1(pts.p, count, pk->c, pk->W, pk->N, dst, st);
+}
+static int unfold_rows(lzkp_pk *pk, cudaStream_t st) {
+    if (!pk->folded) return LZKP_OK;
+    TRY(rebuild_rows(pk, pk->orig_l, pk->row_l0, pk->n_wit, st));
+    TRY(rebuild_rows(pk, pk->orig_h, pk->row_h0, pk->n - 1, st));
+    pk->folded = false;
+    return LZKP_OK;
+}
+static int fold_circuit(lzkp_pk *pk, uint32_t m, const uint32_t *c_rowptr, const uint32_t *c_col, const uint8_t *c_val,
+                        Fr wi, Fr gi, Fr s, cudaStream_t st) {
+    const uint32_t n = pk->n, nh = n - 1, ni = pk->n_inst, nw = pk->n_wit, W = pk->W;
+    std::vector<std::vector<std::pair<uint32_t, Fr>>> cols(nw);
+    for (uint32_t i = 0; i < m; i++)
+        for (uint32_t e = c_rowptr[i]; e < c_rowptr[i + 1]; e++) {
+            if (c_col[e] < ni) return LZKP_OK;
+            Fr v;
+            memcpy(v.l, c_val + 32 * (size_t)e, 32);
+            cols[c_col[e] - ni].push_back({i, Fr::from_canonical(v)});
+        }
+    std::vector<uint32_t> cptr{0}, crow, ecol;
+    std::vector<Fr> cval;
+    for (uint32_t j = 0; j < nw; j++) {
+        if (cols[j].empty()) continue;
+        ecol.push_back(j);
+        for (auto &e : cols[j]) { crow.push_back(e.first); cval.push_back(e.second); }
+        cptr.push_back((uint32_t)crow.size());
+    }
+    const uint32_t U = nh + (uint32_t)ecol.size();
+    DBuf gs, d_cptr, d_crow, d_cval, d_ecol, sc, dig, part, res, stat, bad, new_h, new_l;
+    TRY(pk->map_winv.alloc(sizeof(Fr) * n));
+    TRY(gs.alloc(sizeof(Fr) * n));
+    LAUNCH(k_pow_table, (n + 127) / 128, 128, 0, st, pk->map_winv.as<Fr>(), wi, Fr::one(), n, 0u);
+    LAUNCH(k_pow_table, (n + 127) / 128, 128, 0, st, gs.as<Fr>(), gi, s, n, 0u);
+    TRY(upload(d_cptr, cptr)); TRY(upload(d_crow, crow)); TRY(upload(d_cval, cval)); TRY(upload(d_ecol, ecol));
+    MsmPlan plan;
+    {
+        std::vector<std::vector<BaseRef>> msm(1);
+        for (uint32_t i = 0; i < nh; i++) msm[0].push_back({i, pk->row_h0 + i});
+        TRY(finish_plan(plan, msm, W));
+    }
+    const uint32_t dig_bytes = pk->c > 16 ? 4u : 2u;
+    const int iv = fit_variant(plan, 2);
+    const uint64_t per = (uint64_t)n * 32 + (uint64_t)nh * W * dig_bytes + (uint64_t)plan.n_items[iv] * sizeof(G1XYZZ) + 256;
+    const uint32_t Pc = (uint32_t)std::max<uint64_t>(1, std::min<uint64_t>({(uint64_t)U, 65535, (512ull << 20) / per}));
+    TRY(sc.alloc((size_t)Pc * n * sizeof(Fr)));
+    TRY(dig.alloc((size_t)nh * W * Pc * dig_bytes));
+    TRY(part.alloc((size_t)plan.n_items[iv] * Pc * sizeof(G1XYZZ)));
+    TRY(res.alloc((size_t)Pc * sizeof(G1XYZZ)));
+    TRY(stat.alloc((size_t)Pc * sizeof(int32_t)));
+    TRY(bad.alloc(sizeof(int)));
+    TRY(new_h.alloc((size_t)nh * sizeof(G1Affine)));
+    TRY(new_l.alloc((size_t)nw * sizeof(G1Affine)));
+    CUDA_TRY(cudaMemsetAsync(bad.p, 0, sizeof(int), st));
+    if (nw) CUDA_TRY(cudaMemcpyAsync(new_l.p, pk->orig_l.p, (size_t)nw * sizeof(G1Affine), cudaMemcpyDeviceToDevice, st));
+    for (uint32_t u0 = 0; u0 < U; u0 += Pc) {
+        const uint32_t P = std::min(Pc, U - u0), gx = (P + 127) / 128, ny = std::min(nh, 32768u);
+        LAUNCH(k_fold_scalars, dim3((nh + 127) / 128, P), 128, 0, st, sc.as<Fr>(), u0, pk->map_winv.as<Fr>(), gs.as<Fr>(), s,
+               d_cptr.as<uint32_t>(), d_crow.as<uint32_t>(), d_cval.as<Fr>(), pk->log_n);
+        if (dig_bytes == 2)
+            LAUNCH(k_digits<int16_t>, dim3(gx, ny), 128, 0, st, sc.as<Fr>(), n, 0u, dig.as<int16_t>(), 0u, P, (uint32_t)pk->c, W,
+                   stat.as<int32_t>(), nh);
+        else
+            LAUNCH(k_digits<int32_t>, dim3(gx, ny), 128, 0, st, sc.as<Fr>(), n, 0u, dig.as<int32_t>(), 0u, P, (uint32_t)pk->c, W,
+                   stat.as<int32_t>(), nh);
+        batch_msm_g1(BatchMsmArgs{pk->g1.table.p, pk->N, plan.unit_dig.as<uint32_t>(), plan.unit_tbl.as<uint32_t>(),
+                                  plan.items[iv].p, plan.n_items[iv], plan.msm_items[iv].p, 1u, dig.p, dig_bytes, P, part.p,
+                                  res.p},
+                     st);
+        LAUNCH(k_fold_rows, gx, 128, 0, st, res.as<G1XYZZ>(), u0, P, nh, d_ecol.as<uint32_t>(), pk->orig_l.as<G1Affine>(),
+               new_h.as<G1Affine>(), new_l.as<G1Affine>(), bad.as<int>());
+    }
+    int n_bad = 0;
+    CUDA_TRY(cudaMemcpyAsync(&n_bad, bad.p, sizeof(int), cudaMemcpyDeviceToHost, st));
+    CUDA_TRY(cudaStreamSynchronize(st));
+    CUDA_TRY(cudaGetLastError());
+    if (n_bad) return LZKP_OK;
+    pk->folded = true;
+    TRY(rebuild_rows(pk, new_l, pk->row_l0, nw, st));
+    TRY(rebuild_rows(pk, new_h, pk->row_h0, nh, st));
+    CUDA_TRY(cudaStreamSynchronize(st));
+    return LZKP_OK;
+}
+
 static inline void wires_to_canonical(Fr *z, uint32_t P, uint32_t nv, uint32_t first, uint32_t count, cudaStream_t st) {
     const size_t total = (size_t)P * count;
     LAUNCH(k_wires_to_canonical, (unsigned)((total + 127) / 128), 128, 0, st, z, P, nv, first, count);
@@ -723,15 +840,29 @@
     ~Region() { if (b) cudaEventRecord(b, st); }
 };
 
-static int run_witness_map(lzkp_pk *pk, Workspace &ws, uint32_t P, cudaStream_t st) {
+static int run_witness_map(lzkp_pk *pk, Workspace &ws, uint32_t P, cudaStream_t st, bool folded) {
     const uint32_t n = pk->n, threads = std::max(32u, std::min(n / 2, 512u));
     const size_t smem = (size_t)32 * n;
     Region reg(pk, LZKP_REGION_WITNESS_MAP, st);
+    if (folded) {
+        Fr *ab = ws.abc.as<Fr>();
+        LAUNCH(k_spmv_abc, dim3((n + 127) / 128, P), 128, 0, st, pk->csr[0], pk->csr[1], pk->csr[2], ws.z.as<Fr>(), ab, P,
+               pk->n_vars, pk->m, pk->n_inst, n, 0);
+        if (pk->tiled_wm) {
+            Fr *tmp = ws.tmp.as<Fr>();
+            TRY(large_ntt_device(ab, tmp, pk->log_n, 1, 0, st, 2 * P, n));
+            TRY(large_ntt_device(tmp, ab, pk->log_n, 0, 1, st, 2 * P, n));
+        } else {
+            LAUNCH(k_ntt_icoset, dim3(P, 2), threads, smem, st, ab, pk->ntt, P, pk->log_n);
+        }
+        LAUNCH(k_map_fold_q, dim3((n + 127) / 128, P), 128, 0, st, ab, ws.h.as<Fr>(), pk->map_winv.as<Fr>(), P, pk->log_n);
+        return LZKP_OK;
+    }
     if (pk->tiled_wm) {
         Fr *abc = ws.abc.as<Fr>(), *tmp = ws.tmp.as<Fr>(), *h = ws.h.as<Fr>();
         const size_t plane = (size_t)P * n;
         LAUNCH(k_spmv_abc, dim3((n + 127) / 128, P), 128, 0, st, pk->csr[0], pk->csr[1], pk->csr[2], ws.z.as<Fr>(), abc, P,
-               pk->n_vars, pk->m, pk->n_inst, n);
+               pk->n_vars, pk->m, pk->n_inst, n, 1);
         TRY(large_ntt_device(abc, tmp, pk->log_n, 1, 0, st, 3 * P, n));
         TRY(large_ntt_device(tmp, abc, pk->log_n, 0, 1, st, 3 * P, n));
         LAUNCH(k_pointwise_h, (unsigned)((plane + 127) / 128), 128, 0, st, abc, abc + plane, abc + 2 * plane, tmp, pk->ntt.zinv,
@@ -741,7 +872,7 @@
         return LZKP_OK;
     }
     LAUNCH(k_spmv_abc, dim3((n + 127) / 128, P), 128, 0, st, pk->csr[0], pk->csr[1], pk->csr[2], ws.z.as<Fr>(),
-           ws.abc.as<Fr>(), P, pk->n_vars, pk->m, pk->n_inst, n);
+           ws.abc.as<Fr>(), P, pk->n_vars, pk->m, pk->n_inst, n, 1);
     LAUNCH(k_ntt_icoset, dim3(P, 3), threads, smem, st, ws.abc.as<Fr>(), pk->ntt, P, pk->log_n);
     LAUNCH(k_ntt_final, P, threads, smem, st, ws.abc.as<Fr>(), ws.h.as<Fr>(), pk->ntt, P, pk->log_n);
     return LZKP_OK;
@@ -795,7 +926,7 @@
         }
         }
         if (!(phase & 2)) return LZKP_OK;
-        if (!have_h && cnt[3]) TRY(run_witness_map(pk, ws, P, st));
+        if (!have_h && cnt[3]) TRY(run_witness_map(pk, ws, P, st, false));
         TRY(msm_device_raw(pk->L_h, ws.h.as<uint8_t>() + (size_t)lo[3] * 32, cnt[3], res1 + 3, st));
         for (int i = 0; i < 3; i++) {
             CUDA_TRY(cudaEventRecord(pk->L_ev_done[i], pk->L_st[i]));
@@ -835,42 +966,42 @@
         return BatchMsmArgs{pl.table.p, pk->N, pl.unit_dig.as<uint32_t>(), pl.unit_tbl.as<uint32_t>(), pl.items[iv].p,
                             pl.n_items[iv], pl.msm_items[iv].p, pl.n_msm, dig, dig_bytes, P, partial, out};
     };
-    cudaStream_t st_g2 = st;
+    static const bool g2_conc = !getenv("LZKP_G2_CONCURRENT") || atoi(getenv("LZKP_G2_CONCURRENT")) != 0;
+    const bool g2_side = lat || g2_conc;
+    auto fork_g2 = [&]() -> int {
+        CUDA_TRY(cudaEventRecord(pk->L_ev_in, st));
+        CUDA_TRY(cudaStreamWaitEvent(pk->L_st[0], pk->L_ev_in, 0));
+        { Region reg(pk, LZKP_REGION_MSM_G2, pk->L_st[0]); batch_msm_g2(args(pk->g2, fit_variant(pk->g2, item_variant_g2(P)), ws.part2.p, ws.res2.p), pk->L_st[0]); }
+        CUDA_TRY(cudaEventRecord(pk->L_ev_done[0], pk->L_st[0]));
+        return LZKP_OK;
+    };
     if (lat) {
         {
             Region reg(pk, LZKP_REGION_DIGITS, st);
             LAUNCH(k_fr_mul_canonical, gx, 128, 0, st, d_r, d_s, ws.rs.as<Fr>(), P);
             if (dig_bytes == 2) TRY(digits_z((int16_t *)dig)); else TRY(digits_z((int32_t *)dig));
         }
-        st_g2 = pk->L_st[0];
-        CUDA_TRY(cudaEventRecord(pk->L_ev_in, st));
-        CUDA_TRY(cudaStreamWaitEvent(st_g2, pk->L_ev_in, 0));
-        { Region reg(pk, LZKP_REGION_MSM_G2, st_g2); batch_msm_g2(args(pk->g2, fit_variant(pk->g2, item_variant_g2(P)), ws.part2.p, ws.res2.p), st_g2); }
-        CUDA_TRY(cudaEventRecord(pk->L_ev_done[0], st_g2));
-        if (!have_h) TRY(run_witness_map(pk, ws, P, st));
+        TRY(fork_g2());
+        if (!have_h) TRY(run_witness_map(pk, ws, P, st, pk->folded));
         { Region reg(pk, LZKP_REGION_DIGITS, st); if (dig_bytes == 2) TRY(digits_h((int16_t *)dig)); else TRY(digits_h((int32_t *)dig)); }
     } else {
-        if (!have_h) TRY(run_witness_map(pk, ws, P, st));
-        Region reg(pk, LZKP_REGION_DIGITS, st);
-        LAUNCH(k_fr_mul_canonical, gx, 128, 0, st, d_r, d_s, ws.rs.as<Fr>(), P);
-        if (dig_bytes == 2) { TRY(digits_z((int16_t *)dig)); TRY(digits_h((int16_t *)dig)); }
-        else { TRY(digits_z((int32_t *)dig)); TRY(digits_h((int32_t *)dig)); }
+        if (!have_h) TRY(run_witness_map(pk, ws, P, st, pk->folded));
+        {
+            Region reg(pk, LZKP_REGION_DIGITS, st);
+            LAUNCH(k_fr_mul_canonical, gx, 128, 0, st, d_r, d_s, ws.rs.as<Fr>(), P);
+            if (dig_bytes == 2) { TRY(digits_z((int16_t *)dig)); TRY(digits_h((int16_t *)dig)); }
+            else { TRY(digits_z((int32_t *)dig)); TRY(digits_h((int32_t *)dig)); }
+        }
+        if (g2_side) TRY(fork_g2());
     }
     MsmPlan &pl1 = lat ? pk->g1_lat : pk->g1;
-    static const bool g2_conc = getenv("LZKP_G2_CONCURRENT") && atoi(getenv("LZKP_G2_CONCURRENT")) != 0;
-    if (!lat && g2_conc) {
-        CUDA_TRY(cudaEventRecord(pk->L_ev_in, st));
-        CUDA_TRY(cudaStreamWaitEvent(pk->L_st[0], pk->L_ev_in, 0));
-        { Region reg(pk, LZKP_REGION_MSM_G2, pk->L_st[0]); batch_msm_g2(args(pk->g2, fit_variant(pk->g2, item_variant_g2(P)), ws.part2.p, ws.res2.p), pk->L_st[0]); }
-        CUDA_TRY(cudaEventRecord(pk->L_ev_done[0], pk->L_st[0]));
-    }
     {
         Region reg(pk, LZKP_REGION_MSM_G1, st);
         BatchMsmArgs a1 = args(pl1, fit_variant(pl1, item_variant(P)), ws.part1.p, ws.res1.p);
         a1.table = pk->g1.table.p;
         batch_msm_g1(a1, st);
     }
-    if (lat || g2_conc) CUDA_TRY(cudaStreamWaitEvent(st, pk->L_ev_done[0], 0));
+    if (g2_side) CUDA_TRY(cudaStreamWaitEvent(st, pk->L_ev_done[0], 0));
     else { Region reg(pk, LZKP_REGION_MSM_G2, st); batch_msm_g2(args(pk->g2, fit_variant(pk->g2, item_variant_g2(P)), ws.part2.p, ws.res2.p), st); }
     Region reg(pk, LZKP_REGION_ASSEMBLE, st);
     if (lat) {
@@ -1194,6 +1325,13 @@
     return LZKP_OK;
 }
 
+int lzkp_pk_map_info(const lzkp_pk *pk, uint32_t info[2]) {
+    if (!pk || !info) return fail(LZKP_E_INVALID, "null argument");
+    info[0] = pk->folded ? 4 : 7;
+    info[1] = pk->folded ? 1 : 0;
+    return LZKP_OK;
+}
+
 int lzkp_pk_shard_info(const lzkp_pk *pk, uint32_t first[5], uint32_t count[5], uint32_t *map_ranks) {
     if (!pk || !first || !count) return fail(LZKP_E_INVALID, "null argument");
     if (!pk->large) return fail(LZKP_E_STATE, "not a large-domain proving key");
@@ -1498,7 +1636,7 @@
         TRY(ws_acquire(ws, st));
         TRY(ensure_workspace(pk, ws, P));
         CUDA_TRY(cudaMemcpyAsync(ws.z.p, z + off * nv * 32, (size_t)P * nv * 32, cudaMemcpyHostToDevice, st));
-        TRY(run_witness_map(pk, ws, P, st));
+        TRY(run_witness_map(pk, ws, P, st, false));
         CUDA_TRY(cudaMemcpyAsync(h_out + off * n * 32, ws.h.p, (size_t)P * n * 32, cudaMemcpyDeviceToHost, st));
         TRY(ws_release(ws, st));
         CUDA_TRY(cudaStreamSynchronize(st));
@@ -1517,7 +1655,7 @@
     TRY(ws_acquire(ws, st));
     TRY(ensure_workspace(pk, ws, 1));
     CUDA_TRY(cudaMemcpyAsync(ws.z.p, d_z, (size_t)pk->n_vars * 32, cudaMemcpyDeviceToDevice, st));
-    TRY(run_witness_map(pk, ws, 1, st));
+    TRY(run_witness_map(pk, ws, 1, st, false));
     CUDA_TRY(cudaMemcpyAsync(d_h, ws.h.p, (size_t)pk->n * 32, cudaMemcpyDeviceToDevice, st));
     TRY(ws_release(ws, st));
     return LZKP_OK;
diff --git a/libzkp_b200/csrc/kernels_prove.cuh b/libzkp_b200/csrc/kernels_prove.cuh
--- a/libzkp_b200/csrc/kernels_prove.cuh
+++ b/libzkp_b200/csrc/kernels_prove.cuh
@@ -127,7 +127,7 @@
     return acc;
 }
 __global__ void __launch_bounds__(128) k_spmv_abc(CsrDev A, CsrDev B, CsrDev C, const Fr *z, Fr *abc, uint32_t P,
-                                                  uint32_t nv, uint32_t m, uint32_t n_inst, uint32_t n) {
+                                                  uint32_t nv, uint32_t m, uint32_t n_inst, uint32_t n, int with_c) {
     uint32_t i = blockIdx.x * blockDim.x + threadIdx.x, p = blockIdx.y;
     if (i >= n) return;
     const Fr *zp = z + (size_t)p * nv;
@@ -135,14 +135,14 @@
     if (i < m) {
         a = spmv_row(A, i, zp);
         b = spmv_row(B, i, zp);
-        c = spmv_row(C, i, zp);
+        if (with_c) c = spmv_row(C, i, zp);
     } else if (i < m + n_inst) {
         a = Fr::from_canonical(ld_vec(zp + (i - m)));
     }
     size_t plane = (size_t)P * n, off = (size_t)p * n + i;
     st_vec(abc + off, a);
     st_vec(abc + plane + off, b);
-    st_vec(abc + 2 * plane + off, c);
+    if (with_c) st_vec(abc + 2 * plane + off, c);
 }
 
 struct SmemPoly {
@@ -223,6 +223,19 @@
     for (uint32_t i = threadIdx.x; i < n; i += blockDim.x)
         st_vec(h + off + bitrev(i, log_n), s.get(i) * ldg_vec(T.uncoset_br + i));
 }
+__global__ void __launch_bounds__(128) k_map_fold_q(const Fr *ab, Fr *h, const Fr *winv, uint32_t P, uint32_t log_n) {
+    __shared__ uint4 last_raw[2];
+    Fr *last = reinterpret_cast<Fr *>(last_raw);
+    const uint32_t n = 1u << log_n, k = blockIdx.x * blockDim.x + threadIdx.x;
+    const size_t plane = (size_t)P * n, off = (size_t)blockIdx.y * n;
+    if (threadIdx.x == 0) st_vec(last, ld_vec(ab + off + n - 1) * ld_vec(ab + plane + off + n - 1));
+    __syncthreads();
+    if (k >= n) return;
+    Fr q = Fr::zero();
+    if (k + 1 < n) q = (ld_vec(ab + off + k) * ld_vec(ab + plane + off + k) - ld_vec(last) * ldg_vec(winv + k + 1)).to_canonical();
+    st_vec(h + off + k, q);
+}
+
 __global__ void k_ntt_small(Fr *data, NttTables T, uint32_t log_n, int inverse, int coset) {
     extern __shared__ uint4 smem[];
     const uint32_t n = 1u << log_n;
@@ -464,6 +477,41 @@
     }
 }
 
+__global__ void __launch_bounds__(128) k_fold_scalars(Fr *out, uint32_t u0, const Fr *winv, const Fr *gs, Fr s,
+                                                      const uint32_t *cptr, const uint32_t *crow, const Fr *cval,
+                                                      uint32_t log_n) {
+    const uint32_t n = 1u << log_n, i = blockIdx.x * blockDim.x + threadIdx.x, u = u0 + blockIdx.y;
+    if (i + 1 >= n) return;
+    Fr v;
+    if (u + 1 < n) {
+        v = ldg_vec(gs + i) * ldg_vec(winv + ((u * i) & (n - 1)));
+    } else {
+        const uint32_t t = u - (n - 1);
+        v = Fr::zero();
+        for (uint32_t e = __ldg(cptr + t); e < __ldg(cptr + t + 1); e++)
+            v = v + ldg_vec(cval + e) * ldg_vec(winv + ((__ldg(crow + e) * i) & (n - 1)));
+        v = v * s;
+    }
+    st_vec(out + (size_t)blockIdx.y * n + i, v.to_canonical());
+}
+__global__ void k_fold_rows(const G1XYZZ *res, uint32_t u0, uint32_t cnt, uint32_t nh, const uint32_t *ecol,
+                            const G1Affine *l, G1Affine *new_h, G1Affine *new_l, int *bad) {
+    const uint32_t t = blockIdx.x * blockDim.x + threadIdx.x, u = u0 + t;
+    if (t >= cnt) return;
+    G1XYZZ acc = ld_vec(res + t);
+    G1Affine *dst;
+    if (u < nh) {
+        dst = new_h + u;
+    } else {
+        const uint32_t j = __ldg(ecol + (u - nh));
+        acc = acc.neg();
+        acc.madd_cold(ld_vec(l + j));
+        dst = new_l + j;
+    }
+    if (acc.is_inf()) atomicAdd(bad, 1);
+    st_vec(dst, acc.to_affine());
+}
+
 template <class F>
 __global__ void k_affine_add(const Affine<F> *a, const Affine<F> *b, Affine<F> *out, int negate_b) {
     XYZZ<F> s = XYZZ<F>::from_affine(ld_vec(a));
diff --git a/libzkp_b200/engine.py b/libzkp_b200/engine.py
--- a/libzkp_b200/engine.py
+++ b/libzkp_b200/engine.py
@@ -130,6 +130,11 @@
         w = (C.c_uint64 * 4)()
         check(lib().lzkp_pk_work(self._h, w))
         return tuple(int(x) for x in w)
+
+    def map_info(self):
+        v = (C.c_uint32 * 2)()
+        check(lib().lzkp_pk_map_info(self._h, v))
+        return int(v[0]), bool(v[1])
 
     def shard_info(self):
         first, count, k = (C.c_uint32 * 5)(), (C.c_uint32 * 5)(), C.c_uint32()
```

After: 186,900, median of 6. 1.05x the previous value.
